# tiangexiang/OccNeRF

Measured on AMD Instinct MI355X. Metric: rays/sec at 512x512x128spp, random-init ckpt, higher is better.
Workload: dtype f32; 1 GPU; BASELINE configs[1]: free-view frame, 512x512 image, 128 samples/ray, non-rigid motion on, seeded random-init checkpoint; synthetic SMPL-like body and camera; 183784 rays hit the body bbox (ray_mask); H2D of the ray batch and the prior and D2H of [R,5] inside the step; the frame's rays sharded over the ranks; samples whose motion-weight sum is exactly 0 are dropped after the warp (bit-identical pi; rays_per_frame=183784, samples_per_ray=128, skip_empty_samples=True, dedup_repeated_samples=False, knn_center_cache=True, warp_bone_culling=True, world_size_formed=1

## Files before the change

include/occnerf_hip.h:

```cpp
#ifndef OCCNERF_HIP_H
#define OCCNERF_HIP_H

#include <stdint.h>

#ifdef __cplusplus
extern "C" {
#endif

#define OCCNERF_ABI_VERSION 5

int occnerf_abi_version(void);
const char *occnerf_last_error(void);

int occnerf_experiment_knob(const char *name, int value);


int occnerf_grid_encode_forward(const float *inputs, const float *embeddings,
                                const int32_t *offsets, float *outputs, uint32_t B, uint32_t D,
                                uint32_t C, uint32_t L, float S, uint32_t H, float *dy_dx,
                                uint32_t gridtype, int align_corners, uint32_t interp,
                                void *stream);

int occnerf_grid_encode_backward(const float *grad, const float *inputs, const float *embeddings,
                                 const int32_t *offsets, float *grad_embeddings, uint32_t B,
                                 uint32_t D, uint32_t C, uint32_t L, float S, uint32_t H,
                                 const float *dy_dx, float *grad_inputs, uint32_t gridtype,
                                 int align_corners, uint32_t interp, void *stream);

int occnerf_grid_encode_forward_h(const float *inputs, const float *embeddings, const int32_t *offsets,
                                  const int32_t *h_offsets, float *outputs, uint32_t B, uint32_t D, uint32_t C, uint32_t L,
                                  float S, uint32_t H, float *dy_dx, uint32_t gridtype, int align_corners,
                                  uint32_t interp, void *stream);

int occnerf_grid_grad_runs(const float *grad_rows, const float *inputs, int64_t B, uint32_t D, uint32_t L, uint32_t C,
                           float *grad, void *stream);

int occnerf_grid_encode_backward_h(const float *grad, const float *inputs, const float *embeddings,
                                   const int32_t *offsets, const int32_t *h_offsets, float *grad_embeddings,
                                   uint32_t B, uint32_t D, uint32_t C, uint32_t L, float S, uint32_t H,
                                   const float *dy_dx, float *grad_inputs, uint32_t gridtype, int align_corners,
                                   uint32_t interp, void *scratch, int64_t scratch_bytes, void *stream);

int occnerf_grid_encode_forward_f16(const float *inputs, const void *embeddings, const int32_t *offsets, void *outputs,
                                    uint32_t B, uint32_t D, uint32_t C, uint32_t L, float S, uint32_t H, void *dy_dx,
                                    uint32_t gridtype, int align_corners, uint32_t interp, void *stream);
int occnerf_grid_encode_backward_f16(const void *grad, const float *inputs, const void *embeddings, const int32_t *offsets,
                                     void *grad_embeddings, uint32_t B, uint32_t D, uint32_t C, uint32_t L, float S,
                                     uint32_t H, const void *dy_dx, void *grad_inputs, uint32_t gridtype, int align_corners,
                                     uint32_t interp, void *stream);

int occnerf_grid_encode_forward_f64(const float *inputs, const double *embeddings, const int32_t *offsets, double *outputs,
                                    uint32_t B, uint32_t D, uint32_t C, uint32_t L, float S, uint32_t H, double *dy_dx,
                                    uint32_t gridtype, int align_corners, uint32_t interp, void *stream);
int occnerf_grid_encode_backward_f64(const double *grad, const float *inputs, const double *embeddings, const int32_t *offsets,
                                     double *grad_embeddings, uint32_t B, uint32_t D, uint32_t C, uint32_t L, float S,
                                     uint32_t H, const double *dy_dx, double *grad_inputs, uint32_t gridtype, int align_corners,
                                     uint32_t interp, void *stream);

int occnerf_grad_total_variation(const float *inputs, const float *embeddings, float *grad,
                                 const int32_t *offsets, float weight, uint32_t B, uint32_t D,
                                 uint32_t C, uint32_t L, float S, uint32_t H, uint32_t gridtype,
                                 int align_corners, void *stream);


int occnerf_sample_warp(const float *rays, int64_t n, int32_t S, const float *t_vals,
                        const float *t_rand, const float *Rs, const float *Ts, const float *vol,
                        int32_t nb, int32_t G, const float *h_bbox_min, const float *h_bbox_scale,
                        float *z_vals, float *pts, float *x_skel, float *mask, void *stream);
int occnerf_bone_boxes(const float *vol, int32_t nb, int32_t G, int32_t *boxes, void *stream);
int occnerf_sample_warp_culled(const float *rays, int64_t n, int32_t S, const float *t_vals,
                               const float *Rs, const float *Ts, const float *vol, int32_t nb, int32_t G,
                               const int32_t *boxes, const float *h_bbox_min, const float *h_bbox_scale,
                               float *z_vals, float *x_skel, float *mask, void *stream);

int64_t occnerf_ray_order_temp_bytes(int64_t R);
int occnerf_ray_order(const float *dirs, int64_t R, int64_t stride, int64_t *order, void *temp, int64_t temp_bytes,
                      void *stream);

int occnerf_gen_rays(const double *h_Kinv, const double *h_R, const double *h_T, int32_t f32_camera,
                     int32_t H, int32_t W, const double *h_bbox_min, const double *h_bbox_max, float *rays8,
                     uint8_t *mask, void *stream);

int64_t occnerf_nonrigid_packed_floats(void);
int occnerf_nonrigid_pack(const float *const *h_W, const float *const *h_b, float *packed,
                          void *stream);
int occnerf_nonrigid(const float *xyz_in, int64_t N, const float *cond, const float *h_hann,
                     const float *W0, const float *b0, float *packed, float *xyz_out,
                     void *stream);
int occnerf_nonrigid_rows(float *xyz, int64_t N_max, const int32_t *rows, const int32_t *n_dev,
                          const float *cond, const float *h_hann, const float *W0, const float *b0,
                          float *packed, void *stream);
int occnerf_nonrigid_direct(const float *xyz_in, int64_t N, const float *cond, const float *h_hann,
                            const float *W0, const float *b0, float *packed, float *xyz_out,
                            void *stream);

int64_t occnerf_nonrigid_packed_bf16_bytes(void);
int occnerf_nonrigid_pack_bf16(const float *const *h_W, void *packed_bf16, void *stream);
int occnerf_nonrigid_bf16x3(const float *xyz_in, int64_t N, const float *cond, const float *h_hann,
                            const float *W0, const float *b0, float *packed, const void *packed_bf16,
                            float *xyz_out, void *stream);
int occnerf_nonrigid_bf16x3_rows(float *xyz, int64_t N_max, const int32_t *rows, const int32_t *n_dev,
                                 const float *cond, const float *h_hann, const float *W0, const float *b0,
                                 float *packed, const void *packed_bf16, void *stream);

int occnerf_msknn(const float *xyz, int64_t N, const float *points, const int32_t *index_map,
                  const int32_t *h_scale_begin, const int32_t *h_seed_from_coarser,
                  int32_t nscale, int32_t *knn_idxs, void *stream);

int occnerf_msknn_clustered(const float *xyz, const float *mask, int64_t n_rays, int32_t samples_per_ray,
                            const float *points, const float *centers,
                            const int32_t *cluster_ranges, const float *cluster_radius, int32_t ncl,
                            const float *group_centers, const int32_t *group_ranges, const float *group_radius, int32_t ngrp,
                            const int32_t *h_coarse_rows, const int32_t *h_seed_from_coarser,
                            int32_t nscale, const int32_t *query_rows, const int32_t *n_query_dev, int32_t *ray_start,
                            int32_t *knn_idxs, void *stream);
int occnerf_knn_center(const float *c, const float *points, const int32_t *index_map, const int32_t *h_scale_begin,
                       int32_t nscale, float *center_out, int32_t *idx_out, void *stream);
int occnerf_msknn_clustered_centered(const float *xyz, const float *mask, int64_t n_rays, int32_t samples_per_ray,
                                     const float *points, const float *centers,
                                     const int32_t *cluster_ranges, const float *cluster_radius, int32_t ncl,
                                     const float *group_centers, const int32_t *group_ranges, const float *group_radius, int32_t ngrp,
                                     const int32_t *h_coarse_rows, const int32_t *h_seed_from_coarser,
                                     int32_t nscale, const int32_t *query_rows, const int32_t *n_query_dev, int32_t *ray_start,
                                     const float *center, const int32_t *center_idx, int32_t *knn_idxs, void *stream);

int occnerf_knn_small(const float *q, int32_t nq, const float *s, int32_t ns, int32_t k,
                      int32_t *idx, void *stream);

int occnerf_unit_normals(const double *normals, int32_t P, double *unit, void *stream);

int occnerf_point_sdf(const float *point_cloud, const float *point_base, const double *normals,
                      const double *unit_normals, const int32_t *kidx, int32_t P,
                      double *knn_base, float *dist, void *stream);

int occnerf_point_sdf_backward(const float *point_cloud, const float *point_base, const double *normals,
                               const double *unit_normals, const int32_t *kidx, int32_t P, const double *d_knn_base,
                               const float *d_dist, float *d_point_dist, void *stream);
int32_t occnerf_point_table_stride(void);
int occnerf_point_table(const double *knn_base, const float *point_sdf, const float *learnable,
                        int32_t P, float bound, float two_bound, const float *embeddings,
                        const int32_t *offsets, const int32_t *h_offsets, uint32_t L, float S,
                        uint32_t H, float *table, void *stream);

int occnerf_point_pack(const float *point_base, const double *normals, const double *unit_normals,
                       const float *counter, const float *table, int32_t P, float *point_geo,
                       float *point_tail, void *stream);
int occnerf_sample_features(const float *xyz, int64_t N, const int32_t *knn_idxs, int32_t nscale,
                            const float *point_base, const double *normals,
                            const double *unit_normals, const float *counter,
                            const float *table, float bound, float two_bound,
                            const float *embeddings, const int32_t *offsets,
                            const int32_t *h_offsets, uint32_t L, float S, uint32_t H,
                            const int32_t *geo_idxs, const float *att_in, const int32_t *rows,
                            const int32_t *n_dev, const float *point_geo, const float *point_tail, int32_t P,
                            float *mlp_in, float *raw, float *enc_in, void *stream);
int occnerf_sample_features_centered(const float *xyz, int64_t N, const int32_t *knn_idxs, int32_t nscale,
                            const float *point_base, const double *normals,
                            const double *unit_normals, const float *counter,
                            const float *table, float bound, float two_bound,
                            const float *embeddings, const int32_t *offsets,
                            const int32_t *h_offsets, uint32_t L, float S, uint32_t H,
                            const int32_t *geo_idxs, const float *att_in, const int32_t *rows,
                            const int32_t *n_dev, const float *point_geo, const float *point_tail, int32_t P,
                            const float *center, const float *center_agg,
                                     float *mlp_in, float *raw, float *enc_in, void *stream);

int occnerf_agg_forward(const float *feats, int32_t F, const int32_t *knn, const float *atts, int64_t N, int32_t K,
                        float *agg, void *stream);
int32_t occnerf_agg_backward_slices(int64_t N);
int64_t occnerf_agg_backward_scratch_bytes(int64_t N, int32_t F);
int occnerf_agg_backward(const float *grad_agg, int32_t F, const int32_t *knn, const float *atts, int64_t N,
                         int32_t K, int32_t P, float *partial, void *scratch, int64_t scratch_bytes, void *stream);

int64_t occnerf_live_rows_temp_bytes(int64_t N);
int occnerf_live_rows(const float *mask, int64_t N, int32_t *rows, int32_t *count, void *temp,
                      int64_t temp_bytes, void *stream);
int occnerf_scatter_raw(const float *raw_c, const int32_t *rows, const int32_t *n_dev, int64_t N_max,
                        float *raw_full, void *stream);

int64_t occnerf_repeat_heads_temp_bytes(int64_t N_max);
int occnerf_repeat_heads(const void *keys, int64_t stride_dwords, int32_t key_dwords, const int32_t *rows,
                         const int32_t *n_dev, int64_t N_max, int32_t *scan, int32_t *heads, int32_t *head_count,
                         float *head_mask, void *temp, int64_t temp_bytes, void *stream);
int64_t occnerf_unique_heads_temp_bytes(int64_t cap);
int occnerf_unique_heads(const void *keys, int64_t stride_dwords, int32_t key_dwords, const int32_t *heads,
                         const int32_t *n_dev, int64_t cap, int32_t *heads_out, int32_t *count_out, int32_t *scan,
                         const int32_t *n_scan_dev, int64_t scan_cap, void *temp, int64_t temp_bytes, void *stream);
int occnerf_scatter_raw_heads(const float *raw_h, const float *raw_c, const int32_t *rows, const int32_t *n_dev,
                              const int32_t *scanA, const int32_t *scanB, int64_t N_max, float *raw_full, void *stream);
int occnerf_canonical_mlp_rows(const float *mlp_in, const int32_t *in_rows, int64_t N_max, const int32_t *n_dev,
                               const float *packed, float *raw, void *stream);

int64_t occnerf_canonical_mlp_packed_floats(void);
int occnerf_canonical_mlp_pack(const float *const *h_W, const float *const *h_b, float *packed,
                               void *stream);

int occnerf_canonical_mlp(const float *mlp_in, int64_t N, const float *packed, float *raw,
                          void *stream);
int occnerf_canonical_mlp_direct(const float *mlp_in, int64_t N, const float *packed, float *raw,
                                 void *stream);
int occnerf_canonical_mlp_counted(const float *mlp_in, int64_t N_max, const int32_t *n_dev,
                                  const float *packed, float *raw, void *stream);

int64_t occnerf_canonical_mlp_packed_bf16_bytes(void);
int occnerf_canonical_mlp_pack_bf16(const float *const *h_W, void *packed_bf16, void *stream);
int occnerf_canonical_mlp_bf16x3(const float *mlp_in, int64_t N, const float *packed,
                                 const void *packed_bf16, float *raw, int32_t variant,
                                 void *stream);
int occnerf_canonical_mlp_bf16x3_rows(const float *mlp_in, const int32_t *in_rows, int64_t N_max,
                                      const int32_t *n_dev, const float *packed, const void *packed_bf16,
                                      float *raw, int32_t variant, void *stream);

int occnerf_canonical_mlp_pack_f16(const float *const *h_W, void *packed_f16, void *stream);
int occnerf_canonical_mlp_f16x3(const float *mlp_in, const int32_t *in_rows, int64_t N_max, const int32_t *n_dev,
                                const float *packed, const void *packed_f16, float *raw, uint32_t *domain_flag,
                                void *stream);
int occnerf_nonrigid_pack_f16(const float *const *h_W, void *packed_f16, void *stream);
int occnerf_nonrigid_f16x3(const float *xyz_in, int64_t N_max, const int32_t *rows, const int32_t *n_dev,
                           const float *cond, const float *h_hann, const float *W0, const float *b0, float *packed,
                           const void *packed_f16, float *xyz_out, uint32_t *domain_flag, void *stream);

int occnerf_composite(const float *raw, const float *mask, const float *z_vals, const float *rays,
                      const float *h_bgcolor, int64_t n, int32_t S, float *rgb, float *acc,
                      float *depth, float *weights, int32_t *term, const int64_t *out_rows, void *stream);


int occnerf_linear_pack(const float *W, const float *b, int32_t out_dim, int32_t in_dim, const int32_t *row_map,
                        int32_t n_pad, const int32_t *col_map, int32_t k_pad, int32_t bf16, void *Wp, void *Wt,
                        float *bias_p, void *stream);
int occnerf_linear_forward(const void *x0, int64_t ld0, int32_t k0, const void *x1, int64_t ld1, int32_t k1,
                           const void *W, const float *bias, int32_t relu, const void *mask, int64_t ldm, void *y,
                           int64_t ldy, int32_t out_f32, int32_t n_store, float *aux, int32_t aux_col,
                           int64_t aux_stride, int64_t M, int32_t n_pad, int32_t bf16, void *stream);
int32_t occnerf_linear_wgrad_slices(int64_t M);
int occnerf_linear_wgrad(const void *dz, int64_t lddz, int32_t n_pad, const void *x, int64_t ldx, int32_t k_pad,
                         int64_t M, int32_t bf16, float *part, float *dbpart, void *stream);
int occnerf_linear_wgrad_reduce(const float *part, const float *dbpart, int32_t G, int32_t n_pad, int32_t k_pad,
                                const int32_t *row_map, const int32_t *col_map, float *dW, int32_t in_dim, float *db,
                                int32_t accumulate, void *stream);

int64_t occnerf_trunks_packed_bytes(void);
int occnerf_trunks_pack_bf16(const float *const *h_W, void *packed, void *stream);
int occnerf_trunks_forward_bf16(const float *agg, const float *var, const float *enc, int64_t M, const float *packed_f32,
                                const void *packed_bf16, void *X0, void *const *h_A, void *GEO, void *const *h_B, float *raw4,
                                void *stream);

int occnerf_composite_backward(const float *raw, const float *mask, const float *z_vals, const float *rays,
                               const float *h_bgcolor, int64_t n, int32_t S, const float *g_rgb, const float *g_acc,
                               const float *g_depth, float *d_raw, float *d_mask, void *stream);

int32_t occnerf_warp_backward_slices(int64_t n_samples);
int occnerf_warp_backward(const float *rays, int64_t n, int32_t S, const float *z_vals, const float *g_mask,
                          const float *Rs, const float *Ts, const float *vol, int32_t nb, int32_t G,
                          const float *h_bbox_min, const float *h_bbox_scale, float *d_vol_part, float *d_rt_part,
                          void *stream);

int occnerf_agg_weights(const float *counter, const int32_t *knn, int64_t N, int32_t K, float *atts, float *var,
                        void *stream);

int occnerf_pose_motion_bases_backward(const float *const *h_W, const float *const *h_b, const float *posevec,
                                       const float *dst_Rs, const float *dst_Ts, const float *cnl_gtfms,
                                       const float *dRs, const float *dTs, float *const *h_dW, float *const *h_db,
                                       void *stream);

int occnerf_pose_motion_bases(const float *const *h_W, const float *const *h_b, const float *posevec, int32_t refine,
                              const float *dst_Rs, const float *dst_Ts, const float *cnl_gtfms, float *Rs, float *Ts,
                              void *stream);
int occnerf_prior_softmax(const float *decoded, const float *prior, int32_t C, int64_t V, float *vol, void *stream);
int occnerf_pack_rays(const float *rays, const float *near, const float *far, const int64_t *order, int64_t R, float *rays8,
                      void *stream);

int occnerf_assemble_image(const float *rgb, const float *alpha, const int64_t *ray_index, int64_t R, int32_t height,
                           int32_t width, const float *h_bgcolor01, uint8_t *out_rgb, uint8_t *out_alpha, void *stream);

int occnerf_convt3d_col2im(const float *cols, const float *bias, int32_t Cout, int32_t D, int32_t H, int32_t W,
                           float *out, void *stream);
int occnerf_convt3d_im2col(const float *gy, int32_t Cout, int32_t D, int32_t H, int32_t W, float *dcols, void *stream);

int32_t occnerf_adam_table_row_bytes(void);
int occnerf_adam_step(const void *table, int32_t n_tensors, const int32_t *chunks, int32_t n_chunks,
                      int32_t chunk_elems, double beta1, double beta2, double eps, double max_grad_norm, float *scratch,
                      void *stream);

int64_t occnerf_lpips_packed_floats(void);
int64_t occnerf_lpips_workspace_floats(int32_t N, int32_t H, int32_t W);
int occnerf_lpips_pack(const float *const *h_conv_w, const float *const *h_conv_b, const float *const *h_lin,
                       const float *shift, const float *scale, float *packed, void *stream);
int occnerf_lpips_forward(const float *packed, const float *in0, const float *in1, int32_t N, int32_t H, int32_t W,
                          int32_t in_nhwc, float *work, float *val, float *res, void *stream);
int occnerf_lpips_backward(const float *packed, float *work, int32_t N, int32_t H, int32_t W, int32_t in_nhwc,
                           const float *gres, float *d_in0, float *d_in1, void *stream);

int occnerf_patch_assemble(const float *rgb, const int32_t *row_of_pix, int64_t R, int32_t n_patches, int32_t size,
                           const float *h_bgcolor01, float *img, void *stream);
int occnerf_patch_assemble_backward(const float *d_img, const int32_t *pix_of_row, int64_t R, float *d_rgb, void *stream);

#define OCCNERF_FRAME_METRICS_RECORD 14
int64_t occnerf_frame_metrics_workspace_bytes(int32_t N, int32_t H, int32_t W);
int occnerf_frame_metrics(const uint8_t *pred, const uint8_t *truth, const float *alpha, const uint8_t *body,
                          const float *gt_vis_alpha, const float *gt_alpha, int32_t N, int32_t H, int32_t W,
                          double data_range, double *record, double *ssim_map, void *workspace, void *stream);

#ifdef __cplusplus
}
#endif
#endif
```

occnerf_amd/_lib.py:

```python
import ctypes as C
import os

_HERE = os.path.dirname(os.path.abspath(__file__))
LIB_PATH = os.environ.get('OCCNERF_HIP_LIB') or os.path.join(_HERE, 'liboccnerf_hip.so')

ABI_VERSION = 5

_vp, _i32, _i64, _u32, _f32 = C.c_void_p, C.c_int32, C.c_int64, C.c_uint32, C.c_float

SIGNATURES = {
    'occnerf_abi_version': (C.c_int, []),
    'occnerf_last_error': (C.c_char_p, []),
    'occnerf_experiment_knob': (C.c_int, [C.c_char_p, C.c_int]),
    'occnerf_grid_encode_forward': (C.c_int, [_vp, _vp, _vp, _vp, _u32, _u32, _u32, _u32, _f32, _u32,
                                               _vp, _u32, C.c_int, _u32, _vp]),
    'occnerf_grid_encode_backward': (C.c_int, [_vp, _vp, _vp, _vp, _vp, _u32, _u32, _u32, _u32, _f32,
                                                _u32, _vp, _vp, _u32, C.c_int, _u32, _vp]),
    'occnerf_grid_grad_runs': (C.c_int, [_vp, _vp, _i64, _u32, _u32, _u32, _vp, _vp]),
    'occnerf_grid_encode_forward_h': (C.c_int, [_vp, _vp, _vp, _vp, _vp, _u32, _u32, _u32, _u32, _f32, _u32,
                                                 _vp, _u32, C.c_int, _u32, _vp]),
    'occnerf_grid_encode_backward_h': (C.c_int, [_vp, _vp, _vp, _vp, _vp, _vp, _u32, _u32, _u32, _u32, _f32,
                                                  _u32, _vp, _vp, _u32, C.c_int, _u32, _vp, _i64, _vp]),
    'occnerf_grid_encode_forward_f16': (C.c_int, [_vp, _vp, _vp, _vp, _u32, _u32, _u32, _u32, _f32, _u32,
                                                   _vp, _u32, C.c_int, _u32, _vp]),
    'occnerf_grid_encode_backward_f16': (C.c_int, [_vp, _vp, _vp, _vp, _vp, _u32, _u32, _u32, _u32, _f32,
                                                    _u32, _vp, _vp, _u32, C.c_int, _u32, _vp]),
    'occnerf_grid_encode_forward_f64': (C.c_int, [_vp, _vp, _vp, _vp, _u32, _u32, _u32, _u32, _f32, _u32,
                                                   _vp, _u32, C.c_int, _u32, _vp]),
    'occnerf_grid_encode_backward_f64': (C.c_int, [_vp, _vp, _vp, _vp, _vp, _u32, _u32, _u32, _u32, _f32,
                                                    _u32, _vp, _vp, _u32, C.c_int, _u32, _vp]),
    'occnerf_trunks_packed_bytes': (_i64, []),
    'occnerf_trunks_pack_bf16': (C.c_int, [_vp, _vp, _vp]),
    'occnerf_trunks_forward_bf16': (C.c_int, [_vp, _vp, _vp, _i64, _vp, _vp, _vp, _vp, _vp, _vp, _vp, _vp]),
    'occnerf_grad_total_variation': (C.c_int, [_vp, _vp, _vp, _vp, _f32, _u32, _u32, _u32, _u32, _f32,
                                                _u32, _u32, C.c_int, _vp]),
    'occnerf_sample_warp': (C.c_int, [_vp, _i64, _i32, _vp, _vp, _vp, _vp, _vp, _i32, _i32, _vp, _vp,
                                       _vp, _vp, _vp, _vp, _vp]),
    'occnerf_bone_boxes': (C.c_int, [_vp, _i32, _i32, _vp, _vp]),
    'occnerf_sample_warp_culled': (C.c_int, [_vp, _i64, _i32, _vp, _vp, _vp, _vp, _i32, _i32, _vp, _vp, _vp, _vp, _vp, _vp, _vp]),
    'occnerf_nonrigid_packed_floats': (_i64, []),
    'occnerf_nonrigid_pack': (C.c_int, [_vp, _vp, _vp, _vp]),
    'occnerf_nonrigid': (C.c_int, [_vp, _i64, _vp, _vp, _vp, _vp, _vp, _vp, _vp]),
    'occnerf_nonrigid_direct': (C.c_int, [_vp, _i64, _vp, _vp, _vp, _vp, _vp, _vp, _vp]),
    'occnerf_nonrigid_packed_bf16_bytes': (_i64, []),
    'occnerf_nonrigid_pack_bf16': (C.c_int, [_vp, _vp, _vp]),
    'occnerf_nonrigid_bf16x3': (C.c_int, [_vp, _i64, _vp, _vp, _vp, _vp, _vp, _vp, _vp, _vp]),
    'occnerf_nonrigid_bf16x3_rows': (C.c_int, [_vp, _i64, _vp, _vp, _vp, _vp, _vp, _vp, _vp, _vp, _vp]),
    'occnerf_msknn': (C.c_int, [_vp, _i64, _vp, _vp, _vp, _vp, _i32, _vp, _vp]),
    'occnerf_msknn_clustered': (C.c_int, [_vp, _vp, _i64, _i32, _vp, _vp, _vp, _vp, _i32, _vp, _vp, _vp, _i32, _vp, _vp, _i32,
                                           _vp, _vp, _vp, _vp, _vp]),
    'occnerf_msknn_clustered_centered': (C.c_int, [_vp, _vp, _i64, _i32, _vp, _vp, _vp, _vp, _i32, _vp, _vp, _vp, _i32, _vp, _vp, _i32,
                                           _vp, _vp, _vp, _vp, _vp, _vp, _vp]),
    'occnerf_knn_center': (C.c_int, [_vp, _vp, _vp, _vp, _i32, _vp, _vp, _vp]),
    'occnerf_knn_small': (C.c_int, [_vp, _i32, _vp, _i32, _i32, _vp, _vp]),
    'occnerf_unit_normals': (C.c_int, [_vp, _i32, _vp, _vp]),
    'occnerf_point_sdf': (C.c_int, [_vp, _vp, _vp, _vp, _vp, _i32, _vp, _vp, _vp]),
    'occnerf_ray_order_temp_bytes': (_i64, [_i64]),
    'occnerf_ray_order': (C.c_int, [_vp, _i64, _i64, _vp, _vp, _i64, _vp]),
    'occnerf_point_sdf_backward': (C.c_int, [_vp, _vp, _vp, _vp, _vp, _i32, _vp, _vp, _vp, _vp]),
    'occnerf_gen_rays': (C.c_int, [_vp, _vp, _vp, _i32, _i32, _i32, _vp, _vp, _vp, _vp, _vp]),
    'occnerf_agg_forward': (C.c_int, [_vp, _i32, _vp, _vp, _i64, _i32, _vp, _vp]),
    'occnerf_agg_backward_slices': (_i32, [_i64]),
    'occnerf_agg_backward_scratch_bytes': (_i64, [_i64, _i32]),
    'occnerf_agg_backward': (C.c_int, [_vp, _i32, _vp, _vp, _i64, _i32, _i32, _vp, _vp, _i64, _vp]),
    'occnerf_live_rows_temp_bytes': (_i64, [_i64]),
    'occnerf_live_rows': (C.c_int, [_vp, _i64, _vp, _vp, _vp, _i64, _vp]),
    'occnerf_scatter_raw': (C.c_int, [_vp, _vp, _vp, _i64, _vp, _vp]),
    'occnerf_repeat_heads_temp_bytes': (_i64, [_i64]),
    'occnerf_repeat_heads': (C.c_int, [_vp, _i64, _i32, _vp, _vp, _i64, _vp, _vp, _vp, _vp, _vp, _i64, _vp]),
    'occnerf_unique_heads_temp_bytes': (_i64, [_i64]),
    'occnerf_unique_heads': (C.c_int, [_vp, _i64, _i32, _vp, _vp, _i64, _vp, _vp, _vp, _vp, _i64, _vp, _i64, _vp]),
    'occnerf_scatter_raw_heads': (C.c_int, [_vp, _vp, _vp, _vp, _vp, _vp, _i64, _vp, _vp]),
    'occnerf_canonical_mlp_rows': (C.c_int, [_vp, _vp, _i64, _vp, _vp, _vp, _vp]),
    'occnerf_canonical_mlp_counted': (C.c_int, [_vp, _i64, _vp, _vp, _vp, _vp]),
    'occnerf_nonrigid_rows': (C.c_int, [_vp, _i64, _vp, _vp, _vp, _vp, _vp, _vp, _vp, _vp]),
    'occnerf_point_table_stride': (_i32, []),
    'occnerf_point_table': (C.c_int, [_vp, _vp, _vp, _i32, _f32, _f32, _vp, _vp, _vp, _u32, _f32, _u32, _vp,
                                       _vp]),
    'occnerf_point_pack': (C.c_int, [_vp, _vp, _vp, _vp, _vp, _i32, _vp, _vp, _vp]),
    'occnerf_sample_features': (C.c_int, [_vp, _i64, _vp, _i32, _vp, _vp, _vp, _vp, _vp, _f32, _f32, _vp,
                                           _vp, _vp, _u32, _f32, _u32, _vp, _vp, _vp, _vp, _vp, _vp, _i32, _vp, _vp,
                                           _vp, _vp]),
    'occnerf_sample_features_centered': (C.c_int, [_vp, _i64, _vp, _i32, _vp, _vp, _vp, _vp, _vp, _f32, _f32, _vp,
                                                    _vp, _vp, _u32, _f32, _u32, _vp, _vp, _vp, _vp, _vp, _vp, _i32, _vp, _vp,
                                                    _vp, _vp, _vp, _vp]),
    'occnerf_canonical_mlp_packed_floats': (_i64, []),
    'occnerf_canonical_mlp_pack': (C.c_int, [_vp, _vp, _vp, _vp]),
    'occnerf_canonical_mlp': (C.c_int, [_vp, _i64, _vp, _vp, _vp]),
    'occnerf_canonical_mlp_direct': (C.c_int, [_vp, _i64, _vp, _vp, _vp]),
    'occnerf_canonical_mlp_packed_bf16_bytes': (_i64, []),
    'occnerf_canonical_mlp_pack_bf16': (C.c_int, [_vp, _vp, _vp]),
    'occnerf_canonical_mlp_bf16x3': (C.c_int, [_vp, _i64, _vp, _vp, _vp, _i32, _vp]),
    'occnerf_canonical_mlp_pack_f16': (C.c_int, [_vp, _vp, _vp]),
    'occnerf_canonical_mlp_f16x3': (C.c_int, [_vp, _vp, _i64, _vp, _vp, _vp, _vp, _vp, _vp]),
    'occnerf_nonrigid_pack_f16': (C.c_int, [_vp, _vp, _vp]),
    'occnerf_nonrigid_f16x3': (C.c_int, [_vp, _i64, _vp, _vp, _vp, _vp, _vp, _vp, _vp, _vp, _vp, _vp, _vp]),
    'occnerf_canonical_mlp_bf16x3_rows': (C.c_int, [_vp, _vp, _i64, _vp, _vp, _vp, _vp, _i32, _vp]),
    'occnerf_composite': (C.c_int, [_vp, _vp, _vp, _vp, _vp, _i64, _i32, _vp, _vp, _vp, _vp, _vp, _vp, _vp]),
    'occnerf_linear_pack': (C.c_int, [_vp, _vp, _i32, _i32, _vp, _i32, _vp, _i32, _i32, _vp, _vp, _vp, _vp]),
    'occnerf_linear_forward': (C.c_int, [_vp, _i64, _i32, _vp, _i64, _i32, _vp, _vp, _i32, _vp, _i64, _vp, _i64, _i32,
                                          _i32, _vp, _i32, _i64, _i64, _i32, _i32, _vp]),
    'occnerf_linear_wgrad_slices': (_i32, [_i64]),
    'occnerf_linear_wgrad': (C.c_int, [_vp, _i64, _i32, _vp, _i64, _i32, _i64, _i32, _vp, _vp, _vp]),
    'occnerf_linear_wgrad_reduce': (C.c_int, [_vp, _vp, _i32, _i32, _i32, _vp, _vp, _vp, _i32, _vp, _i32, _vp]),
    'occnerf_composite_backward': (C.c_int, [_vp, _vp, _vp, _vp, _vp, _i64, _i32, _vp, _vp, _vp, _vp, _vp, _vp]),
    'occnerf_warp_backward_slices': (_i32, [_i64]),
    'occnerf_warp_backward': (C.c_int, [_vp, _i64, _i32, _vp, _vp, _vp, _vp, _vp, _i32, _i32, _vp, _vp, _vp, _vp, _vp]),
    'occnerf_agg_weights': (C.c_int, [_vp, _vp, _i64, _i32, _vp, _vp, _vp]),
    'occnerf_pose_motion_bases': (C.c_int, [_vp, _vp, _vp, _i32, _vp, _vp, _vp, _vp, _vp, _vp]),
    'occnerf_pose_motion_bases_backward': (C.c_int, [_vp, _vp, _vp, _vp, _vp, _vp, _vp, _vp, _vp, _vp, _vp]),
    'occnerf_prior_softmax': (C.c_int, [_vp, _vp, _i32, _i64, _vp, _vp]),
    'occnerf_pack_rays': (C.c_int, [_vp, _vp, _vp, _vp, _i64, _vp, _vp]),
    'occnerf_assemble_image': (C.c_int, [_vp, _vp, _vp, _i64, _i32, _i32, _vp, _vp, _vp, _vp]),
    'occnerf_convt3d_col2im': (C.c_int, [_vp, _vp, _i32, _i32, _i32, _i32, _vp, _vp]),
    'occnerf_convt3d_im2col': (C.c_int, [_vp, _i32, _i32, _i32, _i32, _vp, _vp]),
    'occnerf_adam_table_row_bytes': (_i32, []),
    'occnerf_adam_step': (C.c_int, [_vp, _i32, _vp, _i32, _i32] + [C.c_double] * 4 + [_vp, _vp]),
    'occnerf_lpips_packed_floats': (_i64, []),
    'occnerf_lpips_workspace_floats': (_i64, [_i32, _i32, _i32]),
    'occnerf_lpips_pack': (C.c_int, [_vp, _vp, _vp, _vp, _vp, _vp, _vp]),
    'occnerf_lpips_forward': (C.c_int, [_vp, _vp, _vp, _i32, _i32, _i32, _i32, _vp, _vp, _vp, _vp]),
    'occnerf_lpips_backward': (C.c_int, [_vp, _vp, _i32, _i32, _i32, _i32, _vp, _vp, _vp, _vp]),
    'occnerf_patch_assemble': (C.c_int, [_vp, _vp, _i64, _i32, _i32, _vp, _vp, _vp]),
    'occnerf_patch_assemble_backward': (C.c_int, [_vp, _vp, _i64, _vp, _vp]),
    'occnerf_frame_metrics_workspace_bytes': (_i64, [_i32, _i32, _i32]),
    'occnerf_frame_metrics': (C.c_int, [_vp, _vp, _vp, _vp, _vp, _vp, _i32, _i32, _i32, C.c_double, _vp, _vp, _vp, _vp]),
}

_lib = None


def lib():
    global _lib
    if _lib is None:
        if not os.path.exists(LIB_PATH):
            raise ImportError(
                f'{LIB_PATH} not found: the gfx950 kernels are not built. Run '
                '`python -c "import __graft_entry__ as g; g.build()"` (or `make -C '
                'occnerf_amd/csrc`). There is no CPU fallback for this path.')
        import torch
        handle = C.CDLL(LIB_PATH)
        for name, (res, args) in SIGNATURES.items():
            fn = getattr(handle, name)
            fn.restype, fn.argtypes = res, args
        if handle.occnerf_abi_version() != ABI_VERSION:
            raise ImportError(f'liboccnerf_hip.so: ABI version {handle.occnerf_abi_version()}, this binding was written '
                              f'for {ABI_VERSION} (include/occnerf_hip.h OCCNERF_ABI_VERSION): rebuild the library')
        _lib = handle
    return _lib


def check(rc, what):
    if rc != 0:
        msg = lib().occnerf_last_error().decode(errors='replace')
        raise RuntimeError(f'{what} failed ({rc}): {msg}')
```

occnerf_amd/csrc/compact.hip:

```cpp
#include "common.h"

#include <hipcub/hipcub.hpp>

namespace occ {

struct LivePredicate {
    const float *mask;
    __device__ bool operator()(const int &i) const { return mask[i] != 0.0f; }
};

__global__ void scatter_raw_kernel(const float *__restrict__ raw_c, const int32_t *__restrict__ rows,
                                   const int32_t *__restrict__ n_dev, float *__restrict__ raw_full) {
    const int64_t m = (int64_t)blockIdx.x * blockDim.x + threadIdx.x;
    if (m >= (int64_t)*n_dev) return;
    const int64_t n = rows[m];
#pragma unroll
    for (int c = 0; c < 5; c++) raw_full[n * 5 + c] = raw_c[m * 5 + c];
}

struct RepeatFlag {
    const uint32_t *keys;
    int64_t stride;
    int K;
    const int32_t *rows;
    const int32_t *n_dev;
    __device__ int operator()(const int &m) const {
        if (m >= *n_dev) return 0;
        if (m == 0) return 1;
        const uint32_t *a = keys + (rows ? (int64_t)rows[m] : (int64_t)m) * stride;
        const uint32_t *b = keys + (rows ? (int64_t)rows[m - 1] : (int64_t)(m - 1)) * stride;
        if (((K | (int)stride) & 3) == 0) {
            for (int k = 0; k < K; k += 4) {
                const uint4 x = *reinterpret_cast<const uint4 *>(a + k), y = *reinterpret_cast<const uint4 *>(b + k);
                if (x.x != y.x || x.y != y.y || x.z != y.z || x.w != y.w) return 1;
            }
            return 0;
        }
        for (int k = 0; k < K; k++)
            if (a[k] != b[k]) return 1;
        return 0;
    }
};

__global__ void repeat_flags_wide_kernel(const uint4 *__restrict__ keys, int64_t stride4, int K4,
                                         const int32_t *__restrict__ rows, const int32_t *__restrict__ n_dev,
                                         int64_t N_max, int32_t *__restrict__ flags) {
    const int g = threadIdx.x & 7;
    const int64_t m = ((int64_t)blockIdx.x * blockDim.x + threadIdx.x) >> 3;
    if (m >= N_max) return;
    const int64_t n = *n_dev;
    int diff = 0;
    if (m < n && m > 0) {
        const uint4 *a = keys + (rows ? (int64_t)rows[m] : m) * stride4;
        const uint4 *b = keys + (rows ? (int64_t)rows[m - 1] : m - 1) * stride4;
        for (int k = g; k < K4; k += 8) {
            const uint4 x = a[k], y = b[k];
            diff |= (x.x != y.x) | (x.y != y.y) | (x.z != y.z) | (x.w != y.w);
        }
    }
    diff |= __shfl_xor(diff, 1, 8);
    diff |= __shfl_xor(diff, 2, 8);
    diff |= __shfl_xor(diff, 4, 8);
    if (g == 0) flags[m] = m >= n ? 0 : (m == 0 ? 1 : diff);
}

__global__ void repeat_heads_kernel(const int32_t *__restrict__ scan, const int32_t *__restrict__ rows,
                                    const int32_t *__restrict__ n_dev, int32_t *__restrict__ heads,
                                    int32_t *__restrict__ head_count, float *__restrict__ head_mask) {
    const int64_t m = (int64_t)blockIdx.x * blockDim.x + threadIdx.x;
    const int64_t n = *n_dev;
    if (m == 0 && n <= 0) *head_count = 0;
    if (m >= n) return;
    const int32_t s = scan[m], prev = m ? scan[m - 1] : 0;
    if (s != prev) {
        const int32_t r = rows ? rows[m] : (int32_t)m;
        heads[s - 1] = r;
        if (head_mask) head_mask[r] = 1.0f;
    }
    if (m == n - 1) *head_count = s;
}

__global__ void scatter_raw_heads_kernel(const float *__restrict__ raw_h, const float *__restrict__ raw_c,
                                         const int32_t *__restrict__ rows, const int32_t *__restrict__ n_dev,
                                         const int32_t *__restrict__ scanA, const int32_t *__restrict__ scanB,
                                         float *__restrict__ raw_full) {
    const int64_t m = (int64_t)blockIdx.x * blockDim.x + threadIdx.x;
    if (m >= (int64_t)*n_dev) return;
    const int64_t n = rows[m];
    const int64_t a = scanA ? scanA[m] - 1 : m;
    const int64_t h = scanB ? scanB[a] - 1 : a;
#pragma unroll
    for (int c = 0; c < 4; c++) raw_full[n * 5 + c] = raw_h[h * 5 + c];
    raw_full[n * 5 + 4] = raw_c[a * 5 + 4];
}

__device__ __forceinline__ uint64_t mix64(uint64_t h) {
    h ^= h >> 33;
    h *= 0xff51afd7ed558ccdull;
    h ^= h >> 33;
    h *= 0xc4ceb9fe1a85ec53ull;
    h ^= h >> 33;
    return h;
}

template <int G >
__global__ void unique_insert_kernel(const uint32_t *__restrict__ keys, int64_t stride, int K,
                                     const int32_t *__restrict__ heads, const int32_t *__restrict__ n_dev,
                                     int32_t *__restrict__ table, uint32_t tmask, int32_t *__restrict__ rep) {
    const int g = threadIdx.x % G;
    const int64_t j = ((int64_t)blockIdx.x * blockDim.x + threadIdx.x) / G;
    if (j >= (int64_t)*n_dev) return;
    const uint32_t *a = keys + (heads ? (int64_t)heads[j] : j) * stride;
    uint64_t h = 0x9E3779B97F4A7C15ull * (uint64_t)(g + 1);
    for (int k = g; k < K; k += G) h = mix64(h ^ ((uint64_t)a[k] + ((uint64_t)(k + 1) << 32)));
    if (G > 1) {
        h ^= __shfl_xor(h, 1, G);
        h ^= __shfl_xor(h, 2, G);
        h ^= __shfl_xor(h, 4, G);
    }
    uint32_t slot = (uint32_t)mix64(h) & tmask;
    int32_t r = (int32_t)j;
    for (int probe = 0; probe < 32; probe++) {
        int32_t prev = 0;
        if (g == 0) prev = atomicCAS(&table[slot], -1, (int32_t)j);
        if (G > 1) prev = __shfl(prev, 0, G);
        if (prev == -1) break;
        const uint32_t *b = keys + (heads ? (int64_t)heads[prev] : (int64_t)prev) * stride;
        int diff = 0;
        for (int k = g; k < K; k += G) diff |= a[k] != b[k];
        if (G > 1) {
            diff |= __shfl_xor(diff, 1, G);
            diff |= __shfl_xor(diff, 2, G);
            diff |= __shfl_xor(diff, 4, G);
        }
        if (!diff) {
            r = prev;
            break;
        }
        slot = (slot + 1) & tmask;
    }
    if (g == 0) rep[j] = r;
}

struct IsRepresentative {
    const int32_t *rep, *n_dev;
    __device__ int operator()(const int &j) const { return j < *n_dev && rep[j] == j; }
};

__global__ void unique_finish_kernel(const int32_t *__restrict__ heads, const int32_t *__restrict__ n_dev,
                                     const int32_t *__restrict__ scan2, int32_t *__restrict__ rep,
                                     int32_t *__restrict__ heads_out, int32_t *__restrict__ count_out) {
    const int64_t j = (int64_t)blockIdx.x * blockDim.x + threadIdx.x;
    const int64_t n = *n_dev;
    if (j == 0 && n <= 0) *count_out = 0;
    if (j >= n) return;
    const int32_t r = rep[j];
    if (r == (int32_t)j) heads_out[scan2[j] - 1] = heads ? heads[j] : (int32_t)j;
    if (j == n - 1) *count_out = scan2[j];
    rep[j] = scan2[r] - 1;
}

__global__ void unique_remap_kernel(int32_t *__restrict__ scan, const int32_t *__restrict__ n_scan_dev,
                                    const int32_t *__restrict__ pos) {
    const int64_t m = (int64_t)blockIdx.x * blockDim.x + threadIdx.x;
    if (m >= (int64_t)*n_scan_dev) return;
    scan[m] = pos[scan[m] - 1] + 1;
}

}

OCC_API int64_t occnerf_repeat_heads_temp_bytes(int64_t N) {
    using namespace occ;
    if (N <= 0 || N >= (1ll << 31)) return 0;
    size_t bytes = 0;
    hipcub::CountingInputIterator<int> it(0);
    hipcub::TransformInputIterator<int, RepeatFlag, hipcub::CountingInputIterator<int>> flags(it, RepeatFlag{});
    if (hipcub::DeviceScan::InclusiveSum(nullptr, bytes, flags, (int *)nullptr, (int)N, (hipStream_t)0) != hipSuccess)
        return -1;
    size_t bytes2 = 0;
    if (hipcub::DeviceScan::InclusiveSum(nullptr, bytes2, (int *)nullptr, (int *)nullptr, (int)N, (hipStream_t)0) != hipSuccess)
        return -1;
    return (int64_t)(bytes > bytes2 ? bytes : bytes2);
}

OCC_API int occnerf_repeat_heads(const void *keys, int64_t stride_dwords, int32_t key_dwords, const int32_t *rows,
                                 const int32_t *n_dev, int64_t N_max, int32_t *scan, int32_t *heads,
                                 int32_t *head_count, float *head_mask, void *temp, int64_t temp_bytes,
                                 void *stream) {
    using namespace occ;
    OCC_REQUIRE(keys && n_dev && scan && heads && head_count && temp, "repeat_heads: null argument");
    OCC_REQUIRE(N_max > 0 && N_max < (1ll << 31), "repeat_heads: N=%lld out of range", (long long)N_max);
    OCC_REQUIRE(key_dwords > 0 && stride_dwords >= key_dwords, "repeat_heads: key of %d dwords in rows of %lld",
                key_dwords, (long long)stride_dwords);
    size_t bytes = (size_t)temp_bytes;
    hipError_t e;
    if (key_dwords >= 32 && ((key_dwords | stride_dwords) & 3) == 0) {
        const int64_t fblocks = (N_max * 8 + 255) / 256;
        OCC_REQUIRE(fblocks < (1ll << 31), "repeat_heads: N too large");
        hipLaunchKernelGGL(repeat_flags_wide_kernel, dim3((unsigned)fblocks), dim3(256), 0, as_stream(stream),
                           reinterpret_cast<const uint4 *>(keys), stride_dwords / 4, key_dwords / 4, rows, n_dev, N_max, scan);
        e = hipcub::DeviceScan::InclusiveSum(temp, bytes, scan, scan, (int)N_max, as_stream(stream));
    } else {
        hipcub::CountingInputIterator<int> it(0);
        hipcub::TransformInputIterator<int, RepeatFlag, hipcub::CountingInputIterator<int>> flags(
            it, RepeatFlag{reinterpret_cast<const uint32_t *>(keys), stride_dwords, key_dwords, rows, n_dev});
        e = hipcub::DeviceScan::InclusiveSum(temp, bytes, flags, scan, (int)N_max, as_stream(stream));
    }
    OCC_REQUIRE(e == hipSuccess, "repeat_heads: %s", hipGetErrorString(e));
    const int64_t blocks = (N_max + 255) / 256;
    hipLaunchKernelGGL(repeat_heads_kernel, dim3((unsigned)blocks), dim3(256), 0, as_stream(stream), scan, rows, n_dev,
                       heads, head_count, head_mask);
    return check_launch("repeat_heads");
}

static inline int64_t unique_table_entries(int64_t cap) {
    int64_t t = 1024;
    while (t < cap) t <<= 1;
    return t;
}

OCC_API int64_t occnerf_unique_heads_temp_bytes(int64_t cap) {
    using namespace occ;
    if (cap <= 0 || cap >= (1ll << 30)) return 0;
    size_t bytes = 0;
    hipcub::CountingInputIterator<int> it(0);
    hipcub::TransformInputIterator<int, IsRepresentative, hipcub::CountingInputIterator<int>> flags(it, IsRepresentative{});
    if (hipcub::DeviceScan::InclusiveSum(nullptr, bytes, flags, (int *)nullptr, (int)cap, (hipStream_t)0) != hipSuccess)
        return -1;
    const int64_t words = unique_table_entries(cap) + 2 * ((cap + 63) & ~63ll);
    return words * 4 + (int64_t)((bytes + 255) & ~(size_t)255);
}

OCC_API int occnerf_unique_heads(const void *keys, int64_t stride_dwords, int32_t key_dwords, const int32_t *heads,
                                 const int32_t *n_dev, int64_t cap, int32_t *heads_out, int32_t *count_out,
                                 int32_t *scan, const int32_t *n_scan_dev, int64_t scan_cap, void *temp,
                                 int64_t temp_bytes, void *stream) {
    using namespace occ;
    OCC_REQUIRE(keys && n_dev && heads_out && count_out && temp, "unique_heads: null argument");
    OCC_REQUIRE(cap > 0 && cap < (1ll << 30), "unique_heads: cap=%lld out of range", (long long)cap);
    OCC_REQUIRE(key_dwords > 0 && stride_dwords >= key_dwords, "unique_heads: key of %d dwords in rows of %lld", key_dwords,
                (long long)stride_dwords);
    OCC_REQUIRE(!scan == !n_scan_dev, "unique_heads: scan and its length come together");
    OCC_REQUIRE(temp_bytes >= occnerf_unique_heads_temp_bytes(cap), "unique_heads: temp too small");
    const int64_t T = unique_table_entries(cap), capr = (cap + 63) & ~63ll;
    int32_t *table = reinterpret_cast<int32_t *>(temp), *rep = table + T, *scan2 = rep + capr;
    void *cub_temp = scan2 + capr;
    size_t cub_bytes = (size_t)temp_bytes - (size_t)(T + 2 * capr) * 4;
    hipStream_t st = as_stream(stream);
    OCC_REQUIRE(hipMemsetAsync(table, 0xFF, (size_t)T * 4, st) == hipSuccess, "unique_heads: memset");
    const uint32_t *k32 = reinterpret_cast<const uint32_t *>(keys);
    if (key_dwords >= 32)
        hipLaunchKernelGGL(unique_insert_kernel<8>, dim3((unsigned)((cap * 8 + 255) / 256)), dim3(256), 0, st, k32,
                           stride_dwords, key_dwords, heads, n_dev, table, (uint32_t)(T - 1), rep);
    else
        hipLaunchKernelGGL(unique_insert_kernel<1>, dim3((unsigned)((cap + 255) / 256)), dim3(256), 0, st, k32,
                           stride_dwords, key_dwords, heads, n_dev, table, (uint32_t)(T - 1), rep);
    hipcub::CountingInputIterator<int> it(0);
    hipcub::TransformInputIterator<int, IsRepresentative, hipcub::CountingInputIterator<int>> flags(
        it, IsRepresentative{rep, n_dev});
    const hipError_t e = hipcub::DeviceScan::InclusiveSum(cub_temp, cub_bytes, flags, scan2, (int)cap, st);
    OCC_REQUIRE(e == hipSuccess, "unique_heads: %s", hipGetErrorString(e));
    hipLaunchKernelGGL(unique_finish_kernel, dim3((unsigned)((cap + 255) / 256)), dim3(256), 0, st, heads, n_dev, scan2, rep,
                       heads_out, count_out);
    if (scan)
        hipLaunchKernelGGL(unique_remap_kernel, dim3((unsigned)((scan_cap + 255) / 256)), dim3(256), 0, st, scan, n_scan_dev,
                           rep);
    return check_launch("unique_heads");
}

OCC_API int occnerf_scatter_raw_heads(const float *raw_h, const float *raw_c, const int32_t *rows, const int32_t *n_dev,
                                      const int32_t *scanA, const int32_t *scanB, int64_t N_max, float *raw_full,
                                      void *stream) {
    using namespace occ;
    if (N_max <= 0) return 0;
    OCC_REQUIRE(raw_h && raw_c && rows && n_dev && raw_full, "scatter_raw_heads: null argument");
    const int64_t blocks = (N_max + 255) / 256;
    OCC_REQUIRE(blocks < (1ll << 31), "scatter_raw_heads: N too large");
    hipLaunchKernelGGL(scatter_raw_heads_kernel, dim3((unsigned)blocks), dim3(256), 0, as_stream(stream), raw_h, raw_c,
                       rows, n_dev, scanA, scanB, raw_full);
    return check_launch("scatter_raw_heads");
}

OCC_API int64_t occnerf_live_rows_temp_bytes(int64_t N) {
    using namespace occ;
    if (N <= 0 || N >= (1ll << 31)) return 0;
    size_t bytes = 0;
    hipcub::CountingInputIterator<int> it(0);
    if (hipcub::DeviceSelect::If(nullptr, bytes, it, (int *)nullptr, (int *)nullptr, (int)N, LivePredicate{nullptr},
                                 (hipStream_t)0) != hipSuccess)
        return -1;
    return (int64_t)bytes;
}

OCC_API int occnerf_live_rows(const float *mask, int64_t N, int32_t *rows, int32_t *count, void *temp,
                              int64_t temp_bytes, void *stream) {
    using namespace occ;
    OCC_REQUIRE(mask && rows && count && temp, "live_rows: null argument");
    OCC_REQUIRE(N > 0 && N < (1ll << 31), "live_rows: N=%lld out of range", (long long)N);
    size_t bytes = (size_t)temp_bytes;
    hipcub::CountingInputIterator<int> it(0);
    const hipError_t e = hipcub::DeviceSelect::If(temp, bytes, it, rows, count, (int)N, LivePredicate{mask},
                                                  as_stream(stream));
    OCC_REQUIRE(e == hipSuccess, "live_rows: %s", hipGetErrorString(e));
    return check_launch("live_rows");
}

OCC_API int occnerf_scatter_raw(const float *raw_c, const int32_t *rows, const int32_t *n_dev, int64_t N_max,
                                float *raw_full, void *stream) {
    using namespace occ;
    if (N_max <= 0) return 0;
    OCC_REQUIRE(raw_c && rows && n_dev && raw_full, "scatter_raw: null argument");
    const int64_t blocks = (N_max + 255) / 256;
    OCC_REQUIRE(blocks < (1ll << 31), "scatter_raw: N too large");
    hipLaunchKernelGGL(scatter_raw_kernel, dim3((unsigned)blocks), dim3(256), 0, as_stream(stream), raw_c, rows, n_dev,
                       raw_full);
    return check_launch("scatter_raw");
}
```

occnerf_amd/csrc/composite.hip:

```cpp
#include "common.h"

namespace occ {

__device__ __forceinline__ float softplus_t20(float x) {
    return x > 20.0f ? x : log1pf(expf(x));
}

__device__ __forceinline__ float wave_sum(float v) {
#pragma unroll
    for (int o = 32; o > 0; o >>= 1) v += __shfl_xor(v, o);
    return v;
}

struct CompositeParams {
    float bg[3];
};

__global__ __launch_bounds__(256) void composite_kernel(
    const float *__restrict__ raw, const float *__restrict__ mask, const float *__restrict__ z_vals,
    const float *__restrict__ rays, CompositeParams prm, int64_t n, int S, float *__restrict__ rgb_map,
    float *__restrict__ acc_map, float *__restrict__ depth_map, float *__restrict__ weights,
    int32_t *__restrict__ term, const int64_t *__restrict__ out_rows) {
    const int lane = threadIdx.x & 63;
    const int64_t wave = ((int64_t)blockIdx.x * blockDim.x + threadIdx.x) >> 6;
    const int64_t nwaves = ((int64_t)gridDim.x * blockDim.x) >> 6;
    for (int64_t r = wave; r < n; r += nwaves) {
        const float *ry = rays + r * 8;
        const float dn = norm3(ry[3], ry[4], ry[5]);
        float carry = 1.0f;
        float sr = 0.f, sg = 0.f, sb = 0.f, sd = 0.f, sa = 0.f;
        float best_a = -INFINITY;
        int best_s = 0;
        for (int s0 = 0; s0 < S; s0 += kWave) {
            const int s = s0 + lane;
            const bool live = s < S;
            const int64_t i = r * S + (live ? s : S - 1);
            const float z = z_vals[i];
            float alpha = 0.0f, c0 = 0.f, c1 = 0.f, c2 = 0.f;
            if (live) {
                const float zn = s + 1 < S ? z_vals[i + 1] : 0.0f;
                float dist = s + 1 < S ? __fsub_rn(zn, z) : 1e10f;
                dist = __fmul_rn(dist, dn);
                const float *rw = raw + i * 5;
                const float sp = softplus_t20(rw[3]);
                alpha = __fsub_rn(1.0f, expf(-__fmul_rn(sp, dist)));
                alpha = __fmul_rn(alpha, mask[i]);
                c0 = 1.0f / (1.0f + expf(-rw[0]));
                c1 = 1.0f / (1.0f + expf(-rw[1]));
                c2 = 1.0f / (1.0f + expf(-rw[2]));
            }
            const float t = live ? __fadd_rn(__fsub_rn(1.0f, alpha), 1e-10f) : 1.0f;
            float incl = t;
#pragma unroll
            for (int o = 1; o < kWave; o <<= 1) {
                const float up = __shfl_up(incl, o);
                if (lane >= o) incl *= up;
            }
            float excl = __shfl_up(incl, 1);
            if (lane == 0) excl = 1.0f;
            const float T = carry * excl;
            carry *= __shfl(incl, kWave - 1);
            const float w = live ? alpha * T : 0.0f;
            if (weights && live) weights[i] = w;
            sr += w * c0;
            sg += w * c1;
            sb += w * c2;
            sd += w * z;
            sa += w;
            if (live && alpha > best_a) {
                best_a = alpha;
                best_s = s;
            }
        }
        sr = wave_sum(sr);
        sg = wave_sum(sg);
        sb = wave_sum(sb);
        sd = wave_sum(sd);
        sa = wave_sum(sa);
        if (term) {
#pragma unroll
            for (int o = 32; o > 0; o >>= 1) {
                const float oa = __shfl_xor(best_a, o);
                const int os = __shfl_xor(best_s, o);
                if (oa > best_a || (oa == best_a && os < best_s)) {
                    best_a = oa;
                    best_s = os;
                }
            }
        }
        if (lane == 0) {
            const float rem = 1.0f - sa;
            const int64_t o = out_rows ? out_rows[r] : r;
            rgb_map[o * 3 + 0] = sr + rem * prm.bg[0] / 255.0f;
            rgb_map[o * 3 + 1] = sg + rem * prm.bg[1] / 255.0f;
            rgb_map[o * 3 + 2] = sb + rem * prm.bg[2] / 255.0f;
            acc_map[o] = sa;
            depth_map[o] = sd;
            if (term) term[o] = best_s;
        }
    }
}

}

OCC_API int occnerf_composite(const float *raw, const float *mask, const float *z_vals,
                              const float *rays, const float *h_bgcolor, int64_t n, int32_t S,
                              float *rgb, float *acc, float *depth, float *weights, int32_t *term,
                              const int64_t *out_rows, void *stream) {
    using namespace occ;
    if (n <= 0) return 0;
    OCC_REQUIRE(raw && mask && z_vals && rays && h_bgcolor && rgb && acc && depth, "composite: null argument");
    OCC_REQUIRE(S >= 1, "composite: S=%d", S);
    if (n <= 0) return 0;
    CompositeParams prm;
    for (int c = 0; c < 3; c++) prm.bg[c] = h_bgcolor[c];
    int64_t blocks = (n + 3) / 4;
    if (blocks > (int64_t)kNumCU * 32) blocks = (int64_t)kNumCU * 32;
    hipLaunchKernelGGL(composite_kernel, dim3((unsigned)blocks), dim3(256), 0, as_stream(stream), raw, mask,
                       z_vals, rays, prm, n, S, rgb, acc, depth, weights, term, out_rows);
    return check_launch("composite");
}
```

occnerf_amd/csrc/features.hip:

```cpp
#include "common.h"

#include <cstdlib>

namespace occ {

constexpr int kKnn = 10;
constexpr int kTableCols = 36;
constexpr int kTableStride = 64;

__device__ __forceinline__ double cos3_unit(const float (&a)[3], const double *__restrict__ un) {
    float na = norm3(a[0], a[1], a[2]);
    na = na < 1e-8f ? 1e-8f : na;
    const double t0 = __dmul_rn((double)__fdiv_rn(a[0], na), un[0]);
    const double t1 = __dmul_rn((double)__fdiv_rn(a[1], na), un[1]);
    const double t2 = __dmul_rn((double)__fdiv_rn(a[2], na), un[2]);
    return __dadd_rn(__dadd_rn(t0, t1), t2);
}

__global__ void unit_normals_kernel(const double *__restrict__ normals, int P,
                                    double *__restrict__ unit) {
    const int i = blockIdx.x * blockDim.x + threadIdx.x;
    if (i >= P) return;
    const double b0 = normals[i * 3], b1 = normals[i * 3 + 1], b2 = normals[i * 3 + 2];
    double nb = __dsqrt_rn(__dadd_rn(__dadd_rn(__dmul_rn(b0, b0), __dmul_rn(b1, b1)), __dmul_rn(b2, b2)));
// ... 218 lines not shown
            }
        }
        float dist = __fdiv_rn(dsum, (float)kKnn);
        if (2 * neg > kKnn) dist = -dist;
        float nd = __fdiv_rn(__fadd_rn(dist, 0.2f), 0.5f);
        nd = nd < 0.0f ? 0.0f : (nd > 1.0f ? 1.0f : nd);
        float x[4];
#pragma unroll
        for (int c = 0; c < 3; c++) x[c] = (float)__ddiv_rn(num[c], den);
        x[3] = nd;
        if (enc_in_out) {
#pragma unroll
            for (int c = 0; c < 4; c++) enc_in_out[i * 4 + c] = x[c];
        }
        raw[i * 5 + 4] = dist;

        float *out = mlp_in + i * 68;

        bool oob = false;
#pragma unroll
        for (int d = 0; d < 4; d++) oob |= (x[d] < 0.f || x[d] > 1.f);
        for (int l = 0; l < prm.L; l++) {
            float2 v = make_float2(0.f, 0.f);
            if (!oob) {
                const uint32_t o0 = (uint32_t)offsets[l];
                v = encode_level_d4c2(x, embeddings + o0, (uint32_t)offsets[l + 1] - o0,
                                      lv.scale[l], lv.resolution[l], gm.mode[l]);
            }
            *reinterpret_cast<float2 *>(out + 36 + l * 2) = v;
        }

        float att[4 * kKnn];
        float amin = INFINITY;
#pragma unroll
        for (int j = 0; j < 4 * kKnn; j++) {
            att[j] = j < nk ? (att_in ? att_in[i * nk + j] : counter[id[j]]) : INFINITY;
            amin = fminf(amin, att[j]);
        }
        float amax = -INFINITY;
#pragma unroll
        for (int j = 0; j < 4 * kKnn; j++) {
            if (j < nk) {
                att[j] = __fadd_rn(att[j], __fsub_rn(1.0f, amin));
                amax = fmaxf(amax, att[j]);
            }
        }
        float mean = 0.0f;
#pragma unroll
        for (int j = 0; j < 4 * kKnn; j++) {
            if (j < nk) {
                att[j] = __fdiv_rn(att[j], amax);
                mean = __fadd_rn(mean, att[j]);
            }
        }
        mean = __fdiv_rn(mean, (float)nk);
        float var = 0.0f, smax = -INFINITY;
#pragma unroll
        for (int j = 0; j < 4 * kKnn; j++) {
            if (j < nk) {
                const float dlt = __fsub_rn(att[j], mean);
                var = __fadd_rn(var, __fmul_rn(dlt, dlt));
                smax = fmaxf(smax, att[j]);
            }
        }
        var = __fdiv_rn(var, (float)(nk - 1));
        float ssum = 0.0f;
#pragma unroll
        for (int j = 0; j < 4 * kKnn; j++) {
            if (j < nk) {
                att[j] = expf(__fsub_rn(att[j], smax));
                ssum = __fadd_rn(ssum, att[j]);
            }
        }
        float agg[kTableCols];
#pragma unroll
        for (int f = 0; f < kTableCols; f++) agg[f] = 0.0f;
#pragma unroll
        for (int j = 0; j < 4 * kKnn; j++) {
            if (j < nk) {
                const float a = __fdiv_rn(att[j], ssum);
                const float4 *row = table + (size_t)id[j] * (kTableStride / 4);
#pragma unroll
                for (int v = 0; v < kTableCols / 4; v++) {
                    const float4 t = row[v];
                    agg[v * 4 + 0] = __fadd_rn(agg[v * 4 + 0], __fmul_rn(a, t.x));
                    agg[v * 4 + 1] = __fadd_rn(agg[v * 4 + 1], __fmul_rn(a, t.y));
                    agg[v * 4 + 2] = __fadd_rn(agg[v * 4 + 2], __fmul_rn(a, t.z));
                    agg[v * 4 + 3] = __fadd_rn(agg[v * 4 + 3], __fmul_rn(a, t.w));
                }
            }
        }
        agg[35] = var;
#pragma unroll
        for (int v = 0; v < kTableCols / 4; v++)
            *reinterpret_cast<float4 *>(out + v * 4) =
                make_float4(agg[v * 4], agg[v * 4 + 1], agg[v * 4 + 2], agg[v * 4 + 3]);
    }
}


__global__ void point_pack_kernel(const float *__restrict__ point_base, const double *__restrict__ normals,
                                  const double *__restrict__ unit, const float *__restrict__ counter,
                                  const float *__restrict__ table, int P, float *__restrict__ geo,
                                  float4 *__restrict__ tailc) {
    const int i = blockIdx.x * blockDim.x + threadIdx.x;
    if (i >= P) return;
    float *r = geo + (size_t)i * 16;
    r[0] = point_base[i * 3], r[1] = point_base[i * 3 + 1], r[2] = point_base[i * 3 + 2], r[3] = 0.0f;
    double *d = reinterpret_cast<double *>(r + 4);
    d[0] = normals[i * 3], d[1] = normals[i * 3 + 1], d[2] = normals[i * 3 + 2];
    d[3] = unit[i * 3], d[4] = unit[i * 3 + 1], d[5] = unit[i * 3 + 2];
    const float *t = table + (size_t)i * kTableStride + 32;
    tailc[i] = make_float4(t[0], t[1], t[2], counter[i]);
}

__device__ __forceinline__ float grp_sum8(float v) {
    v += __shfl_xor(v, 1, 8);
    v += __shfl_xor(v, 2, 8);
    v += __shfl_xor(v, 4, 8);
    return v;
}
__device__ __forceinline__ float grp_min8(float v) {
    v = fminf(v, __shfl_xor(v, 1, 8));
    v = fminf(v, __shfl_xor(v, 2, 8));
    return fminf(v, __shfl_xor(v, 4, 8));
}
__device__ __forceinline__ float grp_max8(float v) {
    v = fmaxf(v, __shfl_xor(v, 1, 8));
    v = fmaxf(v, __shfl_xor(v, 2, 8));
    return fmaxf(v, __shfl_xor(v, 4, 8));
}

template <int Q>
__device__ __forceinline__ float quad_bcast(float v) {
    return __builtin_bit_cast(float, __builtin_amdgcn_mov_dpp(__builtin_bit_cast(int, v), Q * 0x55, 0xf, 0xf, true));
}
template <int Q>
__device__ __forceinline__ double quad_bcast_f64(float lo, float hi) {
    return __hiloint2double(__builtin_amdgcn_mov_dpp(__builtin_bit_cast(int, hi), Q * 0x55, 0xf, 0xf, true),
                            __builtin_amdgcn_mov_dpp(__builtin_bit_cast(int, lo), Q * 0x55, 0xf, 0xf, true));
}

constexpr int kLdsTailPoints = 9216;

template <bool GENERIC ,
          bool LDS_TAIL >
__global__ __launch_bounds__(LDS_TAIL ? 768 : 256, 3) void sample_features8_kernel(
    const float *__restrict__ xyz, int64_t N_max, const int32_t *__restrict__ knn_idxs,
    const float4 *__restrict__ geo , const float4 *__restrict__ tailc ,
    const float4 *__restrict__ table, const float2 *__restrict__ embeddings,
    LevelRecs levels, LevelRecs8 levels8, FeatParams prm, const int32_t *__restrict__ rows ,
    const int32_t *__restrict__ n_dev , float *__restrict__ mlp_in, float *__restrict__ raw, float *__restrict__ enc_in_out,
    const float *__restrict__ center ,
    const float *__restrict__ center_agg ) {
    constexpr int NK = 4 * kKnn;
    float ccx = 0.f, ccy = 0.f, ccz = 0.f, cr2 = 0.f;
    if (center) ccx = center[0], ccy = center[1], ccz = center[2], cr2 = center[3];
    __shared__ float4 s_tail[LDS_TAIL ? kLdsTailPoints : 1];
    __shared__ float4 s_out[LDS_TAIL ? 768 : 256];
    static_assert(sizeof(float4) * (size_t)kLdsTailPoints + sizeof(float4) * 768 <= 160 * 1024,
                  "sample_features8_kernel<LDS_TAIL>: (tail, count) image + per-lane encoding slots exceed gfx950's 160 KiB of LDS");
    if constexpr (LDS_TAIL) {
        for (int i = threadIdx.x; i < prm.P; i += blockDim.x) s_tail[i] = tailc[i];
        __syncthreads();
    }
    const int g = threadIdx.x & 7;
    const int lane64 = threadIdx.x & 63;
    const int tr = ((lane64 & 7) << 3) | (lane64 >> 3);
    const int64_t N = n_dev ? (int64_t)*n_dev : N_max;
    if (N <= 0) return;
    const int64_t group0 = ((int64_t)blockIdx.x * blockDim.x + threadIdx.x) >> 3;
    const int64_t ngroups = ((int64_t)gridDim.x * blockDim.x) >> 3;
    const int64_t iters = (N + ngroups - 1) / ngroups;

    struct StageA {
        float p[3];
        int idg, id89;
        int id5[5];
    };
    auto out_row = [&](int64_t it) {
        const int64_t i_raw = group0 + it * ngroups;
        return i_raw < N ? i_raw : N - 1;
    };
    auto load_a = [&](int64_t i, StageA &a) {
        const int32_t *id = knn_idxs + i * NK;
        struct __attribute__((packed, aligned(4))) F3 { float v[3]; };
        struct __attribute__((packed, aligned(4))) I4 { int v[4]; };
        const F3 pq = *reinterpret_cast<const F3 *>(xyz + i * 3);
        a.p[0] = pq.v[0], a.p[1] = pq.v[1], a.p[2] = pq.v[2];
        a.idg = id[g];
        a.id89 = id[8 + (g >> 2)];
        const I4 q = *reinterpret_cast<const I4 *>(id + g * 5);
        a.id5[0] = q.v[0], a.id5[1] = q.v[1], a.id5[2] = q.v[2], a.id5[3] = q.v[3];
        a.id5[4] = id[g * 5 + 4];
    };
    StageA cur, nxt;
    int32_t i1;
    {
        const int64_t o0 = out_row(0), o1 = out_row(1);
        load_a(rows ? (int64_t)rows[o0] : o0, cur);
        i1 = rows ? rows[o1] : (int32_t)o1;
    }
    for (int64_t it = 0; it < iters; it++) {
        const bool live = group0 + it * ngroups < N;
        const int64_t o = out_row(it);
        const int64_t o2 = out_row(it + 2);
        float *out = mlp_in + o * 68;

        bool cached_agg = false;
        if (cr2 > 0.0f) {
            const float dx = cur.p[0] - ccx, dy = cur.p[1] - ccy, dz = cur.p[2] - ccz;
            const bool inside = __builtin_fmaf(dz, dz, __builtin_fmaf(dy, dy, dx * dx)) < cr2;
            cached_agg = __builtin_amdgcn_ballot_w64(live && !inside) == 0;
        }
        float4 tl[5];
#pragma unroll
        for (int k = 0; k < 5; k++) tl[k] = make_float4(0.f, 0.f, 0.f, 0.f);
        if (!cached_agg) {
#pragma unroll
            for (int k = 0; k < 5; k++) tl[k] = LDS_TAIL ? s_tail[cur.id5[k]] : ld32(tailc, (uint32_t)cur.id5[k] * 16u);
        }

        float nrm[5];
        int negf[5];
        double t_att[2] = {0.0, 0.0}, t_num[2][3] = {{0.0, 0.0, 0.0}, {0.0, 0.0, 0.0}};
        {
            float4 pc[5];
#pragma unroll
            for (int k = 0; k < 5; k++) {
                const int nid = k < 4 ? __shfl(cur.idg, 2 * k + (g >> 2), 8) : cur.id89;
                pc[k] = ld32(geo, (uint32_t)nid * 64u + (uint32_t)(g & 3) * 16u);
            }
#pragma unroll
            for (int k = 0; k < 5; k++) {
                const float nbr[3] = {quad_bcast<0>(pc[k].x), quad_bcast<0>(pc[k].y), quad_bcast<0>(pc[k].z)};
                const double nx = quad_bcast_f64<1>(pc[k].x, pc[k].y), ny = quad_bcast_f64<1>(pc[k].z, pc[k].w);
                const double nz = quad_bcast_f64<2>(pc[k].x, pc[k].y);
                float dir[3];
#pragma unroll
                for (int c = 0; c < 3; c++) dir[c] = __fsub_rn(cur.p[c], nbr[c]);
                double dot = __dadd_rn(0.0, __dmul_rn((double)dir[0], nx));
                dot = __dadd_rn(dot, __dmul_rn((double)dir[1], ny));
                dot = __dadd_rn(dot, __dmul_rn((double)dir[2], nz));
                negf[k] = dot < 0.0;
                nrm[k] = norm3(dir[0], dir[1], dir[2]);
                if (k < 2) {
                    const double un[3] = {quad_bcast_f64<2>(pc[k].z, pc[k].w), quad_bcast_f64<3>(pc[k].x, pc[k].y),
                                          quad_bcast_f64<3>(pc[k].z, pc[k].w)};
                    t_att[k] = fabs(cos3_unit(dir, un));
#pragma unroll
                    for (int c = 0; c < 3; c++) {
                        const float pn = __fdiv_rn(__fadd_rn(nbr[c], prm.bound), prm.two_bound);
                        t_num[k][c] = __dmul_rn(t_att[k], (double)pn);
                    }
                }
            }
        }
        float dsum = 0.0f;
        int neg = 0;
#pragma unroll
        for (int j = 0; j < kKnn; j++) {
            dsum = __fadd_rn(dsum, __shfl(nrm[j >> 1], 4 * (j & 1), 8));
            neg += __shfl(negf[j >> 1], 4 * (j & 1), 8);
        }
        double num[3] = {0.0, 0.0, 0.0}, den = 0.0;
#pragma unroll
        for (int j = 0; j < 3; j++) {
#pragma unroll
            for (int c = 0; c < 3; c++) num[c] = __dadd_rn(num[c], __shfl(t_num[j >> 1][c], 4 * (j & 1), 8));
            den = __dadd_rn(den, __shfl(t_att[j >> 1], 4 * (j & 1), 8));
        }
        float dist = __fdiv_rn(dsum, (float)kKnn);
        if (2 * neg > kKnn) dist = -dist;
        float nd = __fdiv_rn(__fadd_rn(dist, 0.2f), 0.5f);
        nd = nd < 0.0f ? 0.0f : (nd > 1.0f ? 1.0f : nd);
        float x[4];
#pragma unroll
        for (int c = 0; c < 3; c++) x[c] = (float)__ddiv_rn(num[c], den);
        x[3] = nd;
        if (live && g == 0) {
            raw[o * 5 + 4] = dist;
            if (enc_in_out) *reinterpret_cast<float4 *>(enc_in_out + o * 4) = make_float4(x[0], x[1], x[2], x[3]);
        }

        float a5[5] = {0.f, 0.f, 0.f, 0.f, 0.f};
        float var = 0.0f;
        float tail[3] = {0.f, 0.f, 0.f};
        if (!cached_agg) {
            float lmin = INFINITY;
#pragma unroll
            for (int k = 0; k < 5; k++) {
                a5[k] = tl[k].w;
                lmin = fminf(lmin, a5[k]);
            }
            const float amin = grp_min8(lmin);
            float lmax = -INFINITY;
#pragma unroll
            for (int k = 0; k < 5; k++) {
                a5[k] = __fadd_rn(a5[k], __fsub_rn(1.0f, amin));
                lmax = fmaxf(lmax, a5[k]);
            }
            const float amax = grp_max8(lmax);
            float lsum = 0.0f;
#pragma unroll
            for (int k = 0; k < 5; k++) {
                a5[k] = __fdiv_rn(a5[k], amax);
                lsum += a5[k];
            }
            const float mean = __fdiv_rn(grp_sum8(lsum), (float)NK);
            float lvar = 0.0f, lsm = -INFINITY;
#pragma unroll
            for (int k = 0; k < 5; k++) {
                const float dl = a5[k] - mean;
                lvar += dl * dl;
                lsm = fmaxf(lsm, a5[k]);
            }
            var = __fdiv_rn(grp_sum8(lvar), (float)(NK - 1));
            const float smax = grp_max8(lsm);
            float le = 0.0f;
#pragma unroll
            for (int k = 0; k < 5; k++) {
                a5[k] = expf(__fsub_rn(a5[k], smax));
                le += a5[k];
            }
            const float ssum = grp_sum8(le);
#pragma unroll
            for (int k = 0; k < 5; k++) a5[k] = __fdiv_rn(a5[k], ssum);

#pragma unroll
            for (int k = 0; k < 5; k++) {
                tail[0] += a5[k] * tl[k].x;
                tail[1] += a5[k] * tl[k].y;
                tail[2] += a5[k] * tl[k].z;
            }
        }

        bool cached_enc = false;
        if (cached_agg) {
            const bool eq = __float_as_uint(x[0]) == __float_as_uint(center_agg[36]) && __float_as_uint(x[1]) == __float_as_uint(center_agg[37]) &&
                            __float_as_uint(x[2]) == __float_as_uint(center_agg[38]) && __float_as_uint(x[3]) == __float_as_uint(center_agg[39]);
            cached_enc = __builtin_amdgcn_ballot_w64(live && !eq) == 0;
        }
        float2 ev[2];
        int32_t i2;
        if (!cached_enc) {
            LevelTaps4 tp[2];
            bool oob = false;
            float xt[4];
#pragma unroll
            for (int d = 0; d < 4; d++) xt[d] = __shfl(x[d], tr);
#pragma unroll
            for (int d = 0; d < 4; d++) oob |= (xt[d] < 0.f || xt[d] > 1.f);
            __builtin_amdgcn_sched_barrier(0);
            if (oob) {
#pragma unroll
                for (int d = 0; d < 4; d++) xt[d] = 0.5f;
            }
#pragma unroll
            for (int a = 0; a < 2; a++) {
                if constexpr (GENERIC) {
                    const LevelRec4 lr = levels.r[2 * (lane64 >> 3) + a];
                    encode_level_d4c2_taps(xt, embeddings, lr.size, lr.scale, lr.res_mode & 0xFFFFFFu, lr.res_mode >> 24,
                                           lr.entry0, tp[a]);
                } else {
                    level_taps_select(xt, embeddings, levels8.r[2 * (lane64 >> 3) + a], tp[a]);
                }
// ... 14 lines not shown
            i2 = rows ? rows[o2] : (int32_t)o2;
            const float4 ce = *reinterpret_cast<const float4 *>(center_agg + 40 + 4 * g);
            ev[0] = make_float2(ce.x, ce.y), ev[1] = make_float2(ce.z, ce.w);
        }
        s_out[threadIdx.x] = make_float4(ev[0].x, ev[0].y, ev[1].x, ev[1].y);

        float agg[4] = {0.f, 0.f, 0.f, 0.f};
        if (!cached_agg) {
            const uint32_t piece = (uint32_t)g * 16u;
            auto issue_chunk = [&](int c, float4 (&t)[10]) {
#pragma unroll
                for (int h = 0; h < 2; h++) {
#pragma unroll
                    for (int k = 0; k < 5; k++)
#ifdef OCC_FEAT_EXP_RESIDENT_ROWS
                        t[h * 5 + k] = ld32(table, (uint32_t)(__shfl(cur.id5[k], 2 * c + h, 8) & 15) * (uint32_t)(kTableStride * 4) + piece);
#else
                        t[h * 5 + k] = ld32(table, (uint32_t)__shfl(cur.id5[k], 2 * c + h, 8) * (uint32_t)(kTableStride * 4) + piece);
#endif
                }
            };
            float4 b0[10], b1[10], b2[10];
            issue_chunk(0, b0);
            issue_chunk(1, b1);
    #pragma unroll 1
            for (int c = 0; c < 4; c++) {
                const int cn = c + 2 < 4 ? c + 2 : 3;
                issue_chunk(cn, b2);
#pragma unroll
                for (int h = 0; h < 2; h++) {
#pragma unroll
                    for (int k = 0; k < 5; k++) {
                        const float w = __shfl(a5[k], 2 * c + h, 8);
                        const float4 t = b0[h * 5 + k];
                        agg[0] = __fadd_rn(agg[0], __fmul_rn(w, t.x));
                        agg[1] = __fadd_rn(agg[1], __fmul_rn(w, t.y));
                        agg[2] = __fadd_rn(agg[2], __fmul_rn(w, t.z));
                        agg[3] = __fadd_rn(agg[3], __fmul_rn(w, t.w));
                    }
                }
#pragma unroll
                for (int k = 0; k < 10; k++) b0[k] = b1[k], b1[k] = b2[k];
            }
#pragma unroll
            for (int c = 0; c < 3; c++) tail[c] = grp_sum8(tail[c]);
        } else {
            const float4 ca = *reinterpret_cast<const float4 *>(center_agg + 4 * g);
            agg[0] = ca.x, agg[1] = ca.y, agg[2] = ca.z, agg[3] = ca.w;
            tail[0] = center_agg[32], tail[1] = center_agg[33], tail[2] = center_agg[34], var = center_agg[35];
        }
        if (live) {
            *reinterpret_cast<float4 *>(out + 4 * g) = make_float4(agg[0], agg[1], agg[2], agg[3]);
            if (g == 0) *reinterpret_cast<float4 *>(out + 32) = make_float4(tail[0], tail[1], tail[2], var);
            *reinterpret_cast<float4 *>(out + 36 + 4 * g) = s_out[threadIdx.x];
        }
        cur = nxt;
        i1 = i2;
    }
}


}

OCC_API int occnerf_unit_normals(const double *normals, int32_t P, double *unit, void *stream) {
    using namespace occ;
    OCC_REQUIRE(normals && unit, "unit_normals: null argument");
    if (P <= 0) return 0;
    hipLaunchKernelGGL(unit_normals_kernel, dim3((P + 255) / 256), dim3(256), 0, as_stream(stream), normals, P, unit);
    return check_launch("unit_normals");
}

OCC_API int occnerf_point_sdf(const float *point_cloud, const float *point_base,
                              const double *normals, const double *unit_normals,
                              const int32_t *kidx, int32_t P, double *knn_base, float *dist,
                              void *stream) {
    using namespace occ;
    OCC_REQUIRE(point_cloud && point_base && normals && unit_normals && kidx && knn_base && dist,
                "point_sdf: null argument");
    if (P <= 0) return 0;
    hipLaunchKernelGGL(point_sdf_kernel, dim3((P + 255) / 256), dim3(256), 0, as_stream(stream), point_cloud,
                       point_base, normals, unit_normals, kidx, P, knn_base, dist);
    return check_launch("point_sdf");
}

OCC_API int occnerf_point_sdf_backward(const float *point_cloud, const float *point_base, const double *normals,
                                       const double *unit_normals, const int32_t *kidx, int32_t P, const double *d_knn_base,
                                       const float *d_dist, float *d_point_dist, void *stream) {
    using namespace occ;
    OCC_REQUIRE(point_cloud && point_base && normals && unit_normals && kidx && d_knn_base && d_dist && d_point_dist,
                "point_sdf_backward: null argument");
    if (P <= 0) return 0;
    hipLaunchKernelGGL(point_sdf_backward_kernel, dim3((P + 255) / 256), dim3(256), 0, as_stream(stream), point_cloud, point_base,
                       normals, unit_normals, kidx, P, d_knn_base, d_dist, d_point_dist);
    return check_launch("point_sdf_backward");
}

OCC_API int32_t occnerf_point_table_stride(void) { return occ::kTableStride; }

OCC_API int occnerf_point_table(const double *knn_base, const float *point_sdf,
                                const float *learnable, int32_t P, float bound, float two_bound,
                                const float *embeddings, const int32_t *offsets,
                                const int32_t *h_offsets, uint32_t L, float S, uint32_t H, float *table,
                                void *stream) {
    using namespace occ;
    OCC_REQUIRE(knn_base && point_sdf && learnable && embeddings && offsets && table, "point_table: null argument");
    OCC_REQUIRE(L >= 1 && L <= 16, "point_table: L=%u unsupported", L);
    if (P <= 0) return 0;
    const GridLevels lv = make_grid_levels(L, S, H);
    const GridModes4 gm = modes_from_host_offsets(L, lv, h_offsets);
    hipLaunchKernelGGL(point_table_kernel, dim3((P + 255) / 256), dim3(256), 0, as_stream(stream), knn_base,
                       point_sdf, learnable, P, bound, two_bound, reinterpret_cast<const float2 *>(embeddings),
                       offsets, (int)L, lv, gm, table);
    return check_launch("point_table");
}

OCC_API int occnerf_point_pack(const float *point_base, const double *normals, const double *unit_normals,
                               const float *counter, const float *table, int32_t P, float *point_geo,
                               float *point_tail, void *stream) {
    using namespace occ;
    OCC_REQUIRE(point_base && normals && unit_normals && counter && table && point_geo && point_tail,
                "point_pack: null argument");
    if (P <= 0) return 0;
    hipLaunchKernelGGL(point_pack_kernel, dim3((P + 255) / 256), dim3(256), 0, as_stream(stream), point_base, normals,
                       unit_normals, counter, table, P, point_geo, reinterpret_cast<float4 *>(point_tail));
    return check_launch("point_pack");
}

OCC_API int occnerf_sample_features(const float *xyz, int64_t N, const int32_t *knn_idxs,
                                    int32_t nscale, const float *point_base, const double *normals,
                                    const double *unit_normals, const float *counter,
                                    const float *table, float bound, float two_bound,
                                    const float *embeddings, const int32_t *offsets,
                                    const int32_t *h_offsets, uint32_t L, float S, uint32_t H,
                                    const int32_t *geo_idxs,
                                    const float *att_in, const int32_t *rows, const int32_t *n_dev,
                                    const float *point_geo, const float *point_tail, int32_t P,
                                    float *mlp_in, float *raw, float *enc_in, void *stream) {
    return occnerf_sample_features_centered(xyz, N, knn_idxs, nscale, point_base, normals, unit_normals, counter, table, bound,
                                            two_bound, embeddings, offsets, h_offsets, L, S, H, geo_idxs, att_in, rows, n_dev,
                                            point_geo, point_tail, P, nullptr, nullptr, mlp_in, raw, enc_in, stream);
}

OCC_API int occnerf_sample_features_centered(const float *xyz, int64_t N, const int32_t *knn_idxs,
                                             int32_t nscale, const float *point_base, const double *normals,
                                             const double *unit_normals, const float *counter,
                                             const float *table, float bound, float two_bound,
                                             const float *embeddings, const int32_t *offsets,
                                             const int32_t *h_offsets, uint32_t L, float S, uint32_t H,
                                             const int32_t *geo_idxs,
                                             const float *att_in, const int32_t *rows, const int32_t *n_dev,
                                             const float *point_geo, const float *point_tail, int32_t P,
                                             const float *center, const float *center_agg,
                                             float *mlp_in, float *raw, float *enc_in, void *stream) {
    using namespace occ;
    OCC_REQUIRE(!center == !center_agg, "sample_features: center and center_agg come together");
    if (N <= 0) return 0;
    OCC_REQUIRE(xyz && knn_idxs && point_base && normals && unit_normals && (counter || att_in) && table &&
                    embeddings && offsets && mlp_in && raw, "sample_features: null argument");
    OCC_REQUIRE(nscale >= 1 && nscale <= 4, "sample_features: nscale=%d unsupported", nscale);
    OCC_REQUIRE(L == 16, "sample_features: built for the 16-level encoder of occnerf_mlp.py:45 (L=%u)", L);
    if (N <= 0) return 0;
    const GridLevels lv = make_grid_levels(L, S, H);
    const GridModes4 gm = modes_from_host_offsets(L, lv, h_offsets);
    FeatParams prm{bound, two_bound, nscale, (int)L, (int)P};
    OCC_REQUIRE(!n_dev || rows, "sample_features: a device-side count needs the row list");
    OCC_REQUIRE(!point_geo == !point_tail, "sample_features: point_geo and point_tail come together (occnerf_point_pack)");
    const bool lanes8 = nscale == 4 && !geo_idxs && !att_in && counter && h_offsets && point_geo;
    OCC_REQUIRE(!rows || lanes8,
                "sample_features: a row list is only supported on the renderer's path (4 scales, per-point inputs, "
                "packed point records)");
    if (lanes8) {
        LevelRecs levels;
        for (uint32_t l = 0; l < kMaxLevels; l++)
            levels.r[l] = LevelRec4{(uint32_t)h_offsets[l], (uint32_t)(h_offsets[l + 1] - h_offsets[l]), lv.scale[l],
                                    lv.resolution[l] | (gm.mode[l] << 24)};
        LevelRecs8 levels8;
        bool generic = false;
        for (uint32_t l = 0; l < kMaxLevels; l++) {
            const uint32_t size = (uint32_t)(h_offsets[l + 1] - h_offsets[l]), r1 = lv.resolution[l] + 1;
            const bool dense = gm.mode[l] == kGridDense;
            generic |= gm.mode[l] == kGridGeneric;
            levels8.r[l] = LevelRec8{(uint32_t)h_offsets[l], dense ? 0xFFFFFFFFu : size - 1, lv.scale[l], dense ? 1u : 0u,
                                     dense ? r1 : 2654435761u, dense ? r1 * r1 : 805459861u,
                                     dense ? r1 * r1 * r1 : 3674653429u, 0u};
        }
        OCC_REQUIRE(P > 0, "sample_features: P=%d rows of packed point records", P);
        const bool lds_tail = P <= kLdsTailPoints && N >= 96 * 64;
        const int threads = lds_tail ? 768 : 256;
        int64_t blocks8 = (N * 8 + threads - 1) / threads;
        const int64_t cap = lds_tail ? (int64_t)kNumCU : (int64_t)kNumCU * 32;
        if (blocks8 > cap) blocks8 = cap;
        auto kern = generic ? (lds_tail ? sample_features8_kernel<true, true> : sample_features8_kernel<true, false>)
                            : (lds_tail ? sample_features8_kernel<false, true> : sample_features8_kernel<false, false>);
        hipLaunchKernelGGL(kern, dim3((unsigned)blocks8), dim3(threads), 0, as_stream(stream), xyz,
                           N, knn_idxs, reinterpret_cast<const float4 *>(point_geo),
                           reinterpret_cast<const float4 *>(point_tail),
                           reinterpret_cast<const float4 *>(table), reinterpret_cast<const float2 *>(embeddings),
                           levels, levels8, prm, rows, n_dev, mlp_in, raw, enc_in, center, center_agg);
        return check_launch("sample_features");
    }
    OCC_REQUIRE(!center, "sample_features: the centre aggregate is only supported on the renderer's path");
    int64_t blocks = (N + 255) / 256;
    if (blocks > (int64_t)kNumCU * 16) blocks = (int64_t)kNumCU * 16;
    hipLaunchKernelGGL(sample_features_kernel, dim3((unsigned)blocks), dim3(256), 0, as_stream(stream), xyz, N,
                       knn_idxs, point_base, normals, unit_normals, counter,
                       reinterpret_cast<const float4 *>(table), reinterpret_cast<const float2 *>(embeddings),
                       offsets, lv, gm, prm, geo_idxs, att_in, mlp_in, raw, enc_in);
    return check_launch("sample_features");
}
```

occnerf_amd/csrc/knn.hip:

```cpp
#include "common.h"

#include <map>
#include <mutex>
#include <utility>

#include <cmath>
#include <vector>

namespace occ {

typedef float f32x2 __attribute__((ext_vector_type(2)));

constexpr int kK = 10;

struct KBest {
    float s[kK];
    int i[kK];
};

__device__ __forceinline__ void kbest_reset(KBest &b) {
#pragma unroll
    for (int p = 0; p < kK; p++) {
        b.s[p] = INFINITY;
        b.i[p] = 0;
// ... 172 lines not shown
    if (threadIdx.x < sc.nscale * 10) {
        const int ls = threadIdx.x / 10, j = threadIdx.x % 10;
        idx_out[ls * 10 + j] = index_map[sc.begin[ls] + (int)(unsigned)s_key[ls][j]];
    }
    if (threadIdx.x == 0) {
        float g = INFINITY, dmax = 0.0f;
        for (int ls = 0; ls < sc.nscale; ls++) {
            if (s_key[ls][10] == ~0ull) g = 0.0f;
            for (int j = 0; j < 10; j++)
                g = fminf(g, __uint_as_float((unsigned)(s_key[ls][j + 1] >> 32)) - __uint_as_float((unsigned)(s_key[ls][j] >> 32)));
            if (s_key[ls][10] != ~0ull) dmax = fmaxf(dmax, __uint_as_float((unsigned)(s_key[ls][10] >> 32)));
        }
        const float r = 0.9f * (0.5f * g - 2e-6f * (dmax + 1.0f));
        center_out[0] = cx, center_out[1] = cy, center_out[2] = cz;
        center_out[3] = (r > 0.0f && r < INFINITY) ? r * r : 0.0f;
    }
}

struct ClusteredScales {
    int nscale, ncl, ngrp;
    int coarse_begin, coarse_end;
    int seed[4];
};

struct OneQuery {
    float x, y, z;
    bool live;
};

#define OCC_PT1(P)                                                                          \
    {                                                                                       \
        const float dx = q.x - P.x, dy = q.y - P.y, dz = q.z - P.z;                         \
        const float d2 = __builtin_fmaf(dz, dz, __builtin_fmaf(dy, dy, dx * dx));           \
        consider_lex(best, thr, sb, d2, __float_as_int(P.w));                               \
    }
#define OCC_SCAN1(JB, JE)                                                                   \
    {                                                                                       \
        const int je_ = (JE);                                                               \
        int j = (JB);                                                                       \
        float4 n0 = points[j], n1 = points[j + 1], n2 = points[j + 2], n3 = points[j + 3];  \
        for (; j < je_; j += 4) {                                                           \
            const float4 p0 = n0, p1 = n1, p2 = n2, p3 = n3;                                \
            const int jn = j + 4 < je_ ? j + 4 : j;                                         \
            n0 = points[jn], n1 = points[jn + 1], n2 = points[jn + 2], n3 = points[jn + 3]; \
            OCC_PT1(p0) OCC_PT1(p1) OCC_PT1(p2) OCC_PT1(p3)                                 \
        }                                                                                   \
    }
#define OCC_EMIT1(L)                                                                        \
    if (q.live) {                                                                           \
        struct __attribute__((packed, aligned(4))) I4 { int v[4]; };                        \
        struct __attribute__((packed, aligned(4))) I2 { int v[2]; };                        \
        int32_t *out = knn_idxs + (qi * sc.nscale + (L)) * kK;                              \
        int r_[kK];                                                                         \
        _Pragma("unroll") for (int p = 0; p < kK; p++) r_[p] = key_row(best.k[p]) & 0xFFFF; \
        *reinterpret_cast<I4 *>(out) = I4{{r_[0], r_[1], r_[2], r_[3]}};                    \
        *reinterpret_cast<I4 *>(out + 4) = I4{{r_[4], r_[5], r_[6], r_[7]}};                \
        *reinterpret_cast<I2 *>(out + 8) = I2{{r_[8], r_[9]}};                              \
    }

__device__ __forceinline__ void search_one_query(const OneQuery q, const int64_t qi, const int lane,
                                                 const float4 *__restrict__ points, const float4 *__restrict__ centers,
                                                 const int2 *__restrict__ ranges, const float *__restrict__ radius,
                                                 const float4 *__restrict__ gcenters, const int2 *__restrict__ granges,
                                                 const float *__restrict__ gradius, const ClusteredScales &sc,
                                                 int32_t *__restrict__ knn_idxs) {
    KBest64 best;
    float thr = q.live ? INFINITY : -1.0f, sb = INFINITY;
    kbest64_reset(best);
    OCC_SCAN1(sc.coarse_begin, sc.coarse_end)
    OCC_EMIT1(sc.nscale - 1)
    const unsigned long long lv = __builtin_amdgcn_ballot_w64(q.live);
    const int first = lv ? __builtin_ctzll(lv) : 0;
    const float rx = __shfl(q.x, first), ry = __shfl(q.y, first), rz = __shfl(q.z, first);
    for (int l = sc.nscale - 2; l >= 0; l--) {
        sb = sc.seed[l] ? key_dist(best.k[kK - 1]) : INFINITY;
        thr = q.live ? filter_bound(sb) : -1.0f;
        kbest64_reset(best);
        const int2 *rg = ranges + (size_t)l * sc.ncl;
        const float *rd = radius + (size_t)l * sc.ncl;
        int k_first;
        {
            float bd = INFINITY;
            int bk = 0;
            for (int k = lane; k < sc.ncl; k += kWave) {
                const float4 c = centers[k];
                const float dx = rx - c.x, dy = ry - c.y, dz = rz - c.z;
                const float d = dx * dx + dy * dy + dz * dz;
                const bool has = rg[k].x < rg[k].y;
                if (has && d < bd) {
                    bd = d;
                    bk = k;
                }
            }
#pragma unroll
            for (int o = 32; o > 0; o >>= 1) {
                const float od = __shfl_xor(bd, o);
                const int ok = __shfl_xor(bk, o);
                if (od < bd || (od == bd && ok < bk)) {
                    bd = od;
                    bk = ok;
                }
            }
            k_first = __builtin_amdgcn_readfirstlane(bk);
        }
        {
            const int2 range = rg[k_first];
            OCC_SCAN1(range.x, range.y)
        }
        auto in_reach = [&](const float4 c, const float r) -> bool {
            const float dx = q.x - c.x, dy = q.y - c.y, dz = q.z - c.z;
            const float d2 = __builtin_fmaf(dz, dz, __builtin_fmaf(dy, dy, dx * dx));
            const float lim = (sb + r) * 1.00001f;
            return __builtin_amdgcn_ballot_w64(q.live && !(d2 > lim * lim)) != 0;
        };
        const int ngrp = sc.ngrp > 0 ? sc.ngrp : 1;
        for (int gi = 0; gi < ngrp; gi++) {
            int k_lo = 0, k_hi = sc.ncl;
            if (sc.ngrp > 0) {
                const float gr = gradius[(size_t)l * sc.ngrp + gi];
                if (gr < 0.0f) continue;
                if (!in_reach(gcenters[gi], gr)) continue;
                const int2 gk = granges[gi];
                k_lo = gk.x, k_hi = gk.y;
            }
            for (int k = k_lo; k < k_hi; k++) {
                if (k == k_first) continue;
                const int2 range = rg[k];
                if (range.x >= range.y) continue;
                if (!in_reach(centers[k], rd[k])) continue;
                OCC_SCAN1(range.x, range.y)
            }
        }
        OCC_EMIT1(l)
    }
}
#undef OCC_PT1
#undef OCC_SCAN1
#undef OCC_EMIT1

constexpr float kSplitExtent2 = 0.04f;

template <bool SPLIT >
__global__ __launch_bounds__(256) void msknn_clustered_kernel(
    const float *__restrict__ xyz, const float *__restrict__ mask , int64_t n_rays, int S,
    const float4 *__restrict__ points, const float4 *__restrict__ centers,
    const int2 *__restrict__ ranges , const float *__restrict__ radius ,
    const float4 *__restrict__ gcenters , const int2 *__restrict__ granges ,
    const float *__restrict__ gradius ,
    ClusteredScales sc, int32_t *__restrict__ knn_idxs, unsigned *__restrict__ ticket,
    const int32_t *__restrict__ qrows ,
    const int32_t *__restrict__ ray_start ,
    const float *__restrict__ center ,
    const int32_t *__restrict__ center_idx ,
    const float split_extent2 ) {
    const int lane = threadIdx.x & 63;
    float ccx = 0.f, ccy = 0.f, ccz = 0.f, cr2 = 0.f;
    if (center) ccx = center[0], ccy = center[1], ccz = center[2], cr2 = center[3];
    const int tiles_per_chunk = (S + 3) / 4;
    const int64_t n_tiles = ((n_rays + 63) / 64) * tiles_per_chunk;
    for (;;) {
        unsigned t32 = 0;
        if (lane == 0) t32 = atomicAdd(ticket, 1u);
        const int64_t job = (int64_t)(unsigned)__builtin_amdgcn_readfirstlane((int)t32);
        const int64_t tile = SPLIT ? job >> 2 : job;
        const int part = SPLIT ? (int)(job & 3) : 0;
        if (tile >= n_tiles) break;
        const int64_t n_blocks = (n_rays + 63) / 64;
        const int64_t blk = qrows ? tile % n_blocks : tile / tiles_per_chunk;
        const int64_t ray = blk * 64 + lane;
        const int s0 = (int)(qrows ? tile / n_blocks : tile % tiles_per_chunk) * 4;
        int64_t qi[kQ];
        bool live[kQ];
        f32x2 qx[2], qy[2], qz[2];
        int32_t hs = 0, hn = 0;
        if (qrows) {
            const int64_t r = ray < n_rays ? ray : n_rays - 1;
            hs = ray_start[r];
            hn = ray < n_rays ? ray_start[r + 1] - hs : 0;
        }
#pragma unroll
        for (int a = 0; a < kQ; a++) {
            live[a] = ray < n_rays && (s0 + a) < S;
            const int64_t r = ray < n_rays ? ray : n_rays - 1;
            const int sm = (s0 + a) < S ? (s0 + a) : S - 1;
            qi[a] = r * S + sm;
            if (qrows) {
                live[a] = (s0 + a) < hn;
                qi[a] = live[a] ? (int64_t)qrows[hs + s0 + a] : r * S;
            }
            if (mask && mask[qi[a]] == 0.0f) live[a] = false;
            qx[a >> 1][a & 1] = xyz[qi[a] * 3 + 0];
            qy[a >> 1][a & 1] = xyz[qi[a] * 3 + 1];
            qz[a >> 1][a & 1] = xyz[qi[a] * 3 + 2];
        }
        if (cr2 > 0.0f) {
#pragma unroll
            for (int a = 0; a < kQ; a++) {
                const float dx = qx[a >> 1][a & 1] - ccx, dy = qy[a >> 1][a & 1] - ccy, dz = qz[a >> 1][a & 1] - ccz;
                const float d2 = __builtin_fmaf(dz, dz, __builtin_fmaf(dy, dy, dx * dx));
                if (live[a] && d2 < cr2) {
                    live[a] = false;
                    struct __attribute__((packed, aligned(4))) I4 { int v[4]; };
                    struct __attribute__((packed, aligned(4))) I2 { int v[2]; };
                    for (int l = 0; part == 0 && l < sc.nscale; l++) {
                        int32_t *out = knn_idxs + (qi[a] * sc.nscale + l) * kK;
                        const int32_t *ci = center_idx + l * kK;
                        *reinterpret_cast<I4 *>(out) = I4{{ci[0], ci[1], ci[2], ci[3]}};
                        *reinterpret_cast<I4 *>(out + 4) = I4{{ci[4], ci[5], ci[6], ci[7]}};
                        *reinterpret_cast<I2 *>(out + 8) = I2{{ci[8], ci[9]}};
                    }
                }
            }
        }
        if (__builtin_amdgcn_ballot_w64(live[0] || live[1] || live[2] || live[3]) == 0) continue;
        if constexpr (SPLIT) {
            float lo[3] = {INFINITY, INFINITY, INFINITY}, hi[3] = {-INFINITY, -INFINITY, -INFINITY};
#pragma unroll
            for (int a = 0; a < kQ; a++) {
                if (live[a]) {
                    const float v[3] = {qx[a >> 1][a & 1], qy[a >> 1][a & 1], qz[a >> 1][a & 1]};
#pragma unroll
                    for (int d = 0; d < 3; d++) lo[d] = fminf(lo[d], v[d]), hi[d] = fmaxf(hi[d], v[d]);
                }
            }
#pragma unroll
            for (int o = 32; o > 0; o >>= 1) {
#pragma unroll
                for (int d = 0; d < 3; d++) {
                    lo[d] = fminf(lo[d], __shfl_xor(lo[d], o));
                    hi[d] = fmaxf(hi[d], __shfl_xor(hi[d], o));
                }
            }
            const float ex = hi[0] - lo[0], ey = hi[1] - lo[1], ez = hi[2] - lo[2];
            const float ext2 = __int_as_float(__builtin_amdgcn_readfirstlane(__float_as_int(ex * ex + ey * ey + ez * ez)));
            const bool spread = ext2 > split_extent2;
            if (!spread && part != 0) continue;
            if (spread) {
                OneQuery q1{0.f, 0.f, 0.f, false};
                int64_t q1i = 0;
#pragma unroll
                for (int a = 0; a < kQ; a++) {
                    if (a == part) {
                        q1 = OneQuery{qx[a >> 1][a & 1], qy[a >> 1][a & 1], qz[a >> 1][a & 1], live[a]};
                        q1i = qi[a];
                    }
                }
                if (__builtin_amdgcn_ballot_w64(q1.live) != 0)
                    search_one_query(q1, q1i, lane, points, centers, ranges, radius, gcenters, granges, gradius, sc, knn_idxs);
                continue;
            }
        }
        KBest64 best[kQ];
        float thr[kQ], sb[kQ];

     \
#define OCC_PT4(P)                                                                          \
    {                                                                                       \
        const f32x2 dx0 = qx[0] - P.x, dy0 = qy[0] - P.y, dz0 = qz[0] - P.z;                \
        const f32x2 dx1 = qx[1] - P.x, dy1 = qy[1] - P.y, dz1 = qz[1] - P.z;                \
        const f32x2 da = __builtin_elementwise_fma(dz0, dz0, __builtin_elementwise_fma(dy0, dy0, dx0 * dx0)); \
        const f32x2 db = __builtin_elementwise_fma(dz1, dz1, __builtin_elementwise_fma(dy1, dy1, dx1 * dx1)); \
        if ((da[0] < thr[0]) | (da[1] < thr[1]) | (db[0] < thr[2]) | (db[1] < thr[3])) {    \
            const int row = __float_as_int(P.w);                                            \
            consider_lex(best[0], thr[0], sb[0], da[0], row);                               \
            consider_lex(best[1], thr[1], sb[1], da[1], row);                               \
            consider_lex(best[2], thr[2], sb[2], db[0], row);                               \
            consider_lex(best[3], thr[3], sb[3], db[1], row);                               \
        }                                                                                   \
    }
        \
#define OCC_SCAN(JB, JE)                                                                    \
    {                                                                                       \
        const int je_ = (JE);                                                               \
        int j = (JB);                                                                       \
        float4 n0 = points[j], n1 = points[j + 1], n2 = points[j + 2], n3 = points[j + 3];  \
        for (; j < je_; j += 4) {                                                           \
            const float4 p0 = n0, p1 = n1, p2 = n2, p3 = n3;                                \
            const int jn = j + 4 < je_ ? j + 4 : j;                                         \
            n0 = points[jn], n1 = points[jn + 1], n2 = points[jn + 2], n3 = points[jn + 3]; \
            OCC_PT4(p0) OCC_PT4(p1) OCC_PT4(p2) OCC_PT4(p3)                                 \
        }                                                                                   \
    }
       \
#define OCC_EMIT(L)                                                                         \
    _Pragma("unroll") for (int a = 0; a < kQ; a++) {                                        \
        if (live[a]) {                                                                      \
            struct __attribute__((packed, aligned(4))) I4 { int v[4]; };                    \
            struct __attribute__((packed, aligned(4))) I2 { int v[2]; };                    \
            int32_t *out = knn_idxs + (qi[a] * sc.nscale + (L)) * kK;                       \
            int r_[kK];                                                                     \
            _Pragma("unroll") for (int p = 0; p < kK; p++) r_[p] = key_row(best[a].k[p]) & 0xFFFF; \
            *reinterpret_cast<I4 *>(out) = I4{{r_[0], r_[1], r_[2], r_[3]}};                \
            *reinterpret_cast<I4 *>(out + 4) = I4{{r_[4], r_[5], r_[6], r_[7]}};            \
            *reinterpret_cast<I2 *>(out + 8) = I2{{r_[8], r_[9]}};                          \
        }                                                                                   \
    }

#pragma unroll
        for (int a = 0; a < kQ; a++) {
            thr[a] = live[a] ? INFINITY : -1.0f;
            sb[a] = INFINITY;
            kbest64_reset(best[a]);
        }
        OCC_SCAN(sc.coarse_begin, sc.coarse_end)
        OCC_EMIT(sc.nscale - 1)

        for (int l = sc.nscale - 2; l >= 0; l--) {
#pragma unroll
            for (int a = 0; a < kQ; a++) {
                sb[a] = sc.seed[l] ? key_dist(best[a].k[kK - 1]) : INFINITY;
                thr[a] = live[a] ? filter_bound(sb[a]) : -1.0f;
                kbest64_reset(best[a]);
            }
            const int2 *rg = ranges + (size_t)l * sc.ncl;
            const float *rd = radius + (size_t)l * sc.ncl;
            int k_first;
            {
                const float rx = __int_as_float(__builtin_amdgcn_readfirstlane(__float_as_int(qx[0][0])));
                const float ry = __int_as_float(__builtin_amdgcn_readfirstlane(__float_as_int(qy[0][0])));
                const float rz = __int_as_float(__builtin_amdgcn_readfirstlane(__float_as_int(qz[0][0])));
                float bd = INFINITY;
                int bk = 0;
                for (int k = lane; k < sc.ncl; k += kWave) {
                    const float4 c = centers[k];
                    const float dx = rx - c.x, dy = ry - c.y, dz = rz - c.z;
                    const float d = dx * dx + dy * dy + dz * dz;
                    const bool has = rg[k].x < rg[k].y;
                    if (has && d < bd) {
                        bd = d;
                        bk = k;
                    }
                }
#pragma unroll
                for (int o = 32; o > 0; o >>= 1) {
                    const float od = __shfl_xor(bd, o);
                    const int ok = __shfl_xor(bk, o);
                    if (od < bd || (od == bd && ok < bk)) {
                        bd = od;
                        bk = ok;
                    }
                }
                k_first = __builtin_amdgcn_readfirstlane(bk);
            }
            {
                const int2 range = rg[k_first];
                OCC_SCAN(range.x, range.y)
            }
            auto in_reach = [&](const float4 c, const float r) -> bool {
                bool want = false;
#pragma unroll
                for (int h = 0; h < 2; h++) {
                    const f32x2 dx = qx[h] - c.x, dy = qy[h] - c.y, dz = qz[h] - c.z;
                    const f32x2 d2 = __builtin_elementwise_fma(dz, dz, __builtin_elementwise_fma(dy, dy, dx * dx));
#pragma unroll
                    for (int e = 0; e < 2; e++) {
                        const float lim = (sb[2 * h + e] + r) * 1.00001f;
                        want |= live[2 * h + e] && !(d2[e] > lim * lim);
// ... 13 lines not shown
                }
                for (int k = k_lo; k < k_hi; k++) {
                    if (k == k_first) continue;
                    const int2 range = rg[k];
                    if (range.x >= range.y) continue;
                    if (!in_reach(centers[k], rd[k])) continue;
                    OCC_SCAN(range.x, range.y)
                }
            }
            OCC_EMIT(l)
        }
#undef OCC_PT4
#undef OCC_SCAN
#undef OCC_EMIT
    }
}

template <int K, int LQ>
__global__ __launch_bounds__(256) void knn_small_kernel(const float *__restrict__ q, int nq,
                                                        const float *__restrict__ s, int ns,
                                                        int32_t *__restrict__ idx) {
    const int g = threadIdx.x & (LQ - 1);
    const int i_raw = (blockIdx.x * blockDim.x + threadIdx.x) / LQ;
    const int i = i_raw < nq ? i_raw : nq - 1;
    const float qx = q[i * 3], qy = q[i * 3 + 1], qz = q[i * 3 + 2];
    double best[K];
#pragma unroll
    for (int p = 0; p < K; p++) best[p] = key64(INFINITY, 0x7fffffff);
    for (int j0 = g; j0 < ns; j0 += 4 * LQ) {
        float sx[4], sy[4], sz[4];
#pragma unroll
        for (int u = 0; u < 4; u++) {
            const int j = j0 + u * LQ < ns ? j0 + u * LQ : ns - 1;
            sx[u] = s[j * 3];
            sy[u] = s[j * 3 + 1];
            sz[u] = s[j * 3 + 2];
        }
#pragma unroll
        for (int u = 0; u < 4; u++) {
            const int j = j0 + u * LQ;
            if (j >= ns) break;
            const float dx = qx - sx[u], dy = qy - sy[u], dz = qz - sz[u];
            double t = key64(sqrtf(__fmaf_rn(dz, dz, __fmaf_rn(dy, dy, __fmul_rn(dx, dx)))), j);
            if (t < best[K - 1]) {
#pragma unroll
                for (int p = 0; p < K; p++) {
                    const double lo = fmin(best[p], t);
                    t = fmax(best[p], t);
                    best[p] = lo;
                }
            }
        }
    }
#pragma unroll
    for (int o = 1; o < LQ; o <<= 1) {
        double other[K];
#pragma unroll
        for (int p = 0; p < K; p++) other[p] = __shfl_xor(best[p], o, LQ);
#pragma unroll
        for (int e = 0; e < K; e++) {
            double t = other[e];
#pragma unroll
            for (int p = 0; p < K; p++) {
                const double lo = fmin(best[p], t);
                t = fmax(best[p], t);
                best[p] = lo;
            }
        }
    }
    if (g == 0 && i_raw < nq) {
#pragma unroll
        for (int p = 0; p < K; p++) idx[i * K + p] = key_row(best[p]);
    }
}

}

OCC_API int occnerf_msknn(const float *xyz, int64_t N, const float *points,
                          const int32_t *index_map, const int32_t *h_scale_begin,
                          const int32_t *h_seed_from_coarser, int32_t nscale, int32_t *knn_idxs,
                          void *stream) {
    using namespace occ;
    if (N <= 0) return 0;
    OCC_REQUIRE(xyz && points && index_map && h_scale_begin && knn_idxs, "msknn: null argument");
    OCC_REQUIRE(nscale >= 1 && nscale <= 4, "msknn: nscale=%d unsupported (1..4)", nscale);
    if (N <= 0) return 0;
    MsKnnScales sc;
    sc.nscale = nscale;
    for (int l = 0; l < nscale; l++) {
        sc.begin[l] = h_scale_begin[l];
        sc.end[l] = h_scale_begin[l + 1];
        OCC_REQUIRE(sc.begin[l] % 4 == 0, "msknn: scale %d must start at a multiple of 4 rows "
                    "(pad each scale with +inf rows)", l);
        OCC_REQUIRE(sc.end[l] - sc.begin[l] >= kK, "msknn: scale %d has fewer than %d points", l, kK);
        sc.seed[l] = h_seed_from_coarser ? h_seed_from_coarser[l] : 0;
    }
    const int64_t tile = 256 * kQ;
    int64_t blocks = (N + tile - 1) / tile;
    if (blocks > (int64_t)kNumCU * 8) blocks = (int64_t)kNumCU * 8;
    hipLaunchKernelGGL(msknn_kernel, dim3((unsigned)blocks), dim3(256), 0, as_stream(stream), xyz, N,
                       reinterpret_cast<const float4 *>(points), index_map, sc, knn_idxs);
    return check_launch("msknn");
}

namespace occ {
__global__ void ray_list_ranges_kernel(const int32_t *__restrict__ qrows, const int32_t *__restrict__ n_dev, int64_t n_rays,
                                       int S, int32_t *__restrict__ ray_start) {
    const int64_t r = (int64_t)blockIdx.x * blockDim.x + threadIdx.x;
    if (r > n_rays) return;
    const int32_t n = *n_dev;
    const int64_t key = r * S;
    int32_t lo = 0, hi = n;
    while (lo < hi) {
        const int32_t mid = (lo + hi) >> 1;
        if ((int64_t)qrows[mid] < key) lo = mid + 1;
        else hi = mid;
    }
    ray_start[r] = lo;
}
}

OCC_API int occnerf_knn_center(const float *c, const float *points, const int32_t *index_map,
                               const int32_t *h_scale_begin, int32_t nscale, float *center_out, int32_t *idx_out, void *stream) {
    using namespace occ;
    OCC_REQUIRE(c && points && index_map && h_scale_begin && center_out && idx_out, "knn_center: null argument");
    OCC_REQUIRE(nscale >= 1 && nscale <= 4, "knn_center: nscale=%d unsupported (1..4)", nscale);
    MsKnnScales sc;
    sc.nscale = nscale;
    for (int l = 0; l < nscale; l++) {
        sc.begin[l] = h_scale_begin[l];
        sc.end[l] = h_scale_begin[l + 1];
        sc.seed[l] = 0;
        OCC_REQUIRE(sc.end[l] - sc.begin[l] >= kK, "knn_center: scale %d has fewer than %d points", l, kK);
    }
    hipLaunchKernelGGL(knn_center_kernel, dim3(1), dim3(256), 0, as_stream(stream), c, reinterpret_cast<const float4 *>(points),
                       index_map, sc, center_out, idx_out);
    return check_launch("knn_center");
}

OCC_API int occnerf_msknn_clustered(const float *xyz, const float *mask, int64_t n_rays, int32_t samples_per_ray,
                                    const float *points,
                                    const float *centers, const int32_t *cluster_ranges,
                                    const float *cluster_radius, int32_t ncl, const float *group_centers,
                                    const int32_t *group_ranges, const float *group_radius, int32_t ngrp,
                                    const int32_t *h_coarse_rows,
                                    const int32_t *h_seed_from_coarser, int32_t nscale,
                                    const int32_t *query_rows, const int32_t *n_query_dev, int32_t *ray_start,
                                    int32_t *knn_idxs, void *stream) {
    return occnerf_msknn_clustered_centered(xyz, mask, n_rays, samples_per_ray, points, centers, cluster_ranges, cluster_radius, ncl,
                                            group_centers, group_ranges, group_radius, ngrp, h_coarse_rows, h_seed_from_coarser,
                                            nscale, query_rows, n_query_dev, ray_start, nullptr, nullptr, knn_idxs, stream);
}

OCC_API int occnerf_msknn_clustered_centered(const float *xyz, const float *mask, int64_t n_rays, int32_t samples_per_ray,
                                             const float *points,
                                             const float *centers, const int32_t *cluster_ranges,
                                             const float *cluster_radius, int32_t ncl, const float *group_centers,
                                             const int32_t *group_ranges, const float *group_radius, int32_t ngrp,
                                             const int32_t *h_coarse_rows,
                                             const int32_t *h_seed_from_coarser, int32_t nscale,
                                             const int32_t *query_rows, const int32_t *n_query_dev, int32_t *ray_start,
                                             const float *center, const int32_t *center_idx,
                                             int32_t *knn_idxs, void *stream) {
    using namespace occ;
    OCC_REQUIRE(!center == !center_idx, "msknn_clustered: center and center_idx come together (occnerf_knn_center)");
    if (n_rays <= 0 || samples_per_ray <= 0) return 0;
    OCC_REQUIRE((!query_rows && !n_query_dev && !ray_start) || (query_rows && n_query_dev && ray_start),
                "msknn_clustered: query_rows, n_query_dev and the ray_start scratch come together");
    OCC_REQUIRE(!(query_rows && mask), "msknn_clustered: a query list replaces the mask");
    OCC_REQUIRE(xyz && points && centers && cluster_ranges && cluster_radius && h_coarse_rows && knn_idxs,
                "msknn_clustered: null argument");
    OCC_REQUIRE(nscale >= 2 && nscale <= 4, "msknn_clustered: nscale=%d unsupported (2..4)", nscale);
    OCC_REQUIRE(ncl >= 1, "msknn_clustered: ncl=%d", ncl);
    OCC_REQUIRE((ngrp == 0 && !group_centers && !group_ranges && !group_radius) ||
                    (ngrp > 0 && group_centers && group_ranges && group_radius),
                "msknn_clustered: group_centers, group_ranges, group_radius and ngrp come together");
    ClusteredScales sc;
    sc.nscale = nscale;
    sc.ncl = ncl;
    sc.ngrp = ngrp;
    sc.coarse_begin = h_coarse_rows[0];
    sc.coarse_end = h_coarse_rows[1];
    OCC_REQUIRE(sc.coarse_begin % 4 == 0 && (sc.coarse_end - sc.coarse_begin) % 4 == 0 &&
                    sc.coarse_end - sc.coarse_begin >= kK, "msknn_clustered: bad coarse row range");
    for (int l = 0; l < 4; l++) {
        sc.seed[l] = (l < nscale && h_seed_from_coarser) ? h_seed_from_coarser[l] : 0;
    }
    const int64_t tiles = ((n_rays + 63) / 64) * ((samples_per_ray + 3) / 4);
    OCC_REQUIRE(tiles < (1ll << 31), "msknn_clustered: too many tiles for one launch");
    const bool split = tiles <= (int64_t)kNumCU * 12 * 4;
    int64_t blocks = ((split ? 4 * tiles : tiles) + 3) / 4;
    if (blocks > (int64_t)kNumCU * 3) blocks = (int64_t)kNumCU * 3;
    constexpr int kTicketLines = 1024;
    static std::mutex mu;
    static std::map<int, unsigned *> pools;
    static std::map<std::pair<int, void *>, unsigned *> lines;
    int dev = 0;
    OCC_REQUIRE(hipGetDevice(&dev) == hipSuccess && dev >= 0, "msknn_clustered: device id");
    unsigned *ticket;
    {
        std::lock_guard<std::mutex> lock(mu);
        unsigned *&pool = pools[dev];
        if (!pool)
            OCC_REQUIRE(hipMalloc(&pool, kTicketLines * 64) == hipSuccess,
                        "msknn_clustered: hipMalloc of the ticket lines (the first call must not be inside a stream capture)");
        auto it = lines.find(std::make_pair(dev, stream));
        if (it == lines.end()) {
            int used = 0;
            for (auto &kv : lines) used += kv.first.first == dev;
            OCC_REQUIRE(used < kTicketLines, "msknn_clustered: more than %d streams on device %d", kTicketLines, dev);
            it = lines.emplace(std::make_pair(dev, stream), pool + 16 * used).first;
        }
        ticket = it->second;
    }
    OCC_REQUIRE(hipMemsetAsync(ticket, 0, sizeof(unsigned), as_stream(stream)) == hipSuccess, "msknn_clustered: memset");
    if (query_rows)
        hipLaunchKernelGGL(ray_list_ranges_kernel, dim3((unsigned)((n_rays + 256) / 256)), dim3(256), 0, as_stream(stream),
                           query_rows, n_query_dev, n_rays, samples_per_ray, ray_start);
    auto kern = split ? msknn_clustered_kernel<true> : msknn_clustered_kernel<false>;
    hipLaunchKernelGGL(kern, dim3((unsigned)blocks), dim3(256), 0, as_stream(stream), xyz, mask,
                       n_rays, samples_per_ray, reinterpret_cast<const float4 *>(points),
                       reinterpret_cast<const float4 *>(centers), reinterpret_cast<const int2 *>(cluster_ranges),
                       cluster_radius, reinterpret_cast<const float4 *>(group_centers),
                       reinterpret_cast<const int2 *>(group_ranges), group_radius, sc, knn_idxs, ticket, query_rows, ray_start,
                       center, center_idx, kSplitExtent2);
    return check_launch("msknn_clustered");
}

OCC_API int occnerf_knn_small(const float *q, int32_t nq, const float *s, int32_t ns, int32_t k,
                              int32_t *idx, void *stream) {
    using namespace occ;
    if (nq <= 0) return 0;
    OCC_REQUIRE(q && s && idx, "knn_small: null argument");
    OCC_REQUIRE(ns >= k, "knn_small: fewer support points (%d) than k (%d)", ns, k);
    if (nq <= 0) return 0;
    hipStream_t st = as_stream(stream);
    const bool wide = ns >= 1024 && nq <= (1 << 20);
    const dim3 block(64), grid(wide ? nq : (nq + 7) / 8);
#define OCC_KS(KK)                                                                                      \
    case KK:                                                                                            \
        if (wide) hipLaunchKernelGGL((knn_small_kernel<KK, 64>), grid, block, 0, st, q, nq, s, ns, idx); \
        else hipLaunchKernelGGL((knn_small_kernel<KK, 8>), grid, block, 0, st, q, nq, s, ns, idx);       \
        break;
    switch (k) {
        OCC_KS(1)
        OCC_KS(3)
        OCC_KS(10)
        OCC_KS(16)
        default: set_error("knn_small: k=%d not built (1, 3, 10, 16)", k); return 1;
    }
#undef OCC_KS
    return check_launch("knn_small");
}
```

occnerf_amd/network.py:

```python
import os

import numpy as np
import torch
import torch.nn as nn

from . import geometry, ops
from .canonical_mlp import CanonicalMLP
from .config import get_cfg
from .rayorder import ray_patch_order
from .modules import (BodyPoseRefiner, MotionBasisComputer, MotionWeightVolumeDecoder,
                      NonRigidMotionMLP, hann_window_weights)


class _Replica(nn.Module):

    def __init__(self, module):
        super().__init__()
        self.module = module

    def forward(self, *a, **k):
        return self.module(*a, **k)


def _load_smpl(cfg):
# ... 59 lines not shown
            mlp_depth=cfg.canonical_mlp.mlp_depth, mlp_width=cfg.canonical_mlp.mlp_width,
            input_ch=63, skips=[], bound=self.bound, detailed_bound=self.detailed_bound))
        self._ctx = self._packed = self._wconst = None

    def deploy_mlps_to_secondary_gpus(self):
        return self

    @property
    def point_cloud(self):
        return self.point_base + self.point_dist

    def _f16x3_flag_word(self):
        w = self.__dict__.get('_f16x3_word')
        if w is None or w.device != self.point_base.device:
            w = self.__dict__['_f16x3_word'] = torch.zeros(1, device=self.point_base.device, dtype=torch.int32)
        return w

    def _f16x3_enqueue_check(self, flag, what):
        self._frames_rendered = getattr(self, '_frames_rendered', 0) + 1
        host = torch.empty(1, dtype=torch.int32, pin_memory=True)
        host.copy_(flag, non_blocking=True)
        flag.zero_()
        done = torch.cuda.Event()
        done.record(torch.cuda.current_stream(flag.device))
        self.__dict__.setdefault('_f16x3_pending', []).append((done, host, f'{what} {self._frames_rendered}'))

    def check_f16x3_domain(self, wait=True):
        pending = self.__dict__.get('_f16x3_pending')
        while pending:
            done, host, frame_no = pending[0]
            if not wait and not done.query():
                return
            done.synchronize()
            pending.pop(0)
            if int(host[0]) != 0:
                pending.clear()
                raise RuntimeError(f"occnerf_amd: {frame_no} of this Network left the domain of the f16x3 kernels (a hidden activation "
                                   'reached 4 094): its results are not fp32-grade -- use mlp_precision=\'fp32\' / '
                                   "train_nonrigid_f16x3=False (a render with cfg.f16x3_domain_check=True falls back by itself, at the "
                                   'price of one wait per frame)')

    def invalidate_cache(self):
        self._ctx = self._packed = self._wconst = None
        self._ray_orders = {}
        self.__dict__.pop('_per_step_graph', None)

    def load_state_dict(self, *a, **k):
        out = super().load_state_dict(*a, **k)
        self.invalidate_cache()
        return out

    def _apply(self, fn, *a, **k):
        out = super()._apply(fn, *a, **k)
        self.invalidate_cache()
        return out

    def _context(self):
        dev = self.point_base.device
        if self._ctx is not None and self._ctx['device'] == dev:
            return self._ctx
        base = self.point_base.detach()
        P = base.shape[0]
        sets = [torch.arange(P)] + [f.long() for f in self.fps_index]
        rows, imap, begin = [], [], [0]
        for idx in sets:
            pts = base[idx.to(dev)]
            pad = (-pts.shape[0]) % 4
            rows.append(torch.cat([pts, torch.full((pad, 3), float('inf'), device=dev)]))
            imap.append(torch.cat([idx, torch.zeros(pad, dtype=idx.dtype)]))
            begin.append(begin[-1] + pts.shape[0] + pad)
        pts4 = torch.cat(rows)
        pts4 = torch.cat([pts4, torch.zeros(pts4.shape[0], 1, device=dev)], dim=1).contiguous()
        as_sets = [set(s.tolist()) for s in sets]
        seed = [int(l + 1 < len(sets) and as_sets[l + 1] <= as_sets[l]) for l in range(len(sets))]
        normals = self.point_norms.to(dev).double().contiguous()
        cl = geometry.build_knn_clusters(base.cpu().numpy(), [s.numpy() for s in sets])
        clusters = {k: (torch.from_numpy(np.ascontiguousarray(v)).to(dev) if k in
                        ('points', 'index_map', 'centers', 'ranges', 'radius', 'group_centers', 'group_ranges', 'group_radius') else v)
                    for k, v in cl.items()}
        self._ctx = {
            'clusters': clusters,
            'device': dev, 'points': pts4, 'index_map': torch.cat(imap).int().to(dev),
            'scale_begin': begin, 'seed': seed, 'normals': normals,
            'unit': ops.unit_normals(normals),
            'bound32': float(np.float32(self.bound)),
            'two_bound32': float(np.float32(2 * np.float64(self.bound))),
        }
        return self._ctx

    def _packed_weights(self):
        cm, nr = self.cnl_mlp.module, self.non_rigid_mlp.module
        nr_lin = [m for m in nr.block_mlps if isinstance(m, nn.Linear)]
        cw, cb = cm.linear_params()
        prec = str(self.cfg.get('mlp_precision', 'fp32'))
        if prec not in ('fp32', 'bf16x3', 'f16x3'):
            raise RuntimeError(f"cfg.mlp_precision must be 'fp32', 'f16x3' or 'bf16x3', got {prec!r}")
        pack_c = {'bf16x3': ops.canonical_mlp_pack_bf16, 'f16x3': ops.canonical_mlp_pack_f16}.get(prec)
        pack_n = {'bf16x3': ops.nonrigid_pack_bf16, 'f16x3': ops.nonrigid_pack_f16}.get(prec)
        srcs = cw + cb + [m.weight for m in nr_lin] + [m.bias for m in nr_lin]
        key = (prec, str(self.cfg.get('f16x3_domain_check', True))) + tuple((t.data_ptr(), t._version) for t in srcs)
        if self._packed is not None and self._packed['key'] == key:
            return self._packed
        self._packed = {
            'key': key,
            'cnl': ops.canonical_mlp_pack(cw, cb),
            'cnl_bf16': pack_c(cw) if pack_c else None,
            'nr': ops.nonrigid_pack([m.weight.detach() for m in nr_lin],
                                    [m.bias.detach() for m in nr_lin]),
            'nr_bf16': pack_n([m.weight.detach() for m in nr_lin]) if pack_n else None,
            'nr_w0': nr_lin[0].weight.detach(), 'nr_b0': nr_lin[0].bias.detach(),
            'domain_flag': torch.zeros(1, device=cw[0].device, dtype=torch.int32)
            if (prec == 'f16x3' and self.cfg.get('f16x3_domain_check', True)) else None,
        }
        return self._packed

    def _weight_constants(self):
        dec_mod = self.mweight_vol_decoder
        enc = self.cnl_mlp.module.encoder
        srcs = list(dec_mod.parameters()) + [self.point_dist, self.point_base, enc.embeddings]
        key = tuple((t.data_ptr(), t._version) for t in srcs)
        if self._wconst is not None and self._wconst['key'] == key:
            return self._wconst
        with torch.no_grad():
            dec = dec_mod.decoder.forward_gemm(dec_mod.const_embedding[None])[0].contiguous()
            table = self._point_stage(self._context())
        self._wconst = {'key': key, 'dec': dec, 'table': table}
        return self._wconst

    def _point_pack(self, wc):
        srcs = [self.point_counter, self.point_base]
        key = (wc['table'].data_ptr(),) + tuple((t.data_ptr(), t._version) for t in srcs)
        if wc.get('pack_key') != key:
            ctx = self._context()
            wc['pack'] = ops.point_pack(self.point_base.detach(), ctx['normals'], ctx['unit'],
                                        self.point_counter.detach(), wc['table'])
            wc['pack_key'] = key
        return wc['pack']

    def _point_stage(self, ctx):
        enc = self.cnl_mlp.module.encoder
        pc = self.point_cloud.detach().float().contiguous()
        base = self.point_base.detach()
        kidx = ops.knn_small(pc, base, 3)
        knn_base, sdf = ops.point_sdf(pc, base, ctx['normals'], ctx['unit'], kidx)
        table = ops.point_table(knn_base, sdf, pc, ctx['bound32'], ctx['two_bound32'],
                                enc.embeddings.detach(), enc.offsets, enc.log2_per_level_scale,
                                enc.base_resolution)
        return table

    def _stage_features(self, rays8, z, xyz, mask, pk, cond, hann, table, pack, center=None):
        cfg, ctx = self.cfg, self._context()
        S = int(cfg.N_samples)
        enc = self.cnl_mlp.module.encoder
        rows, count = ops.live_rows(mask)
        self.last_live_count = count
        dedup = bool(cfg.get('dedup_repeated_samples', True))
        scan_a = scan_b = mrows = mcount = None
        frows, fcount, kmask = rows, count, mask
        if not cfg.ignore_non_rigid_motions:
            if pk['nr_bf16'] is not None:
                ops.nonrigid_bf16x3_rows(xyz, rows, count, cond, hann, pk['nr_w0'], pk['nr_b0'], pk['nr'], pk['nr_bf16'],
                                         domain_flag=pk['domain_flag'])
            else:
                ops.nonrigid_rows(xyz, rows, count, cond, hann, pk['nr_w0'], pk['nr_b0'], pk['nr'])
        if dedup:
            scan_a, frows, fcount, kmask = ops.repeat_heads(xyz, 3, count, rows=rows,
                                                            want_mask=not cfg.get('knn_query_list', True))
            if cfg.get('dedup_global_positions', False):
                frows, fcount = ops.unique_heads(xyz, 3, frows, fcount, scan=scan_a, scan_count=count)
        self.last_head_counts = (fcount, None)
        if cfg.get('knn_query_list', True):
            knn = ops.msknn_clustered(xyz, rays8.shape[0], S, ctx['clusters'], ctx['seed'], rows=frows, count=fcount, center=center)
        else:
            knn = ops.msknn_clustered(xyz, rays8.shape[0], S, ctx['clusters'], ctx['seed'], mask=kmask, center=center)
        if center is not None and len(center) > 3 and center[3] != self._center_stamp(table):
            raise RuntimeError('stale kNN centre: its cached feature row was computed from another table / counter / embedding '
                               'version than this frame\'s (ops.sample_features freshness contract)')
        mlp_in, raw_c, _ = ops.sample_features(
            xyz, knn, self.point_base.detach(), ctx['normals'], ctx['unit'],
            self.point_counter.detach(), table, ctx['bound32'], ctx['two_bound32'],
            enc.embeddings.detach(), enc.offsets, enc.log2_per_level_scale, enc.base_resolution,
            rows=frows, count=fcount, pack=pack, center=None if center is None else center[0],
            center_agg=None if center is None else center[2])
        del knn
        if dedup:
            scan_b, mrows, mcount, _ = ops.repeat_heads(mlp_in, 68, fcount)
            if cfg.get('dedup_global', True):
                mrows, mcount = ops.unique_heads(mlp_in, 68, mrows, mcount, scan=scan_b, scan_count=fcount)
            self.last_head_counts = (fcount, mcount)
        return {'dedup': dedup, 'rays8': rays8, 'z': z, 'mask': mask, 'rows': rows, 'count': count, 'mlp_in': mlp_in,
                'raw_c': raw_c, 'scan_a': scan_a, 'scan_b': scan_b, 'mrows': mrows, 'mcount': mcount, 'cnl': pk['cnl'],
                'cnl_bf16': pk['cnl_bf16'], 'domain_flag': pk['domain_flag'], 'N': xyz.shape[0]}

    @staticmethod
    def _stage_mlp_composite(st, bgcolor, out, out_rows):
        dev, N = st['mlp_in'].device, st['N']

        def mlp(raw_out, count, in_rows=None):
            if st['cnl_bf16'] is not None:
                ops.canonical_mlp_bf16x3(st['mlp_in'], st['cnl'], st['cnl_bf16'], raw_out, count=count, in_rows=in_rows,
                                         domain_flag=st['domain_flag'])
            else:
                ops.canonical_mlp(st['mlp_in'], st['cnl'], raw_out, count=count, in_rows=in_rows)
        if st['dedup']:
            raw_h = torch.empty(st['mlp_in'].shape[0], 5, device=dev)
            mlp(raw_h, st['mcount'], st['mrows'])
            raw = ops.scatter_raw_heads(raw_h, st['raw_c'], st['rows'], st['count'], st['scan_a'], st['scan_b'],
                                        torch.zeros(N, 5, device=dev))
        else:
            mlp(st['raw_c'], st['count'])
            raw = ops.scatter_raw(st['raw_c'], st['rows'], st['count'], torch.zeros(N, 5, device=dev))
        st['mlp_in'] = None
        return ops.composite(raw, st['mask'], st['z'], st['rays8'], bgcolor, out=out, out_rows=out_rows)[:3]

    def _nonrigid_f16_pack(self):
        pk = self._packed_weights()
        if pk.get('nr_f16_train') is None:
            nr_lin = [m for m in self.non_rigid_mlp.module.block_mlps if isinstance(m, nn.Linear)]
            pk['nr_f16_train'] = pk['nr_bf16'] if (pk['nr_bf16'] is not None and pk['nr_bf16'].dtype == torch.float16) else \
                ops.nonrigid_pack_f16([m.weight.detach() for m in nr_lin])
        return pk['nr_f16_train']

    def _knn_center_lists(self, cond, hann):
        ctx, pk = self._context(), self._packed_weights()
        c = torch.zeros(64, 3, device=self.point_base.device)
        if not self.cfg.ignore_non_rigid_motions:
            c = ops.nonrigid(c, cond, hann, pk['nr_w0'], pk['nr_b0'], pk['nr'], direct=True)
        return ops.knn_center(c[0].contiguous(), ctx['points'], ctx['index_map'], ctx['scale_begin'])

    def _knn_center(self, cond, hann, table, pack):
        ctx, pk = self._context(), self._packed_weights()
        c = torch.zeros(64, 3, device=self.point_base.device)
        if not self.cfg.ignore_non_rigid_motions:
            c = ops.nonrigid(c, cond, hann, pk['nr_w0'], pk['nr_b0'], pk['nr'], direct=True)
        center, idx = ops.knn_center(c[0].contiguous(), ctx['points'], ctx['index_map'], ctx['scale_begin'])
        enc = self.cnl_mlp.module.encoder
        row, _, enc_in = ops.sample_features(
            c[:8].contiguous(), idx[None].expand(8, -1, -1).contiguous(), self.point_base.detach(), ctx['normals'], ctx['unit'],
            self.point_counter.detach(), table, ctx['bound32'], ctx['two_bound32'], enc.embeddings.detach(), enc.offsets,
            enc.log2_per_level_scale, enc.base_resolution, pack=pack, want_enc_in=True)
        return center, idx, ops.center_row(row[0], enc_in[0]), self._center_stamp(table)

    def _center_stamp(self, table):
        return (table.data_ptr(), table._version, self.point_counter._version, self.cnl_mlp.module.encoder.embeddings._version)

    def _render_rays(self, rays8, Rs, Ts, vol, bbox_min, bbox_scale, bgcolor, cond, hann,
                     table, t_rand=None, out=None, out_rows=None, pack=None, boxes=None, center=None):
        cfg, ctx = self.cfg, self._context()
        S = int(cfg.N_samples)
        enc = self.cnl_mlp.module.encoder
        t_vals = torch.linspace(0., 1., steps=S, device=rays8.device)
        z, xyz, mask, _ = ops.sample_warp(rays8, S, t_vals, Rs, Ts, vol, bbox_min, bbox_scale,
                                          t_rand=t_rand, boxes=boxes)
        pk = self._packed_weights()
        N = xyz.shape[0]
        if cfg.get('skip_empty_samples', True) and cfg.get('knn_culling', True):
            st = self._stage_features(rays8, z, xyz, mask, pk, cond, hann, table, pack, center)
            return self._stage_mlp_composite(st, bgcolor, out, out_rows)

        if not cfg.ignore_non_rigid_motions:
            if pk['nr_bf16'] is not None:
                ops.nonrigid_bf16x3(xyz, cond, hann, pk['nr_w0'], pk['nr_b0'], pk['nr'], pk['nr_bf16'], out=xyz, domain_flag=pk['domain_flag'])
            else:
                ops.nonrigid(xyz, cond, hann, pk['nr_w0'], pk['nr_b0'], pk['nr'], out=xyz)
        if cfg.get('knn_culling', True):
            knn = ops.msknn_clustered(xyz, rays8.shape[0], S, ctx['clusters'], ctx['seed'], center=center)
        else:
            knn = ops.msknn(xyz, ctx['points'], ctx['index_map'], ctx['scale_begin'], ctx['seed'])
        mlp_in, raw, _ = ops.sample_features(
            xyz, knn, self.point_base.detach(), ctx['normals'], ctx['unit'],
            self.point_counter.detach(), table, ctx['bound32'], ctx['two_bound32'],
            enc.embeddings.detach(), enc.offsets, enc.log2_per_level_scale, enc.base_resolution, pack=pack)
        del knn
        if pk['cnl_bf16'] is not None:
            ops.canonical_mlp_bf16x3(mlp_in, pk['cnl'], pk['cnl_bf16'], raw, domain_flag=pk['domain_flag'])
        else:
            ops.canonical_mlp(mlp_in, pk['cnl'], raw)
        del mlp_in
        return ops.composite(raw, mask, z, rays8, bgcolor, out=out, out_rows=out_rows)[:3]

    @staticmethod
    def _ray_patch_order(rays_d):
        return ray_patch_order(rays_d)

    @staticmethod
    def _host3(v):
        return ops.host_float3(v)

    @torch.no_grad()
    def live_samples_per_ray(self, rays, dst_Rs, dst_Ts, cnl_gtfms, motion_weights_priors, dst_posevec=None,
                             near=None, far=None, iter_val=1e7, **kwargs):
        cfg, dev = self.cfg, self.point_base.device
        f32 = lambda t: t.detach().float().contiguous().to(dev)
        wc = self._weight_constants()
        refine = iter_val >= cfg.pose_decoder.get('kick_in_iter', 0)
        Rs, Ts = ops.pose_motion_bases(self.pose_decoder, f32(dst_posevec).reshape(-1), refine, f32(dst_Rs), f32(dst_Ts),
                                       f32(cnl_gtfms))
        vol = ops.prior_softmax(wc['dec'], f32(motion_weights_priors))
        rays8 = ops.pack_rays(f32(rays).reshape(2, -1, 3), f32(near).reshape(-1), f32(far).reshape(-1), None)
        S = int(cfg.N_samples)
        t_vals = torch.linspace(0., 1., steps=S, device=dev)
        boxes = ops.bone_boxes(vol, Rs.shape[0]) if cfg.get('warp_bone_culling', True) else None
        _, _, mask, _ = ops.sample_warp(rays8, S, t_vals, Rs, Ts, vol, self._host3(kwargs['cnl_bbox_min_xyz']),
                                        self._host3(kwargs['cnl_bbox_scale_xyz']), boxes=boxes)
        return (mask.view(-1, S) != 0).sum(dim=1)

    @torch.no_grad()
    def render_preamble(self, data, iter_val=1e7):
        f32 = lambda t: t.detach().float().contiguous().to(self.point_base.device)
        wc = self._weight_constants()
        refine = iter_val >= self.cfg.pose_decoder.get('kick_in_iter', 0)
        Rs, Ts = ops.pose_motion_bases(self.pose_decoder, f32(data['dst_posevec']).reshape(-1), refine, f32(data['dst_Rs']),
                                       f32(data['dst_Ts']), f32(data['cnl_gtfms']))
        return Rs, Ts, ops.prior_softmax(wc['dec'], f32(data['motion_weights_priors']))

    def forward(self, rays, dst_Rs, dst_Ts, cnl_gtfms, motion_weights_priors, dst_posevec=None,
                near=None, far=None, iter_val=1e7, **kwargs):
        cfg = self.cfg
        dev = self.point_base.device
        if dev.type != 'cuda':
            raise RuntimeError('occnerf_amd.Network renders on a GPU only; move the module with '
                               '.cuda() first (the reference has no CPU path either)')
        dst_Rs, dst_Ts = dst_Rs[None], dst_Ts[None]
        dst_posevec, cnl_gtfms = dst_posevec[None], cnl_gtfms[None]
        motion_weights_priors = motion_weights_priors[None]
        want_grad = torch.is_grad_enabled()
        fused = not want_grad and not self.training
        R = int(near.numel())
        shape = list(rays[1].shape[:-1])
        if R == 0:
            z = torch.zeros(0, device=dev)
            return {'rgb': z.reshape(shape + [3]), 'alpha': z.reshape(shape), 'depth': z.reshape(shape),
                    'comp_loss': torch.zeros(0 if self.training else 1, device=dev)}

        nr = cfg.non_rigid_motion_mlp
        hann = hann_window_weights(nr.multires, iter_val, nr.kick_in_iter, nr.full_band_iter)
        refine = iter_val >= cfg.pose_decoder.get('kick_in_iter', 0)
        bbox_min = self._host3(kwargs['cnl_bbox_min_xyz'])
        bbox_scale = self._host3(kwargs['cnl_bbox_scale_xyz'])
        bgcolor = self._host3(kwargs['bgcolor'])
        S = int(cfg.N_samples)
        rays_o, rays_d = rays

        def morton_order(dirs):
            if not cfg.get('ray_patch_order', True):
                return None
            key = kwargs.get('ray_order_key')
            hit = self._ray_orders.get(key) if key is not None else None
            if hit is not None and hit.numel() == R and hit.device == dirs.device:
                return hit
            order = self._ray_patch_order(dirs)
            if key is not None:
                if len(self._ray_orders) >= 8:
                    self._ray_orders.clear()
                self._ray_orders[key] = order
            return order

        if fused:
            self.check_f16x3_domain(wait=False)
            with torch.no_grad():
                wc = self._weight_constants()
                pack = self._point_pack(wc)
                f32 = lambda t: t.detach().float().contiguous()
                cond = f32(dst_posevec).reshape(-1) if iter_val >= nr.kick_in_iter else \
# ... 91 lines not shown
```

occnerf_amd/ops.py:

```python
import ctypes as C

import numpy as np
import torch

from . import _lib

_f32p = C.POINTER(C.c_float)


def _chk(t, dtype, name):
    if not torch.is_tensor(t):
        raise RuntimeError(f'{name} must be a tensor')
    if not t.is_cuda:
        raise RuntimeError(f'{name} must be a CUDA(HIP) tensor; there is no CPU path')
    if not t.is_contiguous():
        raise RuntimeError(f'{name} must be a contiguous tensor')
    if t.dtype != dtype:
        raise RuntimeError(f'{name} must be {dtype}, got {t.dtype}')
    return t.data_ptr()


def _guard_dev(dev):
    if torch.device(dev).type != 'cuda':
        raise RuntimeError(f'tensors are on {dev}: this path runs on a GPU only, there is no CPU path')
# ... 96 lines not shown
            *args, _chk(outputs, dt, 'outputs'), int(B), int(D), int(Cc), int(L), float(S), int(H), _opt(dy_dx, dt, 'dy_dx'),
            int(gridtype), int(bool(align_corners)), int(interp), _stream(inputs))
    _lib.check(rc, 'grid_encode_forward')


def grid_encode_backward(grad, inputs, embeddings, offsets, grad_embeddings, B, D, Cc, L, S, H,
                         dy_dx=None, grad_inputs=None, gridtype=0, align_corners=False, interp=0):
    dt = _encoder_dtype(grad, 'grid_encode_backward')
    fp32 = dt == torch.float32
    scratch = torch.empty(int(L) * int(B), device=inputs.device, dtype=torch.int64) if (fp32 and int(D) == 4 and int(Cc) == 2
                                                                                      and int(B) >= 32768) else None
    with _guard(inputs):
        args = [_chk(grad, dt, 'grad'), _chk(inputs, torch.float32, 'inputs'), _chk(embeddings, dt, 'embeddings'),
                _chk(offsets, torch.int32, 'offsets')]
        if fp32:
            args.append(_host_offsets(offsets))
        args += [_chk(grad_embeddings, dt, 'grad_embeddings'), int(B), int(D), int(Cc), int(L), float(S), int(H),
                 _opt(dy_dx, dt, 'dy_dx'), _opt(grad_inputs, dt, 'grad_inputs'), int(gridtype), int(bool(align_corners)),
                 int(interp)]
        if fp32:
            args += [None if scratch is None else scratch.data_ptr(), 0 if scratch is None else scratch.numel() * 8]
        rc = getattr(_lib.lib(), 'occnerf_grid_encode_backward' + _ENCODER_ENTRY[dt])(*args, _stream(inputs))
    _lib.check(rc, 'grid_encode_backward')


def grad_total_variation(inputs, embeddings, grad, offsets, weight, B, D, Cc, L, S, H, gridtype=0,
                         align_corners=False):
    rc = _lib.lib().occnerf_grad_total_variation(None, None, None, None, float(weight), int(B), int(D),
                                                 int(Cc), int(L), float(S), int(H), int(gridtype),
                                                 int(bool(align_corners)), None)
    _lib.check(rc, 'grad_total_variation')


def _host_f64(vals, n):
    a = np.ascontiguousarray(np.asarray(vals, dtype=np.float64).ravel())
    assert a.size == n, (a.size, n)
    return a, a.ctypes.data_as(C.c_void_p)


def gen_rays(K, E, H, W, bbox_min, bbox_max, device):
    dev = torch.device(device)
    if dev.type != 'cuda':
        raise RuntimeError(f'gen_rays: needs a GPU device, got {dev}')
    f32 = int(np.asarray(K).dtype == np.float32 and np.asarray(E).dtype == np.float32)
    E = np.asarray(E, dtype=np.float64)
    k0, pk = _host_f64(np.linalg.inv(np.asarray(K)).astype(np.float64), 9)
    r0, pr = _host_f64(E[:3, :3], 9)
    t0, pt = _host_f64(E[:3, 3], 3)
    l0, pl = _host_f64(bbox_min, 3)
    h0, ph = _host_f64(bbox_max, 3)
    rays8 = torch.empty(H * W, 8, device=dev, dtype=torch.float32)
    mask = torch.empty(H * W, device=dev, dtype=torch.uint8)
    with _guard_dev(dev):
        rc = _lib.lib().occnerf_gen_rays(pk, pr, pt, f32, int(H), int(W), pl, ph, rays8.data_ptr(),
                                         mask.data_ptr(), _stream(rays8))
    _lib.check(rc, 'gen_rays')
    return rays8, mask


def bone_boxes(vol, nb):
    boxes = torch.empty(nb, 6, device=vol.device, dtype=torch.int32)
    with _guard(vol):
        rc = _lib.lib().occnerf_bone_boxes(_chk(vol, torch.float32, 'vol'), int(nb), int(vol.shape[-1]), boxes.data_ptr(), _stream(vol))
    _lib.check(rc, 'bone_boxes')
    return boxes


def sample_warp(rays8, S, t_vals, Rs, Ts, vol, bbox_min, bbox_scale, t_rand=None, want_pts=False, boxes=None):
    n = rays8.shape[0]
    dev = rays8.device
    if boxes is not None and t_rand is None and not want_pts:
        z = torch.empty(n, S, device=dev, dtype=torch.float32)
        xs = torch.empty(n * S, 3, device=dev, dtype=torch.float32)
        mk = torch.empty(n * S, device=dev, dtype=torch.float32)
        _kmin, pmin = _host_f32(bbox_min, 3)
        _ksc, psc = _host_f32(bbox_scale, 3)
        with _guard_dev(dev):
            rc = _lib.lib().occnerf_sample_warp_culled(
                _chk(rays8, torch.float32, 'rays'), n, int(S), _chk(t_vals, torch.float32, 't_vals'),
                _chk(Rs, torch.float32, 'Rs'), _chk(Ts, torch.float32, 'Ts'), _chk(vol, torch.float32, 'vol'), int(Rs.shape[0]),
                int(vol.shape[-1]), _chk(boxes, torch.int32, 'boxes'), pmin, psc, z.data_ptr(), xs.data_ptr(), mk.data_ptr(),
                _stream(rays8))
        _lib.check(rc, 'sample_warp_culled')
        return z, xs, mk, None
    z = torch.empty(n, S, device=dev, dtype=torch.float32)
    xs = torch.empty(n * S, 3, device=dev, dtype=torch.float32)
    mk = torch.empty(n * S, device=dev, dtype=torch.float32)
    pts = torch.empty(n * S, 3, device=dev, dtype=torch.float32) if want_pts else None
    _kmin, pmin = _host_f32(bbox_min, 3)
    _ksc, psc = _host_f32(bbox_scale, 3)
    with _guard_dev(dev):
        rc = _lib.lib().occnerf_sample_warp(
            _chk(rays8, torch.float32, 'rays'), n, int(S), _chk(t_vals, torch.float32, 't_vals'),
            _opt(t_rand, torch.float32, 't_rand'), _chk(Rs, torch.float32, 'Rs'),
            _chk(Ts, torch.float32, 'Ts'), _chk(vol, torch.float32, 'vol'), int(Rs.shape[0]),
            int(vol.shape[-1]), pmin, psc, z.data_ptr(), None if pts is None else pts.data_ptr(),
            xs.data_ptr(), mk.data_ptr(), _stream(rays8))
    _lib.check(rc, 'sample_warp')
    return z, xs, mk, pts


def nonrigid_pack(weights, biases):
    dev = weights[0].device
    n = _lib.lib().occnerf_nonrigid_packed_floats()
    packed = torch.zeros(n, device=dev, dtype=torch.float32)
    with _guard_dev(dev):
        rc = _lib.lib().occnerf_nonrigid_pack(_ptr_table(weights, 'W'), _ptr_table(biases, 'b'),
                                              packed.data_ptr(), _stream(packed))
    _lib.check(rc, 'nonrigid_pack')
    return packed


def nonrigid(xyz, cond, hann, W0, b0, packed, out=None, direct=False):
    out = torch.empty_like(xyz) if out is None else out
    _kh, ph = _host_f32(hann, 6)
    fn = _lib.lib().occnerf_nonrigid_direct if direct else _lib.lib().occnerf_nonrigid
    with _guard(xyz):
        rc = fn(
            _chk(xyz, torch.float32, 'xyz'), xyz.shape[0], _chk(cond, torch.float32, 'cond'), ph,
            _chk(W0, torch.float32, 'W0'), _chk(b0, torch.float32, 'b0'),
            _chk(packed, torch.float32, 'packed'), _chk(out, torch.float32, 'xyz_out'), _stream(xyz))
    _lib.check(rc, 'nonrigid')
    return out


def nonrigid_rows(xyz, rows, count, cond, hann, W0, b0, packed):
    _kh, ph = _host_f32(hann, 6)
    with _guard(xyz):
        rc = _lib.lib().occnerf_nonrigid_rows(
            _chk(xyz, torch.float32, 'xyz'), rows.shape[0], _chk(rows, torch.int32, 'rows'),
            _chk(count, torch.int32, 'count'), _chk(cond, torch.float32, 'cond'), ph,
            _chk(W0, torch.float32, 'W0'), _chk(b0, torch.float32, 'b0'), _chk(packed, torch.float32, 'packed'),
            _stream(xyz))
    _lib.check(rc, 'nonrigid_rows')
    return xyz


def live_rows(mask):
    N = mask.shape[0]
    dev = mask.device
    nbytes = int(_lib.lib().occnerf_live_rows_temp_bytes(N))
    if nbytes < 0:
        raise RuntimeError('live_rows: temp size query failed')
    temp = torch.empty(max(nbytes, 16), device=dev, dtype=torch.uint8)
    rows = torch.empty(N, device=dev, dtype=torch.int32)
    count = torch.empty(1, device=dev, dtype=torch.int32)
    with _guard(mask):
        rc = _lib.lib().occnerf_live_rows(_chk(mask, torch.float32, 'mask'), N, rows.data_ptr(), count.data_ptr(),
                                          temp.data_ptr(), nbytes, _stream(mask))
    _lib.check(rc, 'live_rows')
    return rows, count


def scatter_raw(raw_c, rows, count, raw_full):
    with _guard(raw_c):
        rc = _lib.lib().occnerf_scatter_raw(_chk(raw_c, torch.float32, 'raw_c'), _chk(rows, torch.int32, 'rows'),
                                            _chk(count, torch.int32, 'count'), rows.shape[0],
                                            _chk(raw_full, torch.float32, 'raw_full'), _stream(raw_c))
    _lib.check(rc, 'scatter_raw')
    return raw_full


def repeat_heads(keys, key_cols, count, rows=None, want_mask=False):
    dev = keys.device
    if keys.dim() != 2 or not keys.is_contiguous() or keys.element_size() != 4:
        raise RuntimeError('repeat_heads: keys must be a contiguous [M, C] tensor of 4-byte elements')
    cap = keys.shape[0] if rows is None else rows.shape[0]
    scan = torch.empty(cap, device=dev, dtype=torch.int32)
    heads = torch.empty(cap, device=dev, dtype=torch.int32)
    head_count = torch.empty(1, device=dev, dtype=torch.int32)
    head_mask = torch.zeros(keys.shape[0], device=dev, dtype=torch.float32) if want_mask else None
    if cap == 0:
        head_count.zero_()
        return scan, heads, head_count, head_mask
    nbytes = int(_lib.lib().occnerf_repeat_heads_temp_bytes(cap))
    if nbytes < 0:
        raise RuntimeError('repeat_heads: temp size query failed')
    temp = torch.empty(max(nbytes, 16), device=dev, dtype=torch.uint8)
    with _guard_dev(dev):
        rc = _lib.lib().occnerf_repeat_heads(
            keys.data_ptr(), keys.shape[1], int(key_cols), _opt(rows, torch.int32, 'rows'),
            _chk(count, torch.int32, 'count'), cap, scan.data_ptr(), heads.data_ptr(), head_count.data_ptr(),
            None if head_mask is None else head_mask.data_ptr(), temp.data_ptr(), nbytes, _stream(keys))
    _lib.check(rc, 'repeat_heads')
    return scan, heads, head_count, head_mask


def unique_heads(keys, key_cols, heads, count, scan=None, scan_count=None):
    dev = keys.device
    if keys.dim() != 2 or not keys.is_contiguous() or keys.element_size() != 4:
        raise RuntimeError('unique_heads: keys must be a contiguous [M, C] tensor of 4-byte elements')
    cap = keys.shape[0] if heads is None else heads.shape[0]
    heads_out = torch.empty(cap, device=dev, dtype=torch.int32)
    count_out = torch.empty(1, device=dev, dtype=torch.int32)
    if cap == 0:
        count_out.zero_()
        return heads_out, count_out
    nbytes = int(_lib.lib().occnerf_unique_heads_temp_bytes(cap))
    if nbytes <= 0:
        raise RuntimeError('unique_heads: temp size query failed')
    temp = torch.empty(nbytes, device=dev, dtype=torch.uint8)
    with _guard_dev(dev):
        rc = _lib.lib().occnerf_unique_heads(
            keys.data_ptr(), keys.shape[1], int(key_cols), _opt(heads, torch.int32, 'heads'),
            _chk(count, torch.int32, 'count'), cap, heads_out.data_ptr(), count_out.data_ptr(),
            _opt(scan, torch.int32, 'scan'), _opt(scan_count, torch.int32, 'scan_count'),
            0 if scan is None else scan.shape[0], temp.data_ptr(), nbytes, _stream(keys))
    _lib.check(rc, 'unique_heads')
    return heads_out, count_out


def scatter_raw_heads(raw_h, raw_c, rows, count, scan_a, scan_b, raw_full):
    with _guard(raw_c):
        rc = _lib.lib().occnerf_scatter_raw_heads(
            _chk(raw_h, torch.float32, 'raw_h'), _chk(raw_c, torch.float32, 'raw_c'), _chk(rows, torch.int32, 'rows'),
            _chk(count, torch.int32, 'count'), _opt(scan_a, torch.int32, 'scan_a'), _opt(scan_b, torch.int32, 'scan_b'),
            rows.shape[0], _chk(raw_full, torch.float32, 'raw_full'), _stream(raw_c))
    _lib.check(rc, 'scatter_raw_heads')
    return raw_full


def nonrigid_pack_bf16(weights):
    dev = weights[0].device
    n = _lib.lib().occnerf_nonrigid_packed_bf16_bytes()
    packed = torch.zeros(n // 2, device=dev, dtype=torch.bfloat16)
    with _guard_dev(dev):
        rc = _lib.lib().occnerf_nonrigid_pack_bf16(_ptr_table(weights[:6], 'W'), packed.data_ptr(), _stream(packed))
    _lib.check(rc, 'nonrigid_pack_bf16')
    return packed


def nonrigid_pack_f16(weights):
    dev = weights[0].device
    n = _lib.lib().occnerf_nonrigid_packed_bf16_bytes()
    packed = torch.zeros(n // 2, device=dev, dtype=torch.float16)
    with _guard_dev(dev):
        rc = _lib.lib().occnerf_nonrigid_pack_f16(_ptr_table(weights[:6], 'W'), packed.data_ptr(), _stream(packed))
    _lib.check(rc, 'nonrigid_pack_f16')
    return packed


def _nonrigid_f16x3(xyz, rows, count, cond, hann, W0, b0, packed, packed_f16, out, domain_flag=None):
    _kh, ph = _host_f32(hann, 6)
    n_max = xyz.shape[0] if rows is None else rows.shape[0]
    with _guard(xyz):
        rc = _lib.lib().occnerf_nonrigid_f16x3(
            _chk(xyz, torch.float32, 'xyz'), n_max, _opt(rows, torch.int32, 'rows'), _opt(count, torch.int32, 'count'),
            _chk(cond, torch.float32, 'cond'), ph, _chk(W0, torch.float32, 'W0'), _chk(b0, torch.float32, 'b0'),
            _chk(packed, torch.float32, 'packed'), _chk(packed_f16, torch.float16, 'packed_f16'),
            _chk(out, torch.float32, 'xyz_out'), _opt(domain_flag, torch.int32, 'domain_flag'), _stream(xyz))
    _lib.check(rc, 'nonrigid_f16x3')
    return out


def nonrigid_bf16x3(xyz, cond, hann, W0, b0, packed, packed_bf16, out=None, domain_flag=None):
    out = torch.empty_like(xyz) if out is None else out
    if packed_bf16.dtype == torch.float16:
        return _nonrigid_f16x3(xyz, None, None, cond, hann, W0, b0, packed, packed_bf16, out, domain_flag)
    _kh, ph = _host_f32(hann, 6)
    with _guard(xyz):
        rc = _lib.lib().occnerf_nonrigid_bf16x3(
            _chk(xyz, torch.float32, 'xyz'), xyz.shape[0], _chk(cond, torch.float32, 'cond'), ph,
            _chk(W0, torch.float32, 'W0'), _chk(b0, torch.float32, 'b0'), _chk(packed, torch.float32, 'packed'),
            _chk(packed_bf16, torch.bfloat16, 'packed_bf16'), _chk(out, torch.float32, 'xyz_out'), _stream(xyz))
    _lib.check(rc, 'nonrigid_bf16x3')
    return out


def nonrigid_bf16x3_rows(xyz, rows, count, cond, hann, W0, b0, packed, packed_bf16, domain_flag=None):
    if packed_bf16.dtype == torch.float16:
        return _nonrigid_f16x3(xyz, rows, count, cond, hann, W0, b0, packed, packed_bf16, xyz, domain_flag)
    _kh, ph = _host_f32(hann, 6)
    with _guard(xyz):
        rc = _lib.lib().occnerf_nonrigid_bf16x3_rows(
            _chk(xyz, torch.float32, 'xyz'), rows.shape[0], _chk(rows, torch.int32, 'rows'), _chk(count, torch.int32, 'count'),
            _chk(cond, torch.float32, 'cond'), ph, _chk(W0, torch.float32, 'W0'), _chk(b0, torch.float32, 'b0'),
            _chk(packed, torch.float32, 'packed'), _chk(packed_bf16, torch.bfloat16, 'packed_bf16'), _stream(xyz))
    _lib.check(rc, 'nonrigid_bf16x3_rows')
    return xyz


def msknn(xyz, points, index_map, scale_begin, seed_from_coarser):
    N = xyz.shape[0]
    nscale = len(scale_begin) - 1
    out = torch.empty(N, nscale, 10, device=xyz.device, dtype=torch.int32)
    _kb, pb = _host_i32(scale_begin)
    _ks, ps = _host_i32(seed_from_coarser)
    with _guard(xyz):
        rc = _lib.lib().occnerf_msknn(_chk(xyz, torch.float32, 'xyz'), N,
                                      _chk(points, torch.float32, 'points'),
                                      _chk(index_map, torch.int32, 'index_map'), pb, ps, nscale,
                                      out.data_ptr(), _stream(xyz))
    _lib.check(rc, 'msknn')
    return out


def knn_center(c, points, index_map, scale_begin):
    nscale = len(scale_begin) - 1
    center = torch.empty(4, device=c.device, dtype=torch.float32)
    idx = torch.empty(nscale, 10, device=c.device, dtype=torch.int32)
    _kb, pb = _host_i32(scale_begin)
    with _guard(c):
        rc = _lib.lib().occnerf_knn_center(_chk(c, torch.float32, 'c'), _chk(points, torch.float32, 'points'),
                                           _chk(index_map, torch.int32, 'index_map'), pb, nscale, center.data_ptr(), idx.data_ptr(),
                                           _stream(c))
    _lib.check(rc, 'knn_center')
    return center, idx


def msknn_clustered(xyz, n_rays, S, cl, seed_from_coarser, mask=None, rows=None, count=None, out=None, center=None):
    nscale = int(cl['ranges'].shape[0]) + 1
    if out is None:
        out = torch.empty(n_rays * S, nscale, 10, device=xyz.device, dtype=torch.int32)
    if (rows is None) != (count is None) or (rows is not None and mask is not None):
        raise RuntimeError('msknn_clustered: rows and count come together, instead of mask')
    ray_start = torch.empty(n_rays + 1, device=xyz.device, dtype=torch.int32) if rows is not None else None
    _kc, pc = _host_i32(cl['coarse_rows'])
    _ks, ps = _host_i32(seed_from_coarser)
    with _guard(xyz):
        rc = _lib.lib().occnerf_msknn_clustered_centered(
            _chk(xyz, torch.float32, 'xyz'), _opt(mask, torch.float32, 'mask'), int(n_rays), int(S),
            _chk(cl['points'], torch.float32, 'points'), _chk(cl['centers'], torch.float32, 'centers'), _chk(cl['ranges'], torch.int32, 'cluster_ranges'),
            _chk(cl['radius'], torch.float32, 'cluster_radius'), int(cl['ncl']),
            _opt(cl.get('group_centers'), torch.float32, 'group_centers'), _opt(cl.get('group_ranges'), torch.int32, 'group_ranges'),
            _opt(cl.get('group_radius'), torch.float32, 'group_radius'), int(cl.get('ngrp', 0)), pc, ps, nscale,
            _opt(rows, torch.int32, 'rows'), _opt(count, torch.int32, 'count'),
            None if ray_start is None else ray_start.data_ptr(),
            None if center is None else _chk(center[0], torch.float32, 'center'),
            None if center is None else _chk(center[1], torch.int32, 'center_idx'), out.data_ptr(), _stream(xyz))
    _lib.check(rc, 'msknn_clustered')
    return out


def knn_small(q, s, k):
    out = torch.empty(q.shape[0], k, device=q.device, dtype=torch.int32)
    with _guard(q):
        rc = _lib.lib().occnerf_knn_small(_chk(q, torch.float32, 'q'), q.shape[0],
                                          _chk(s, torch.float32, 's'), s.shape[0], int(k),
                                          out.data_ptr(), _stream(q))
    _lib.check(rc, 'knn_small')
    return out


def unit_normals(normals):
    out = torch.empty_like(normals)
    with _guard(normals):
        rc = _lib.lib().occnerf_unit_normals(_chk(normals, torch.float64, 'normals'), normals.shape[0],
                                             out.data_ptr(), _stream(normals))
    _lib.check(rc, 'unit_normals')
    return out


def point_sdf(point_cloud, point_base, normals, unit, kidx):
    P = point_cloud.shape[0]
    kb = torch.empty(P, 3, device=point_cloud.device, dtype=torch.float64)
    dist = torch.empty(P, device=point_cloud.device, dtype=torch.float32)
    with _guard(point_cloud):
        rc = _lib.lib().occnerf_point_sdf(
            _chk(point_cloud, torch.float32, 'point_cloud'), _chk(point_base, torch.float32, 'point_base'),
            _chk(normals, torch.float64, 'normals'), _chk(unit, torch.float64, 'unit_normals'),
            _chk(kidx, torch.int32, 'kidx'), P, kb.data_ptr(), dist.data_ptr(), _stream(point_cloud))
    _lib.check(rc, 'point_sdf')
    return kb, dist


def table_stride():
    return int(_lib.lib().occnerf_point_table_stride())


def point_table(knn_base, sdf, learnable, bound32, two_bound32, embeddings, offsets, S, H):
    P = knn_base.shape[0]
    table = torch.empty(P, table_stride(), device=knn_base.device, dtype=torch.float32)
    with _guard(knn_base):
        rc = _lib.lib().occnerf_point_table(
            _chk(knn_base, torch.float64, 'knn_base'), _chk(sdf, torch.float32, 'point_sdf'),
            _chk(learnable, torch.float32, 'learnable'), P, float(bound32), float(two_bound32),
            _chk(embeddings, torch.float32, 'embeddings'), _chk(offsets, torch.int32, 'offsets'),
            _host_offsets(offsets), int(offsets.shape[0] - 1), float(S), int(H), table.data_ptr(),
            _stream(knn_base))
    _lib.check(rc, 'point_table')
    return table


def point_pack(point_base, normals, unit, counter, table):
    P, dev = point_base.shape[0], point_base.device
    geo = torch.empty(P, 16, device=dev, dtype=torch.float32)
    tail = torch.empty(P, 4, device=dev, dtype=torch.float32)
    with _guard_dev(dev):
        rc = _lib.lib().occnerf_point_pack(
            _chk(point_base, torch.float32, 'point_base'), _chk(normals, torch.float64, 'normals'),
            _chk(unit, torch.float64, 'unit_normals'), _chk(counter, torch.float32, 'counter'),
            _chk(table, torch.float32, 'table'), P, geo.data_ptr(), tail.data_ptr(), _stream(point_base))
    _lib.check(rc, 'point_pack')
    return geo, tail


def center_row(mlp_in_row, enc_in_row):
    return torch.cat([mlp_in_row[:36], enc_in_row[:4], mlp_in_row[36:68]]).contiguous()


def sample_features(xyz, knn_idxs, point_base, normals, unit, counter, table, bound32, two_bound32,
                    embeddings, offsets, S, H, raw=None, want_enc_in=False, geo_idxs=None,
                    att_in=None, rows=None, count=None, pack=None, center=None, center_agg=None):
    N = xyz.shape[0] if rows is None else rows.shape[0]
    dev = xyz.device
    if (pack is None and N > 0 and knn_idxs.shape[1] == 4 and geo_idxs is None and att_in is None
            and counter is not None and table.dim() == 2 and table.shape[1] == table_stride()):
        pack = point_pack(point_base, normals, unit, counter, table)
    geo, tail = pack if pack is not None else (None, None)
    if table.dim() != 2 or table.shape[1] != table_stride():
        raise RuntimeError(f'sample_features: table must be [P,{table_stride()}] (ops.point_table), got {tuple(table.shape)}')
    mlp_in = torch.empty(N, 68, device=dev, dtype=torch.float32)
    raw = torch.empty(N, 5, device=dev, dtype=torch.float32) if raw is None else raw
    enc_in = torch.empty(N, 4, device=dev, dtype=torch.float32) if want_enc_in else None
    with _guard_dev(dev):
        rc = _lib.lib().occnerf_sample_features_centered(
            _chk(xyz, torch.float32, 'xyz'), N, _chk(knn_idxs, torch.int32, 'knn_idxs'),
            int(knn_idxs.shape[1]), _chk(point_base, torch.float32, 'point_base'),
            _chk(normals, torch.float64, 'normals'), _chk(unit, torch.float64, 'unit_normals'),
            _opt(counter, torch.float32, 'counter'), _chk(table, torch.float32, 'table'),
            float(bound32), float(two_bound32), _chk(embeddings, torch.float32, 'embeddings'),
            _chk(offsets, torch.int32, 'offsets'), _host_offsets(offsets), int(offsets.shape[0] - 1),
            float(S), int(H), _opt(geo_idxs, torch.int32, 'geo_idxs'), _opt(att_in, torch.float32, 'att_in'),
            _opt(rows, torch.int32, 'rows'), _opt(count, torch.int32, 'count'),
            _opt(geo, torch.float32, 'point_geo'), _opt(tail, torch.float32, 'point_tail'),
            0 if geo is None else int(geo.shape[0]),
            _opt(center, torch.float32, 'center'), _opt(center_agg, torch.float32, 'center_agg'),
            mlp_in.data_ptr(), _chk(raw, torch.float32, 'raw'),
            None if enc_in is None else enc_in.data_ptr(), _stream(xyz))
    _lib.check(rc, 'sample_features')
    return mlp_in, raw, enc_in


def canonical_mlp_pack(weights, biases):
    dev = weights[0].device
    n = _lib.lib().occnerf_canonical_mlp_packed_floats()
    packed = torch.zeros(n, device=dev, dtype=torch.float32)
    with _guard_dev(dev):
        rc = _lib.lib().occnerf_canonical_mlp_pack(_ptr_table(weights, 'W'), _ptr_table(biases, 'b'),
                                                   packed.data_ptr(), _stream(packed))
    _lib.check(rc, 'canonical_mlp_pack')
    return packed


def canonical_mlp(mlp_in, packed, raw, direct=False, count=None, in_rows=None):
    if in_rows is not None:
        with _guard(mlp_in):
            rc = _lib.lib().occnerf_canonical_mlp_rows(
                _chk(mlp_in, torch.float32, 'mlp_in'), _chk(in_rows, torch.int32, 'in_rows'), in_rows.shape[0],
                _chk(count, torch.int32, 'count'), _chk(packed, torch.float32, 'packed'),
                _chk(raw, torch.float32, 'raw'), _stream(mlp_in))
        _lib.check(rc, 'canonical_mlp_rows')
        return raw
    if count is not None:
        with _guard(mlp_in):
            rc = _lib.lib().occnerf_canonical_mlp_counted(
                _chk(mlp_in, torch.float32, 'mlp_in'), mlp_in.shape[0], _chk(count, torch.int32, 'count'),
                _chk(packed, torch.float32, 'packed'), _chk(raw, torch.float32, 'raw'), _stream(mlp_in))
        _lib.check(rc, 'canonical_mlp_counted')
        return raw
    fn = _lib.lib().occnerf_canonical_mlp_direct if direct else _lib.lib().occnerf_canonical_mlp
    with _guard(mlp_in):
        rc = fn(_chk(mlp_in, torch.float32, 'mlp_in'), mlp_in.shape[0], _chk(packed, torch.float32, 'packed'),
                _chk(raw, torch.float32, 'raw'), _stream(mlp_in))
    _lib.check(rc, 'canonical_mlp')
    return raw


def trunks_pack_bf16(weights, out=None):
    dev = weights[0].device
    if out is None:
        out = torch.zeros(_lib.lib().occnerf_trunks_packed_bytes() // 2, device=dev, dtype=torch.bfloat16)
    with _guard_dev(dev):
        rc = _lib.lib().occnerf_trunks_pack_bf16(_ptr_table(weights[:9], 'W'), out.data_ptr(), _stream(out))
    _lib.check(rc, 'trunks_pack_bf16')
    return out


def trunks_forward_bf16(agg, var, enc, packed_f32, packed_bf16):
    M, dev, bf = agg.shape[0], agg.device, torch.bfloat16
    X0 = torch.empty(M, 96, device=dev, dtype=bf)
    A = [torch.empty(M, 256, device=dev, dtype=bf) for _ in range(4)]
    GEO = torch.empty(M, 96, device=dev, dtype=bf)
    B = [torch.empty(M, 256, device=dev, dtype=bf) for _ in range(4)]
    raw4 = torch.empty(M, 4, device=dev, dtype=torch.float32)
    pa = (C.c_void_p * 4)(*[t.data_ptr() for t in A])
    pb = (C.c_void_p * 4)(*[t.data_ptr() for t in B])
    with _guard(agg):
        rc = _lib.lib().occnerf_trunks_forward_bf16(
            _chk(agg, torch.float32, 'agg'), _chk(var, torch.float32, 'var'), _chk(enc, torch.float32, 'enc'), M,
            _chk(packed_f32, torch.float32, 'packed_f32'), _chk(packed_bf16, torch.bfloat16, 'packed_bf16'), X0.data_ptr(), pa,
            GEO.data_ptr(), pb, raw4.data_ptr(), _stream(agg))
    _lib.check(rc, 'trunks_forward_bf16')
    return X0, A, GEO, B, raw4


def canonical_mlp_pack_bf16(weights):
    dev = weights[0].device
    n = _lib.lib().occnerf_canonical_mlp_packed_bf16_bytes()
    packed = torch.zeros(n // 2, device=dev, dtype=torch.bfloat16)
    with _guard_dev(dev):
        rc = _lib.lib().occnerf_canonical_mlp_pack_bf16(_ptr_table(weights, 'W'), packed.data_ptr(),
                                                        _stream(packed))
    _lib.check(rc, 'canonical_mlp_pack_bf16')
    return packed


def canonical_mlp_pack_f16(weights):
    dev = weights[0].device
    n = _lib.lib().occnerf_canonical_mlp_packed_bf16_bytes()
    packed = torch.zeros(n // 2, device=dev, dtype=torch.float16)
    with _guard_dev(dev):
        rc = _lib.lib().occnerf_canonical_mlp_pack_f16(_ptr_table(weights, 'W'), packed.data_ptr(), _stream(packed))
    _lib.check(rc, 'canonical_mlp_pack_f16')
    return packed


def canonical_mlp_bf16x3(mlp_in, packed, packed_bf16, raw, variant=0, count=None, in_rows=None, domain_flag=None):
    if packed_bf16.dtype == torch.float16:
        n_max = mlp_in.shape[0] if in_rows is None else in_rows.shape[0]
        with _guard(mlp_in):
            rc = _lib.lib().occnerf_canonical_mlp_f16x3(
                _chk(mlp_in, torch.float32, 'mlp_in'), _opt(in_rows, torch.int32, 'in_rows'), n_max,
                _opt(count, torch.int32, 'count'), _chk(packed, torch.float32, 'packed'),
                _chk(packed_bf16, torch.float16, 'packed_f16'), _chk(raw, torch.float32, 'raw'),
                _opt(domain_flag, torch.int32, 'domain_flag'), _stream(mlp_in))
        _lib.check(rc, 'canonical_mlp_f16x3')
        return raw
    with _guard(mlp_in):
        if count is None:
            assert in_rows is None
            rc = _lib.lib().occnerf_canonical_mlp_bf16x3(
                _chk(mlp_in, torch.float32, 'mlp_in'), mlp_in.shape[0], _chk(packed, torch.float32, 'packed'),
                _chk(packed_bf16, torch.bfloat16, 'packed_bf16'), _chk(raw, torch.float32, 'raw'),
                int(variant), _stream(mlp_in))
        else:
            n_max = mlp_in.shape[0] if in_rows is None else in_rows.shape[0]
            rc = _lib.lib().occnerf_canonical_mlp_bf16x3_rows(
                _chk(mlp_in, torch.float32, 'mlp_in'), _opt(in_rows, torch.int32, 'in_rows'), n_max,
                _chk(count, torch.int32, 'count'), _chk(packed, torch.float32, 'packed'),
                _chk(packed_bf16, torch.bfloat16, 'packed_bf16'), _chk(raw, torch.float32, 'raw'), int(variant),
                _stream(mlp_in))
    _lib.check(rc, 'canonical_mlp_bf16x3')
    return raw


def composite(raw, mask, z_vals, rays8, bgcolor, want_weights=False, want_term=False, out=None, out_rows=None):
    n, S = z_vals.shape
    dev = raw.device
    if out is None:
        if out_rows is not None:
            raise RuntimeError('composite: out_rows needs caller-allocated outputs')
        out = (torch.empty(n, 3, device=dev, dtype=torch.float32), torch.empty(n, device=dev, dtype=torch.float32),
               torch.empty(n, device=dev, dtype=torch.float32))
    rgb, acc, dep = out
    for t, nm in ((rgb, 'rgb'), (acc, 'acc'), (dep, 'depth')):
        _chk(t, torch.float32, nm)
    w = torch.empty(n, S, device=dev, dtype=torch.float32) if want_weights else None
    tp = torch.empty(n, device=dev, dtype=torch.int32) if want_term else None
    _kbg, pbg = _host_f32(bgcolor, 3)
    with _guard_dev(dev):
        rc = _lib.lib().occnerf_composite(
            _chk(raw, torch.float32, 'raw'), _chk(mask, torch.float32, 'mask'),
            _chk(z_vals, torch.float32, 'z_vals'), _chk(rays8, torch.float32, 'rays'), pbg, n, int(S),
            rgb.data_ptr(), acc.data_ptr(), dep.data_ptr(), None if w is None else w.data_ptr(),
            None if tp is None else tp.data_ptr(), _opt(out_rows, torch.int64, 'out_rows'), _stream(raw))
    _lib.check(rc, 'composite')
    return rgb, acc, dep, w, tp


def pose_motion_bases(pose_decoder, posevec, refine, dst_Rs, dst_Ts, cnl_gtfms):
    import torch.nn as nn
    dev = dst_Rs.device
    lin = [m for m in pose_decoder.block_mlps if isinstance(m, nn.Linear)]
    if len(lin) != 5 or lin[0].in_features != 69 or lin[0].out_features != 256 or lin[4].out_features != 69:
        raise RuntimeError('pose_motion_bases: the fused kernel is built for the 69 -> 256 x4 -> 69 refiner of occnerf.yaml')
    Rs = torch.empty(24, 3, 3, device=dev, dtype=torch.float32)
    Ts = torch.empty(24, 3, device=dev, dtype=torch.float32)
    with _guard_dev(dev):
        rc = _lib.lib().occnerf_pose_motion_bases(
            _ptr_table([m.weight.detach() for m in lin], 'W'), _ptr_table([m.bias.detach() for m in lin], 'b'),
            _chk(posevec, torch.float32, 'posevec'), int(bool(refine)), _chk(dst_Rs, torch.float32, 'dst_Rs'),
            _chk(dst_Ts, torch.float32, 'dst_Ts'), _chk(cnl_gtfms, torch.float32, 'cnl_gtfms'), Rs.data_ptr(),
            Ts.data_ptr(), _stream(dst_Rs))
    _lib.check(rc, 'pose_motion_bases')
    return Rs, Ts


def prior_softmax(decoded, prior):
    Cn = decoded.shape[0]
    V = decoded.numel() // Cn
    vol = torch.empty_like(decoded)
    with _guard(decoded):
        rc = _lib.lib().occnerf_prior_softmax(_chk(decoded, torch.float32, 'decoded'), _chk(prior, torch.float32, 'prior'),
                                              int(Cn), int(V), vol.data_ptr(), _stream(decoded))
    _lib.check(rc, 'prior_softmax')
    return vol


def ray_order(dirs):
    R = dirs.shape[0]
    order = torch.empty(R, device=dirs.device, dtype=torch.int64)
    if R == 0:
        return order
    if not dirs.is_cuda or dirs.dtype != torch.float32 or dirs.dim() != 2 or dirs.shape[1] != 3 or dirs.stride(1) != 1:
        raise RuntimeError('ray_order: dirs must be a float32 [R,3] GPU tensor with unit element stride')
    nbytes = int(_lib.lib().occnerf_ray_order_temp_bytes(R))
    if nbytes < 0:
        raise RuntimeError('ray_order: temp size query failed')
    temp = torch.empty(nbytes, device=dirs.device, dtype=torch.uint8)
    with _guard(dirs):
        rc = _lib.lib().occnerf_ray_order(dirs.data_ptr(), R, int(dirs.stride(0)), order.data_ptr(), temp.data_ptr(), nbytes,
                                          _stream(dirs))
    _lib.check(rc, 'ray_order')
    return order


def pack_rays(rays, near, far, order=None):
    R = rays.shape[1]
    rays8 = torch.empty(R, 8, device=rays.device, dtype=torch.float32)
    with _guard(rays):
        rc = _lib.lib().occnerf_pack_rays(_chk(rays, torch.float32, 'rays'), _chk(near, torch.float32, 'near'),
                                          _chk(far, torch.float32, 'far'), _opt(order, torch.int64, 'order'), R,
                                          rays8.data_ptr(), _stream(rays))
    _lib.check(rc, 'pack_rays')
    return rays8


def agg_forward(feats, knn, atts):
    N, K = knn.shape
    F = feats.shape[1]
    agg = torch.empty(N, F, device=feats.device, dtype=torch.float32)
    with _guard(feats):
        rc = _lib.lib().occnerf_agg_forward(_chk(feats, torch.float32, 'feats'), int(F), _chk(knn, torch.int32, 'knn'),
                                            _chk(atts, torch.float32, 'atts'), N, int(K), agg.data_ptr(), _stream(feats))
    _lib.check(rc, 'agg_forward')
    return agg


def agg_backward(grad_agg, knn, atts, P):
    N, K = knn.shape
    F = grad_agg.shape[1]
    W = int(_lib.lib().occnerf_agg_backward_slices(N))
    partial = torch.empty(W, P, F, device=grad_agg.device, dtype=torch.float32)
    nbytes = int(_lib.lib().occnerf_agg_backward_scratch_bytes(N, int(F)))
    scratch = torch.empty(max(nbytes, 16), device=grad_agg.device, dtype=torch.uint8)
    with _guard(grad_agg):
        rc = _lib.lib().occnerf_agg_backward(_chk(grad_agg, torch.float32, 'grad_agg'), int(F),
                                             _chk(knn, torch.int32, 'knn'), _chk(atts, torch.float32, 'atts'), N,
                                             int(K), int(P), partial.data_ptr(), scratch.data_ptr(), nbytes,
                                             _stream(grad_agg))
    _lib.check(rc, 'agg_backward')
    return partial.sum(0)


class _Aggregate(torch.autograd.Function):
    @staticmethod
    def forward(ctx, feats, knn, atts):
        feats = feats.contiguous()
        ctx.save_for_backward(knn, atts)
        ctx.P = feats.shape[0]
        return agg_forward(feats, knn, atts)

    @staticmethod
    def backward(ctx, grad_agg):
        knn, atts = ctx.saved_tensors
        return agg_backward(grad_agg.contiguous(), knn, atts, ctx.P), None, None


def aggregate(feats, knn, atts):
    return _Aggregate.apply(feats, knn.contiguous(), atts.contiguous())


def lpips_pack(conv_w, conv_b, lins, shift, scale):
    dev = conv_w[0].device
    packed = torch.empty(int(_lib.lib().occnerf_lpips_packed_floats()), device=dev, dtype=torch.float32)
    w = [t.detach().contiguous() for t in conv_w]
    b = [t.detach().contiguous() for t in conv_b]
    li = [t.detach().contiguous() for t in lins]
    sh, sc = shift.detach().contiguous(), scale.detach().contiguous()
    if len(w) != 13 or len(b) != 13 or len(li) != 5:
        raise RuntimeError('lpips_pack: needs 13 conv weights, 13 conv biases and 5 lin weights')
    with _guard_dev(dev):
        hw, hb, hl = _ptr_table(w, 'conv weight'), _ptr_table(b, 'conv bias'), _ptr_table(li, 'lin weight')
        rc = _lib.lib().occnerf_lpips_pack(hw, hb, hl, _chk(sh, torch.float32, 'shift'), _chk(sc, torch.float32, 'scale'),
                                           packed.data_ptr(), _stream(packed))
    _lib.check(rc, 'lpips_pack')
    return packed


def _lpips_layout(in0, in1):
    if in0.is_contiguous() and in1.is_contiguous():
        return in0, in1, 0
    p0, p1 = in0.permute(0, 2, 3, 1), in1.permute(0, 2, 3, 1)
    if p0.is_contiguous() and p1.is_contiguous():
        return in0, in1, 1
    return in0.contiguous(), in1.contiguous(), 0


def lpips_forward(packed, in0, in1, want_res=False):
    if in0.dim() != 4 or in0.shape != in1.shape or in0.shape[1] != 3:
        raise RuntimeError(f'lpips: in0 and in1 must both be [N,3,H,W], got {tuple(in0.shape)} and {tuple(in1.shape)}')
    N, _, H, W = in0.shape
    in0, in1, nhwc = _lpips_layout(in0, in1)
    with _guard(in0):
        nw = int(_lib.lib().occnerf_lpips_workspace_floats(N, H, W))
        if nw < 0:
            raise RuntimeError(f'lpips: H and W must be >= 16 so that relu5_3 is not empty (got {H} x {W}), N >= 1')
        work = torch.empty(nw, device=in0.device, dtype=torch.float32)
        val = torch.empty(N, device=in0.device, dtype=torch.float32)
        res = torch.empty(5, N, device=in0.device, dtype=torch.float32) if want_res else None
        a0 = _chk(in0.permute(0, 2, 3, 1) if nhwc else in0, torch.float32, 'in0')
        a1 = _chk(in1.permute(0, 2, 3, 1) if nhwc else in1, torch.float32, 'in1')
        rc = _lib.lib().occnerf_lpips_forward(_chk(packed, torch.float32, 'packed'), a0, a1, N, H, W, nhwc, work.data_ptr(),
                                              val.data_ptr(), None if res is None else res.data_ptr(), _stream(in0))
    _lib.check(rc, 'lpips_forward')
    return val, res, work, nhwc


def lpips_backward(packed, work, shape, nhwc, gres, need0, need1):
    N, _, H, W = shape

    def alloc():
# ... 34 lines not shown
```

Measured before the change: 1.209 million rays/s.

## Composite directly from compacted rows and restrict kNN to searched samples

Adds a per-ray segmented live-row selection (count, scan, ballot-write), which yields each ray's start offset into the compacted sample list. Compositing then reads raw values straight from the compacted buffer instead of scattering them into a zero-filled full [N,5] tensor. kNN search and feature sampling also get a 'searched' variant that uses the cached centre index so it only processes searched samples. The aim is to remove the scatter and zero-fill traffic and wasted kNN work on dead samples, at the cost of an extra scan pass and more kernel variants.

```diff
diff --git a/include/occnerf_hip.h b/include/occnerf_hip.h
--- a/include/occnerf_hip.h
+++ b/include/occnerf_hip.h
@@ -117,6 +117,13 @@
 int occnerf_knn_center(const float *c, const float *points, const int32_t *index_map, const int32_t *h_scale_begin,
                        int32_t nscale, float *center_out, int32_t *idx_out, void *stream);
 int occnerf_msknn_clustered_centered(const float *xyz, const float *mask, int64_t n_rays, int32_t samples_per_ray,
+                                     const float *points, const float *centers,
+                                     const int32_t *cluster_ranges, const float *cluster_radius, int32_t ncl,
+                                     const float *group_centers, const int32_t *group_ranges, const float *group_radius, int32_t ngrp,
+                                     const int32_t *h_coarse_rows, const int32_t *h_seed_from_coarser,
+                                     int32_t nscale, const int32_t *query_rows, const int32_t *n_query_dev, int32_t *ray_start,
+                                     const float *center, const int32_t *center_idx, int32_t *knn_idxs, void *stream);
+int occnerf_msknn_clustered_searched(const float *xyz, const float *mask, int64_t n_rays, int32_t samples_per_ray,
                                      const float *points, const float *centers,
                                      const int32_t *cluster_ranges, const float *cluster_radius, int32_t ncl,
                                      const float *group_centers, const int32_t *group_ranges, const float *group_radius, int32_t ngrp,
@@ -164,6 +171,16 @@
                             const int32_t *n_dev, const float *point_geo, const float *point_tail, int32_t P,
                             const float *center, const float *center_agg,
                                      float *mlp_in, float *raw, float *enc_in, void *stream);
+int occnerf_sample_features_searched(const float *xyz, int64_t N, const int32_t *knn_idxs, int32_t nscale,
+                            const float *point_base, const double *normals,
+                            const double *unit_normals, const float *counter,
+                            const float *table, float bound, float two_bound,
+                            const float *embeddings, const int32_t *offsets,
+                            const int32_t *h_offsets, uint32_t L, float S, uint32_t H,
+                            const int32_t *geo_idxs, const float *att_in, const int32_t *rows,
+                            const int32_t *n_dev, const float *point_geo, const float *point_tail, int32_t P,
+                            const float *center, const float *center_agg, const int32_t *center_idx,
+                                     float *mlp_in, float *raw, float *enc_in, void *stream);
 
 int occnerf_agg_forward(const float *feats, int32_t F, const int32_t *knn, const float *atts, int64_t N, int32_t K,
                         float *agg, void *stream);
@@ -177,6 +194,9 @@
                       int64_t temp_bytes, void *stream);
 int occnerf_scatter_raw(const float *raw_c, const int32_t *rows, const int32_t *n_dev, int64_t N_max,
                         float *raw_full, void *stream);
+int64_t occnerf_live_select_temp_bytes(int64_t N, int32_t seg);
+int occnerf_live_select(const float *mask, int64_t N, int32_t seg, int32_t *rows, int32_t *count, int32_t *seg_start,
+                        void *temp, int64_t temp_bytes, void *stream);
 
 int64_t occnerf_repeat_heads_temp_bytes(int64_t N_max);
 int occnerf_repeat_heads(const void *keys, int64_t stride_dwords, int32_t key_dwords, const int32_t *rows,
@@ -223,6 +243,9 @@
 int occnerf_composite(const float *raw, const float *mask, const float *z_vals, const float *rays,
                       const float *h_bgcolor, int64_t n, int32_t S, float *rgb, float *acc,
                       float *depth, float *weights, int32_t *term, const int64_t *out_rows, void *stream);
+int occnerf_composite_compact(const float *raw_c, const int32_t *ray_start, const float *mask, const float *z_vals,
+                              const float *rays, const float *h_bgcolor, int64_t n, int32_t S, float *rgb, float *acc,
+                              float *depth, float *weights, int32_t *term, const int64_t *out_rows, void *stream);
 
 
 int occnerf_linear_pack(const float *W, const float *b, int32_t out_dim, int32_t in_dim, const int32_t *row_map,
diff --git a/occnerf_amd/_lib.py b/occnerf_amd/_lib.py
--- a/occnerf_amd/_lib.py
+++ b/occnerf_amd/_lib.py
@@ -51,6 +51,8 @@
                                            _vp, _vp, _vp, _vp, _vp]),
     'occnerf_msknn_clustered_centered': (C.c_int, [_vp, _vp, _i64, _i32, _vp, _vp, _vp, _vp, _i32, _vp, _vp, _vp, _i32, _vp, _vp, _i32,
                                            _vp, _vp, _vp, _vp, _vp, _vp, _vp]),
+    'occnerf_msknn_clustered_searched': (C.c_int, [_vp, _vp, _i64, _i32, _vp, _vp, _vp, _vp, _i32, _vp, _vp, _vp, _i32, _vp, _vp, _i32,
+                                           _vp, _vp, _vp, _vp, _vp, _vp, _vp]),
     'occnerf_knn_center': (C.c_int, [_vp, _vp, _vp, _vp, _i32, _vp, _vp, _vp]),
     'occnerf_knn_small': (C.c_int, [_vp, _i32, _vp, _i32, _i32, _vp, _vp]),
     'occnerf_unit_normals': (C.c_int, [_vp, _i32, _vp, _vp]),
@@ -66,6 +68,8 @@
     'occnerf_live_rows_temp_bytes': (_i64, [_i64]),
     'occnerf_live_rows': (C.c_int, [_vp, _i64, _vp, _vp, _vp, _i64, _vp]),
     'occnerf_scatter_raw': (C.c_int, [_vp, _vp, _vp, _i64, _vp, _vp]),
+    'occnerf_live_select_temp_bytes': (_i64, [_i64, _i32]),
+    'occnerf_live_select': (C.c_int, [_vp, _i64, _i32, _vp, _vp, _vp, _vp, _i64, _vp]),
     'occnerf_repeat_heads_temp_bytes': (_i64, [_i64]),
     'occnerf_repeat_heads': (C.c_int, [_vp, _i64, _i32, _vp, _vp, _i64, _vp, _vp, _vp, _vp, _vp, _i64, _vp]),
     'occnerf_unique_heads_temp_bytes': (_i64, [_i64]),
@@ -84,6 +88,9 @@
     'occnerf_sample_features_centered': (C.c_int, [_vp, _i64, _vp, _i32, _vp, _vp, _vp, _vp, _vp, _f32, _f32, _vp,
                                                     _vp, _vp, _u32, _f32, _u32, _vp, _vp, _vp, _vp, _vp, _vp, _i32, _vp, _vp,
                                                     _vp, _vp, _vp, _vp]),
+    'occnerf_sample_features_searched': (C.c_int, [_vp, _i64, _vp, _i32, _vp, _vp, _vp, _vp, _vp, _f32, _f32, _vp,
+                                                    _vp, _vp, _u32, _f32, _u32, _vp, _vp, _vp, _vp, _vp, _vp, _i32, _vp, _vp,
+                                                    _vp, _vp, _vp, _vp, _vp]),
     'occnerf_canonical_mlp_packed_floats': (_i64, []),
     'occnerf_canonical_mlp_pack': (C.c_int, [_vp, _vp, _vp, _vp]),
     'occnerf_canonical_mlp': (C.c_int, [_vp, _i64, _vp, _vp, _vp]),
@@ -97,6 +104,7 @@
     'occnerf_nonrigid_f16x3': (C.c_int, [_vp, _i64, _vp, _vp, _vp, _vp, _vp, _vp, _vp, _vp, _vp, _vp, _vp]),
     'occnerf_canonical_mlp_bf16x3_rows': (C.c_int, [_vp, _vp, _i64, _vp, _vp, _vp, _vp, _i32, _vp]),
     'occnerf_composite': (C.c_int, [_vp, _vp, _vp, _vp, _vp, _i64, _i32, _vp, _vp, _vp, _vp, _vp, _vp, _vp]),
+    'occnerf_composite_compact': (C.c_int, [_vp, _vp, _vp, _vp, _vp, _vp, _i64, _i32, _vp, _vp, _vp, _vp, _vp, _vp, _vp]),
     'occnerf_linear_pack': (C.c_int, [_vp, _vp, _i32, _i32, _vp, _i32, _vp, _i32, _i32, _vp, _vp, _vp, _vp]),
     'occnerf_linear_forward': (C.c_int, [_vp, _i64, _i32, _vp, _i64, _i32, _vp, _vp, _i32, _vp, _i64, _vp, _i64, _i32,
                                           _i32, _vp, _i32, _i64, _i64, _i32, _i32, _vp]),
diff --git a/occnerf_amd/csrc/compact.hip b/occnerf_amd/csrc/compact.hip
--- a/occnerf_amd/csrc/compact.hip
+++ b/occnerf_amd/csrc/compact.hip
@@ -8,6 +8,53 @@
     const float *mask;
     __device__ bool operator()(const int &i) const { return mask[i] != 0.0f; }
 };
+
+__device__ __forceinline__ int lanes_below(uint64_t b) {
+    return (int)__builtin_amdgcn_mbcnt_hi((uint32_t)(b >> 32), __builtin_amdgcn_mbcnt_lo((uint32_t)b, 0u));
+}
+
+__global__ __launch_bounds__(256) void live_count_kernel(const float *__restrict__ mask, int64_t N, int seg, int64_t nseg,
+                                                         int32_t *__restrict__ seg_count) {
+    const int lane = threadIdx.x & 63;
+    const int64_t wave = ((int64_t)blockIdx.x * blockDim.x + threadIdx.x) >> 6;
+    const int64_t nwaves = ((int64_t)gridDim.x * blockDim.x) >> 6;
+    for (int64_t g = wave; g < nseg; g += nwaves) {
+        const int64_t base = g * seg;
+        const int len = (int)(N - base < seg ? N - base : seg);
+        int cnt = 0;
+        for (int s0 = 0; s0 < len; s0 += 2 * kWave) {
+            const int sa = s0 + lane, sb = s0 + kWave + lane;
+            const float ma = sa < len ? mask[base + sa] : 0.0f;
+            const float mb = sb < len ? mask[base + sb] : 0.0f;
+            cnt += __popcll(__ballot(ma != 0.0f)) + __popcll(__ballot(mb != 0.0f));
+        }
+        if (lane == 0) seg_count[g] = cnt;
+    }
+}
+
+__global__ __launch_bounds__(256) void live_write_kernel(const float *__restrict__ mask, int64_t N, int seg, int64_t nseg,
+                                                         const int32_t *__restrict__ seg_start, int32_t *__restrict__ rows,
+                                                         int32_t *__restrict__ count) {
+    const int lane = threadIdx.x & 63;
+    const int64_t wave = ((int64_t)blockIdx.x * blockDim.x + threadIdx.x) >> 6;
+    const int64_t nwaves = ((int64_t)gridDim.x * blockDim.x) >> 6;
+    for (int64_t g = wave; g < nseg; g += nwaves) {
+        const int64_t base = g * seg;
+        const int len = (int)(N - base < seg ? N - base : seg);
+        int64_t at = seg_start[g];
+        for (int s0 = 0; s0 < len; s0 += 2 * kWave) {
+            const int sa = s0 + lane, sb = s0 + kWave + lane;
+            const bool la = sa < len && mask[base + sa] != 0.0f;
+            const bool lb = sb < len && mask[base + sb] != 0.0f;
+            const uint64_t ba = __ballot(la), bb = __ballot(lb);
+            if (la) rows[at + lanes_below(ba)] = (int32_t)(base + sa);
+            at += __popcll(ba);
+            if (lb) rows[at + lanes_below(bb)] = (int32_t)(base + sb);
+            at += __popcll(bb);
+        }
+        if (g == nseg - 1 && lane == 0) *count = (int32_t)at;
+    }
+}
 
 __global__ void scatter_raw_kernel(const float *__restrict__ raw_c, const int32_t *__restrict__ rows,
                                    const int32_t *__restrict__ n_dev, float *__restrict__ raw_full) {
@@ -305,6 +352,36 @@
     return check_launch("live_rows");
 }
 
+OCC_API int64_t occnerf_live_select_temp_bytes(int64_t N, int32_t seg) {
+    if (N <= 0 || N >= (1ll << 31) || seg <= 0) return 0;
+    const int64_t nseg = (N + seg - 1) / seg;
+    size_t bytes = 0;
+    if (hipcub::DeviceScan::ExclusiveSum(nullptr, bytes, (int *)nullptr, (int *)nullptr, (int)nseg, (hipStream_t)0) !=
+        hipSuccess)
+        return -1;
+    return (int64_t)bytes;
+}
+
+OCC_API int occnerf_live_select(const float *mask, int64_t N, int32_t seg, int32_t *rows, int32_t *count,
+                                int32_t *seg_start, void *temp, int64_t temp_bytes, void *stream) {
+    using namespace occ;
+    OCC_REQUIRE(mask && rows && count && seg_start && temp, "live_select: null argument");
+    OCC_REQUIRE(N > 0 && N < (1ll << 31), "live_select: N=%lld out of range", (long long)N);
+    OCC_REQUIRE(seg > 0, "live_select: segments of %d samples", seg);
+    OCC_REQUIRE(temp_bytes >= occnerf_live_select_temp_bytes(N, seg), "live_select: temp too small");
+    const int64_t nseg = (N + seg - 1) / seg;
+    int64_t blocks = (nseg + 3) / 4;
+    if (blocks > (int64_t)kNumCU * 32) blocks = (int64_t)kNumCU * 32;
+    hipStream_t st = as_stream(stream);
+    hipLaunchKernelGGL(live_count_kernel, dim3((unsigned)blocks), dim3(256), 0, st, mask, N, seg, nseg, seg_start);
+    size_t bytes = (size_t)temp_bytes;
+    const hipError_t e = hipcub::DeviceScan::ExclusiveSum(temp, bytes, seg_start, seg_start, (int)nseg, st);
+    OCC_REQUIRE(e == hipSuccess, "live_select: %s", hipGetErrorString(e));
+    hipLaunchKernelGGL(live_write_kernel, dim3((unsigned)blocks), dim3(256), 0, st, mask, N, seg, nseg, seg_start, rows,
+                       count);
+    return check_launch("live_select");
+}
+
 OCC_API int occnerf_scatter_raw(const float *raw_c, const int32_t *rows, const int32_t *n_dev, int64_t N_max,
                                 float *raw_full, void *stream) {
     using namespace occ;
diff --git a/occnerf_amd/csrc/composite.hip b/occnerf_amd/csrc/composite.hip
--- a/occnerf_amd/csrc/composite.hip
+++ b/occnerf_amd/csrc/composite.hip
@@ -16,11 +16,12 @@
     float bg[3];
 };
 
+template <bool kCompact>
 __global__ __launch_bounds__(256) void composite_kernel(
     const float *__restrict__ raw, const float *__restrict__ mask, const float *__restrict__ z_vals,
     const float *__restrict__ rays, CompositeParams prm, int64_t n, int S, float *__restrict__ rgb_map,
     float *__restrict__ acc_map, float *__restrict__ depth_map, float *__restrict__ weights,
-    int32_t *__restrict__ term, const int64_t *__restrict__ out_rows) {
+    int32_t *__restrict__ term, const int64_t *__restrict__ out_rows, const int32_t *__restrict__ ray_start) {
     const int lane = threadIdx.x & 63;
     const int64_t wave = ((int64_t)blockIdx.x * blockDim.x + threadIdx.x) >> 6;
     const int64_t nwaves = ((int64_t)gridDim.x * blockDim.x) >> 6;
@@ -31,13 +32,36 @@
         float sr = 0.f, sg = 0.f, sb = 0.f, sd = 0.f, sa = 0.f;
         float best_a = -INFINITY;
         int best_s = 0;
+        int64_t row0 = 0;
+        if (kCompact) row0 = ray_start[r];
         for (int s0 = 0; s0 < S; s0 += kWave) {
             const int s = s0 + lane;
             const bool live = s < S;
             const int64_t i = r * S + (live ? s : S - 1);
             const float z = z_vals[i];
             float alpha = 0.0f, c0 = 0.f, c1 = 0.f, c2 = 0.f;
-            if (live) {
+            if (kCompact) {
+                const float m = live ? mask[i] : 0.0f;
+                const bool has = live && m != 0.0f;
+                const uint64_t b = __ballot(has);
+                if (has) {
+                    const int64_t row = row0 + (int)__builtin_amdgcn_mbcnt_hi((uint32_t)(b >> 32),
+                                                                              __builtin_amdgcn_mbcnt_lo((uint32_t)b, 0u));
+                    const float zn = s + 1 < S ? z_vals[i + 1] : 0.0f;
+                    float dist = s + 1 < S ? __fsub_rn(zn, z) : 1e10f;
+                    dist = __fmul_rn(dist, dn);
+                    const float *rw = raw + row * 5;
+                    const float sp = softplus_t20(rw[3]);
+                    alpha = __fsub_rn(1.0f, expf(-__fmul_rn(sp, dist)));
+                    alpha = __fmul_rn(alpha, m);
+                    c0 = 1.0f / (1.0f + expf(-rw[0]));
+                    c1 = 1.0f / (1.0f + expf(-rw[1]));
+                    c2 = 1.0f / (1.0f + expf(-rw[2]));
+                } else if (live) {
+                    alpha = m;
+                }
+                row0 += __popcll(b);
+            } else if (live) {
                 const float zn = s + 1 < S ? z_vals[i + 1] : 0.0f;
                 float dist = s + 1 < S ? __fsub_rn(zn, z) : 1e10f;
                 dist = __fmul_rn(dist, dn);
@@ -116,7 +140,25 @@
     for (int c = 0; c < 3; c++) prm.bg[c] = h_bgcolor[c];
     int64_t blocks = (n + 3) / 4;
     if (blocks > (int64_t)kNumCU * 32) blocks = (int64_t)kNumCU * 32;
-    hipLaunchKernelGGL(composite_kernel, dim3((unsigned)blocks), dim3(256), 0, as_stream(stream), raw, mask,
-                       z_vals, rays, prm, n, S, rgb, acc, depth, weights, term, out_rows);
+    hipLaunchKernelGGL(composite_kernel<false>, dim3((unsigned)blocks), dim3(256), 0, as_stream(stream), raw, mask,
+                       z_vals, rays, prm, n, S, rgb, acc, depth, weights, term, out_rows, (const int32_t *)nullptr);
     return check_launch("composite");
 }
+
+OCC_API int occnerf_composite_compact(const float *raw_c, const int32_t *ray_start, const float *mask, const float *z_vals,
+                                      const float *rays, const float *h_bgcolor, int64_t n, int32_t S, float *rgb,
+                                      float *acc, float *depth, float *weights, int32_t *term, const int64_t *out_rows,
+                                      void *stream) {
+    using namespace occ;
+    if (n <= 0) return 0;
+    OCC_REQUIRE(raw_c && ray_start && mask && z_vals && rays && h_bgcolor && rgb && acc && depth,
+                "composite_compact: null argument");
+    OCC_REQUIRE(S >= 1, "composite_compact: S=%d", S);
+    CompositeParams prm;
+    for (int c = 0; c < 3; c++) prm.bg[c] = h_bgcolor[c];
+    int64_t blocks = (n + 3) / 4;
+    if (blocks > (int64_t)kNumCU * 32) blocks = (int64_t)kNumCU * 32;
+    hipLaunchKernelGGL(composite_kernel<true>, dim3((unsigned)blocks), dim3(256), 0, as_stream(stream), raw_c, mask,
+                       z_vals, rays, prm, n, S, rgb, acc, depth, weights, term, out_rows, ray_start);
+    return check_launch("composite_compact");
+}
diff --git a/occnerf_amd/csrc/features.hip b/occnerf_amd/csrc/features.hip
--- a/occnerf_amd/csrc/features.hip
+++ b/occnerf_amd/csrc/features.hip
@@ -394,7 +394,8 @@
     LevelRecs levels, LevelRecs8 levels8, FeatParams prm, const int32_t *__restrict__ rows ,
     const int32_t *__restrict__ n_dev , float *__restrict__ mlp_in, float *__restrict__ raw, float *__restrict__ enc_in_out,
     const float *__restrict__ center ,
-    const float *__restrict__ center_agg ) {
+    const float *__restrict__ center_agg ,
+    const int32_t *__restrict__ center_idx ) {
     constexpr int NK = 4 * kKnn;
     float ccx = 0.f, ccy = 0.f, ccz = 0.f, cr2 = 0.f;
     if (center) ccx = center[0], ccy = center[1], ccz = center[2], cr2 = center[3];
@@ -436,6 +437,12 @@
         a.id5[0] = q.v[0], a.id5[1] = q.v[1], a.id5[2] = q.v[2], a.id5[3] = q.v[3];
         a.id5[4] = id[g * 5 + 4];
     };
+    int cidg = 0, cid89 = 0, cid5[5] = {0, 0, 0, 0, 0};
+    if (center_idx) {
+        cidg = center_idx[g], cid89 = center_idx[8 + (g >> 2)];
+#pragma unroll
+        for (int k = 0; k < 5; k++) cid5[k] = center_idx[g * 5 + k];
+    }
     StageA cur, nxt;
     int32_t i1;
     {
@@ -454,6 +461,11 @@
             const float dx = cur.p[0] - ccx, dy = cur.p[1] - ccy, dz = cur.p[2] - ccz;
             const bool inside = __builtin_fmaf(dz, dz, __builtin_fmaf(dy, dy, dx * dx)) < cr2;
             cached_agg = __builtin_amdgcn_ballot_w64(live && !inside) == 0;
+            if (center_idx && inside) {
+                cur.idg = cidg, cur.id89 = cid89;
+#pragma unroll
+                for (int k = 0; k < 5; k++) cur.id5[k] = cid5[k];
+            }
         }
         float4 tl[5];
 #pragma unroll
@@ -774,8 +786,25 @@
                                              const float *point_geo, const float *point_tail, int32_t P,
                                              const float *center, const float *center_agg,
                                              float *mlp_in, float *raw, float *enc_in, void *stream) {
+    return occnerf_sample_features_searched(xyz, N, knn_idxs, nscale, point_base, normals, unit_normals, counter, table, bound,
+                                            two_bound, embeddings, offsets, h_offsets, L, S, H, geo_idxs, att_in, rows, n_dev,
+                                            point_geo, point_tail, P, center, center_agg, nullptr, mlp_in, raw, enc_in, stream);
+}
+
+OCC_API int occnerf_sample_features_searched(const float *xyz, int64_t N, const int32_t *knn_idxs,
+                                             int32_t nscale, const float *point_base, const double *normals,
+                                             const double *unit_normals, const float *counter,
+                                             const float *table, float bound, float two_bound,
+                                             const float *embeddings, const int32_t *offsets,
+                                             const int32_t *h_offsets, uint32_t L, float S, uint32_t H,
+                                             const int32_t *geo_idxs,
+                                             const float *att_in, const int32_t *rows, const int32_t *n_dev,
+                                             const float *point_geo, const float *point_tail, int32_t P,
+                                             const float *center, const float *center_agg, const int32_t *center_idx,
+                                             float *mlp_in, float *raw, float *enc_in, void *stream) {
     using namespace occ;
     OCC_REQUIRE(!center == !center_agg, "sample_features: center and center_agg come together");
+    OCC_REQUIRE(!center_idx || center, "sample_features: center_idx comes with center and center_agg");
     if (N <= 0) return 0;
     OCC_REQUIRE(xyz && knn_idxs && point_base && normals && unit_normals && (counter || att_in) && table &&
                     embeddings && offsets && mlp_in && raw, "sample_features: null argument");
@@ -818,7 +847,7 @@
                            N, knn_idxs, reinterpret_cast<const float4 *>(point_geo),
                            reinterpret_cast<const float4 *>(point_tail),
                            reinterpret_cast<const float4 *>(table), reinterpret_cast<const float2 *>(embeddings),
-                           levels, levels8, prm, rows, n_dev, mlp_in, raw, enc_in, center, center_agg);
+                           levels, levels8, prm, rows, n_dev, mlp_in, raw, enc_in, center, center_agg, center_idx);
         return check_launch("sample_features");
     }
     OCC_REQUIRE(!center, "sample_features: the centre aggregate is only supported on the renderer's path");
diff --git a/occnerf_amd/csrc/knn.hip b/occnerf_amd/csrc/knn.hip
--- a/occnerf_amd/csrc/knn.hip
+++ b/occnerf_amd/csrc/knn.hip
@@ -348,7 +348,8 @@
     const int32_t *__restrict__ ray_start ,
     const float *__restrict__ center ,
     const int32_t *__restrict__ center_idx ,
-    const float split_extent2 ) {
+    const float split_extent2 ,
+    const bool store_center ) {
     const int lane = threadIdx.x & 63;
     float ccx = 0.f, ccy = 0.f, ccz = 0.f, cr2 = 0.f;
     if (center) ccx = center[0], ccy = center[1], ccz = center[2], cr2 = center[3];
@@ -398,7 +399,7 @@
                     live[a] = false;
                     struct __attribute__((packed, aligned(4))) I4 { int v[4]; };
                     struct __attribute__((packed, aligned(4))) I2 { int v[2]; };
-                    for (int l = 0; part == 0 && l < sc.nscale; l++) {
+                    for (int l = 0; store_center && part == 0 && l < sc.nscale; l++) {
                         int32_t *out = knn_idxs + (qi[a] * sc.nscale + l) * kK;
                         const int32_t *ci = center_idx + l * kK;
                         *reinterpret_cast<I4 *>(out) = I4{{ci[0], ci[1], ci[2], ci[3]}};
@@ -718,6 +719,15 @@
                                             nscale, query_rows, n_query_dev, ray_start, nullptr, nullptr, knn_idxs, stream);
 }
 
+static int msknn_clustered_launch(const float *xyz, const float *mask, int64_t n_rays, int32_t samples_per_ray,
+                                  const float *points, const float *centers, const int32_t *cluster_ranges,
+                                  const float *cluster_radius, int32_t ncl, const float *group_centers,
+                                  const int32_t *group_ranges, const float *group_radius, int32_t ngrp,
+                                  const int32_t *h_coarse_rows, const int32_t *h_seed_from_coarser, int32_t nscale,
+                                  const int32_t *query_rows, const int32_t *n_query_dev, int32_t *ray_start,
+                                  const float *center, const int32_t *center_idx, bool store_center, int32_t *knn_idxs,
+                                  void *stream);
+
 OCC_API int occnerf_msknn_clustered_centered(const float *xyz, const float *mask, int64_t n_rays, int32_t samples_per_ray,
                                              const float *points,
                                              const float *centers, const int32_t *cluster_ranges,
@@ -728,6 +738,36 @@
                                              const int32_t *query_rows, const int32_t *n_query_dev, int32_t *ray_start,
                                              const float *center, const int32_t *center_idx,
                                              int32_t *knn_idxs, void *stream) {
+    return msknn_clustered_launch(xyz, mask, n_rays, samples_per_ray, points, centers, cluster_ranges, cluster_radius, ncl,
+                                  group_centers, group_ranges, group_radius, ngrp, h_coarse_rows, h_seed_from_coarser, nscale,
+                                  query_rows, n_query_dev, ray_start, center, center_idx, true, knn_idxs, stream);
+}
+
+OCC_API int occnerf_msknn_clustered_searched(const float *xyz, const float *mask, int64_t n_rays, int32_t samples_per_ray,
+                                             const float *points,
+                                             const float *centers, const int32_t *cluster_ranges,
+                                             const float *cluster_radius, int32_t ncl, const float *group_centers,
+                                             const int32_t *group_ranges, const float *group_radius, int32_t ngrp,
+                                             const int32_t *h_coarse_rows,
+                                             const int32_t *h_seed_from_coarser, int32_t nscale,
+                                             const int32_t *query_rows, const int32_t *n_query_dev, int32_t *ray_start,
+                                             const float *center, const int32_t *center_idx,
+                                             int32_t *knn_idxs, void *stream) {
+    using namespace occ;
+    OCC_REQUIRE(center && center_idx, "msknn_clustered_searched: needs the centre cache (occnerf_knn_center)");
+    return msknn_clustered_launch(xyz, mask, n_rays, samples_per_ray, points, centers, cluster_ranges, cluster_radius, ncl,
+                                  group_centers, group_ranges, group_radius, ngrp, h_coarse_rows, h_seed_from_coarser, nscale,
+                                  query_rows, n_query_dev, ray_start, center, center_idx, false, knn_idxs, stream);
+}
+
+static int msknn_clustered_launch(const float *xyz, const float *mask, int64_t n_rays, int32_t samples_per_ray,
+                                  const float *points, const float *centers, const int32_t *cluster_ranges,
+                                  const float *cluster_radius, int32_t ncl, const float *group_centers,
+                                  const int32_t *group_ranges, const float *group_radius, int32_t ngrp,
+                                  const int32_t *h_coarse_rows, const int32_t *h_seed_from_coarser, int32_t nscale,
+                                  const int32_t *query_rows, const int32_t *n_query_dev, int32_t *ray_start,
+                                  const float *center, const int32_t *center_idx, bool store_center, int32_t *knn_idxs,
+                                  void *stream) {
     using namespace occ;
     OCC_REQUIRE(!center == !center_idx, "msknn_clustered: center and center_idx come together (occnerf_knn_center)");
     if (n_rays <= 0 || samples_per_ray <= 0) return 0;
@@ -789,7 +829,7 @@
                        reinterpret_cast<const float4 *>(centers), reinterpret_cast<const int2 *>(cluster_ranges),
                        cluster_radius, reinterpret_cast<const float4 *>(group_centers),
                        reinterpret_cast<const int2 *>(group_ranges), group_radius, sc, knn_idxs, ticket, query_rows, ray_start,
-                       center, center_idx, kSplitExtent2);
+                       center, center_idx, kSplitExtent2, store_center);
     return check_launch("msknn_clustered");
 }
 
diff --git a/occnerf_amd/network.py b/occnerf_amd/network.py
--- a/occnerf_amd/network.py
+++ b/occnerf_amd/network.py
@@ -235,7 +235,7 @@
         cfg, ctx = self.cfg, self._context()
         S = int(cfg.N_samples)
         enc = self.cnl_mlp.module.encoder
-        rows, count = ops.live_rows(mask)
+        rows, count, ray_start = ops.live_select(mask, S)
         self.last_live_count = count
         dedup = bool(cfg.get('dedup_repeated_samples', True))
         scan_a = scan_b = mrows = mcount = None
@@ -252,10 +252,13 @@
             if cfg.get('dedup_global_positions', False):
                 frows, fcount = ops.unique_heads(xyz, 3, frows, fcount, scan=scan_a, scan_count=count)
         self.last_head_counts = (fcount, None)
+        sparse = center is not None and bool(cfg.get('knn_center_sparse', True))
         if cfg.get('knn_query_list', True):
-            knn = ops.msknn_clustered(xyz, rays8.shape[0], S, ctx['clusters'], ctx['seed'], rows=frows, count=fcount, center=center)
+            knn = ops.msknn_clustered(xyz, rays8.shape[0], S, ctx['clusters'], ctx['seed'], rows=frows, count=fcount, center=center,
+                                      searched_only=sparse)
         else:
-            knn = ops.msknn_clustered(xyz, rays8.shape[0], S, ctx['clusters'], ctx['seed'], mask=kmask, center=center)
+            knn = ops.msknn_clustered(xyz, rays8.shape[0], S, ctx['clusters'], ctx['seed'], mask=kmask, center=center,
+                                      searched_only=sparse)
         if center is not None and len(center) > 3 and center[3] != self._center_stamp(table):
             raise RuntimeError('stale kNN centre: its cached feature row was computed from another table / counter / embedding '
                                'version than this frame\'s (ops.sample_features freshness contract)')
@@ -264,14 +267,15 @@
             self.point_counter.detach(), table, ctx['bound32'], ctx['two_bound32'],
             enc.embeddings.detach(), enc.offsets, enc.log2_per_level_scale, enc.base_resolution,
             rows=frows, count=fcount, pack=pack, center=None if center is None else center[0],
-            center_agg=None if center is None else center[2])
+            center_agg=None if center is None else center[2], center_idx=center[1] if sparse else None)
         del knn
         if dedup:
             scan_b, mrows, mcount, _ = ops.repeat_heads(mlp_in, 68, fcount)
             if cfg.get('dedup_global', True):
                 mrows, mcount = ops.unique_heads(mlp_in, 68, mrows, mcount, scan=scan_b, scan_count=fcount)
             self.last_head_counts = (fcount, mcount)
-        return {'dedup': dedup, 'rays8': rays8, 'z': z, 'mask': mask, 'rows': rows, 'count': count, 'mlp_in': mlp_in,
+        return {'dedup': dedup, 'rays8': rays8, 'z': z, 'mask': mask, 'rows': rows, 'count': count, 'ray_start': ray_start,
+                'mlp_in': mlp_in,
                 'raw_c': raw_c, 'scan_a': scan_a, 'scan_b': scan_b, 'mrows': mrows, 'mcount': mcount, 'cnl': pk['cnl'],
                 'cnl_bf16': pk['cnl_bf16'], 'domain_flag': pk['domain_flag'], 'N': xyz.shape[0]}
 
@@ -292,7 +296,9 @@
                                         torch.zeros(N, 5, device=dev))
         else:
             mlp(st['raw_c'], st['count'])
-            raw = ops.scatter_raw(st['raw_c'], st['rows'], st['count'], torch.zeros(N, 5, device=dev))
+            st['mlp_in'] = None
+            return ops.composite_compact(st['raw_c'], st['ray_start'], st['mask'], st['z'], st['rays8'], bgcolor, out=out,
+                                         out_rows=out_rows)[:3]
         st['mlp_in'] = None
         return ops.composite(raw, st['mask'], st['z'], st['rays8'], bgcolor, out=out, out_rows=out_rows)[:3]
 
diff --git a/occnerf_amd/ops.py b/occnerf_amd/ops.py
--- a/occnerf_amd/ops.py
+++ b/occnerf_amd/ops.py
@@ -272,6 +272,23 @@
     return rows, count
 
 
+def live_select(mask, seg):
+    N, seg = mask.shape[0], int(seg)
+    dev = mask.device
+    nbytes = int(_lib.lib().occnerf_live_select_temp_bytes(N, seg))
+    if nbytes < 0:
+        raise RuntimeError('live_select: temp size query failed')
+    temp = torch.empty(max(nbytes, 16), device=dev, dtype=torch.uint8)
+    rows = torch.empty(N, device=dev, dtype=torch.int32)
+    count = torch.empty(1, device=dev, dtype=torch.int32)
+    seg_start = torch.empty((N + seg - 1) // max(seg, 1), device=dev, dtype=torch.int32)
+    with _guard(mask):
+        rc = _lib.lib().occnerf_live_select(_chk(mask, torch.float32, 'mask'), N, seg, rows.data_ptr(), count.data_ptr(),
+                                            seg_start.data_ptr(), temp.data_ptr(), nbytes, _stream(mask))
+    _lib.check(rc, 'live_select')
+    return rows, count, seg_start
+
+
 def scatter_raw(raw_c, rows, count, raw_full):
     with _guard(raw_c):
         rc = _lib.lib().occnerf_scatter_raw(_chk(raw_c, torch.float32, 'raw_c'), _chk(rows, torch.int32, 'rows'),
@@ -428,7 +445,10 @@
     return center, idx
 
 
-def msknn_clustered(xyz, n_rays, S, cl, seed_from_coarser, mask=None, rows=None, count=None, out=None, center=None):
+def msknn_clustered(xyz, n_rays, S, cl, seed_from_coarser, mask=None, rows=None, count=None, out=None, center=None,
+                    searched_only=False):
+    if searched_only and center is None:
+        raise RuntimeError('msknn_clustered: searched_only needs the centre cache')
     nscale = int(cl['ranges'].shape[0]) + 1
     if out is None:
         out = torch.empty(n_rays * S, nscale, 10, device=xyz.device, dtype=torch.int32)
@@ -438,7 +458,8 @@
     _kc, pc = _host_i32(cl['coarse_rows'])
     _ks, ps = _host_i32(seed_from_coarser)
     with _guard(xyz):
-        rc = _lib.lib().occnerf_msknn_clustered_centered(
+        fn = _lib.lib().occnerf_msknn_clustered_searched if searched_only else _lib.lib().occnerf_msknn_clustered_centered
+        rc = fn(
             _chk(xyz, torch.float32, 'xyz'), _opt(mask, torch.float32, 'mask'), int(n_rays), int(S),
             _chk(cl['points'], torch.float32, 'points'), _chk(cl['centers'], torch.float32, 'centers'), _chk(cl['ranges'], torch.int32, 'cluster_ranges'),
             _chk(cl['radius'], torch.float32, 'cluster_radius'), int(cl['ncl']),
@@ -521,7 +542,7 @@
 
 def sample_features(xyz, knn_idxs, point_base, normals, unit, counter, table, bound32, two_bound32,
                     embeddings, offsets, S, H, raw=None, want_enc_in=False, geo_idxs=None,
-                    att_in=None, rows=None, count=None, pack=None, center=None, center_agg=None):
+                    att_in=None, rows=None, count=None, pack=None, center=None, center_agg=None, center_idx=None):
     N = xyz.shape[0] if rows is None else rows.shape[0]
     dev = xyz.device
     if (pack is None and N > 0 and knn_idxs.shape[1] == 4 and geo_idxs is None and att_in is None
@@ -534,7 +555,7 @@
     raw = torch.empty(N, 5, device=dev, dtype=torch.float32) if raw is None else raw
     enc_in = torch.empty(N, 4, device=dev, dtype=torch.float32) if want_enc_in else None
     with _guard_dev(dev):
-        rc = _lib.lib().occnerf_sample_features_centered(
+        rc = _lib.lib().occnerf_sample_features_searched(
             _chk(xyz, torch.float32, 'xyz'), N, _chk(knn_idxs, torch.int32, 'knn_idxs'),
             int(knn_idxs.shape[1]), _chk(point_base, torch.float32, 'point_base'),
             _chk(normals, torch.float64, 'normals'), _chk(unit, torch.float64, 'unit_normals'),
@@ -546,7 +567,7 @@
             _opt(geo, torch.float32, 'point_geo'), _opt(tail, torch.float32, 'point_tail'),
             0 if geo is None else int(geo.shape[0]),
             _opt(center, torch.float32, 'center'), _opt(center_agg, torch.float32, 'center_agg'),
-            mlp_in.data_ptr(), _chk(raw, torch.float32, 'raw'),
+            _opt(center_idx, torch.int32, 'center_idx'), mlp_in.data_ptr(), _chk(raw, torch.float32, 'raw'),
             None if enc_in is None else enc_in.data_ptr(), _stream(xyz))
     _lib.check(rc, 'sample_features')
     return mlp_in, raw, enc_in
@@ -689,6 +710,33 @@
     return rgb, acc, dep, w, tp
 
 
+def composite_compact(raw_c, ray_start, mask, z_vals, rays8, bgcolor, want_weights=False, want_term=False, out=None,
+                      out_rows=None):
+    n, S = z_vals.shape
+    dev = raw_c.device
+    if ray_start.shape[0] != n or mask.numel() != n * S:
+        raise RuntimeError(f'composite_compact: ray_start[{ray_start.shape[0]}] / mask[{mask.numel()}] for {n} rays of {S}')
+    if out is None:
+        if out_rows is not None:
+            raise RuntimeError('composite_compact: out_rows needs caller-allocated outputs')
+        out = (torch.empty(n, 3, device=dev, dtype=torch.float32), torch.empty(n, device=dev, dtype=torch.float32),
+               torch.empty(n, device=dev, dtype=torch.float32))
+    rgb, acc, dep = out
+    for t, nm in ((rgb, 'rgb'), (acc, 'acc'), (dep, 'depth')):
+        _chk(t, torch.float32, nm)
+    w = torch.empty(n, S, device=dev, dtype=torch.float32) if want_weights else None
+    tp = torch.empty(n, device=dev, dtype=torch.int32) if want_term else None
+    _kbg, pbg = _host_f32(bgcolor, 3)
+    with _guard_dev(dev):
+        rc = _lib.lib().occnerf_composite_compact(
+            _chk(raw_c, torch.float32, 'raw_c'), _chk(ray_start, torch.int32, 'ray_start'),
+            _chk(mask, torch.float32, 'mask'), _chk(z_vals, torch.float32, 'z_vals'), _chk(rays8, torch.float32, 'rays'),
+            pbg, n, int(S), rgb.data_ptr(), acc.data_ptr(), dep.data_ptr(), None if w is None else w.data_ptr(),
+            None if tp is None else tp.data_ptr(), _opt(out_rows, torch.int64, 'out_rows'), _stream(raw_c))
+    _lib.check(rc, 'composite_compact')
+    return rgb, acc, dep, w, tp
+
+
 def pose_motion_bases(pose_decoder, posevec, refine, dst_Rs, dst_Ts, cnl_gtfms):
     import torch.nn as nn
     dev = dst_Rs.device
```

Result: no change. 1.219 million rays/s (median of 6 runs) (+0.8%).
